# jizongFox/Self-paced-Contrastive-Learning

Measured on AMD Instinct MI355X. Metric: pretrain slices/sec/node (UNet+InfoNCE, 224^2, bs=32/GPU), higher is better.
Workload: dtype bf16; 1 GPU; BASELINE.json configs[1]: self-paced pretrain step, UNet base (max_channel=256) encoder to Conv5 + ProjectionHead(256,256,256) + SelfPacedSupConLoss(soft, partition labels, correct_grad) fwd+bwd + RAdam; slices_per_gpu=32, images_per_gpu_step=64, image=1x224x224, global_batch=32, parallelism=dp1, params=1311056, hipgraph=epocher, capture_steps=3

## Files before the change

### include/spcl_hip.h

```cpp
#ifndef SPCL_HIP_H
#define SPCL_HIP_H
#include <stddef.h>
#include <stdint.h>
#ifdef __cplusplus
extern "C" {
#endif

#define SPCL_F32 0
#define SPCL_BF16 1

#define SPCL_OK 0
#define SPCL_EINVAL (-1)
#define SPCL_ELAUNCH (-2)
#define SPCL_EUNSUPPORTED (-3)

#define SPCL_ABI_VERSION 22
int spcl_abi_version(void);
const char* spcl_last_error(void);

size_t spcl_supcon_workspace_bytes(int n, int d);
int spcl_supcon_forward(const float* z1, const float* z2, const float* labels, const float* mask, int n, int d,
                        float temperature, int sp_mode, float gamma, int correct_grad, float* ws, float* out,
                        void* stream);
int spcl_supcon_backward(const float* labels, const float* mask, int n, int d, float temperature, int sp_mode,
                         float gamma, const float* ws_fwd, float* ws_bwd, const float* out_fwd,
                         const float* grad_out, float* dz1, float* dz2, void* stream);
size_t spcl_supcon_bwd_workspace_bytes(int n, int d);
int spcl_supcon_unit_gradient_block(int n, int d, size_t* offset_floats, int* row_pitch);
int spcl_supcon_forward_heads(int K, const float* z1, const float* z2, size_t z_stride, const float* labels, int n,
                              int d, float temperature, int sp_mode, const float* gammas, int correct_grad, float* ws,
                              size_t ws_stride, float* out, void* stream);
int spcl_supcon_rows_supported(int n, int d);
int spcl_supcon_forward_rows(int K, const float* o1, const float* o2, size_t o_stride, const float* labels, int n, int d,
                             float temperature, int sp_mode, const float* gammas, int correct_grad, float* ws,
                             size_t ws_stride, float* out, void* stream);
int spcl_supcon_backward_heads(int K, const float* labels, int n, int d, float temperature, int sp_mode,
                               const float* gammas, const float* ws_fwd, size_t ws_stride, float* ws_bwd,
                               size_t wsb_stride, const float* out_fwd, const float* grad_out, float* dz1, float* dz2,
                               size_t z_stride, void* stream);
int spcl_supcon_materialize(const float* labels, const float* mask, int n, int d, float temperature, int sp_mode,
                            float gamma, const float* ws_fwd, float* sim_logits, float* sim_exp, float* pos_mask,
                            float* neg_mask, float* sp_mask, void* stream);

size_t spcl_supcon_xpos_workspace_bytes(int n, int d);
int spcl_supcon_xpos_forward(const float* z1, const float* z2, const float* labels, const float* mask, int n, int d,
                             float temperature, float* ws, float* out, void* stream);
int spcl_supcon_xpos_backward(const float* z1, const float* z2, int n, int d, float temperature, const float* ws,
                              const float* grad_out, float* dz1, float* dz2, void* stream);

size_t spcl_supcon_weighted_workspace_bytes(int n, int d);
int spcl_supcon_weighted_forward(const float* z1, const float* z2, const float* labels, const float* w11,
                                 const float* w22, const float* w12, int blocks, int mask_semantics, int in_mode, int n,
                                 int d, float temperature, float* ws, float* out, void* stream);
int spcl_supcon_weighted_backward(const float* z1, const float* z2, int n, int d, float temperature, float* ws,
                                  const float* grad_out, float* dz1, float* dz2, void* stream);
int spcl_supcon_weighted_materialize(const float* z1, const float* z2, const float* labels, const float* w11,
                                     const float* w22, const float* w12, int blocks, int mask_semantics, int n, int d,
                                     float temperature, float* ws, float* sim_logits, float* sim_exp, float* pos_weight,
                                     float* enable_mask, void* stream);

int spcl_proj_forward(const void* feat, int dtype, int N, int HW, int C, int Cs, const float* w1, const float* b1,
                      const float* w2, const float* b2, int hid, int out_dim, int normalize, float* pooled,
                      float* pre, float* o, float* z, void* stream);
int spcl_proj_backward(const float* dz, int dtype, int N, int HW, int C, int Cs, const float* w1, const float* w2,
                       int hid, int out_dim, int normalize, const float* pooled, const float* pre, const float* o,
                       float* dw1, float* db1, float* dw2, float* db2, float* scratch ,
                       void* dfeat, void* stream);

int spcl_proj_heads_forward(int K, const void* feat, int dtype, int N, int HW, int C, int Cs, const float* const* w1 ,
                            const float* const* b1 , const float* const* w2 , const float* const* b2 ,
                            int hid, int out_dim, int normalize, float* pooled, float* const* pre ,
                            float* const* o , float* const* z , void* stream);
int spcl_proj_heads_backward(int K, const float* const* dz , int dtype, int N, int HW, int C, int Cs,
                             const float* const* w1 , const float* const* w2 , int hid, int out_dim,
                             int normalize, const float* pooled, const float* const* pre ,
                             const float* const* o , float* const* dw1 , float* const* db1 ,
                             float* const* dw2 , float* const* db2 , float* scratch, void* dfeat, void* stream);
int spcl_proj_heads_backward_pooled(int K, const float* const* dz, int dtype, int N, int HW, int C, int Cs,
                                    const float* const* w1, const float* const* w2, int hid, int out_dim, int normalize,
                                    const float* pooled, const float* const* pre, const float* const* o, float* const* dw1,
                                    float* const* db1, float* const* dw2, float* const* db2, float* scratch, void* dfeat_nc,
                                    void* stream);


size_t spcl_conv_packed_elems(int Cin, int Cout, int kind, int dtype);
int spcl_conv_pack_weights(const float* w_oihw, int Cin, int Cout, int kind, int dtype, void* packed, void* stream);
int spcl_conv_pack_weights_both(const float* w_oihw, int Cin, int Cout, int dtype, void* packed_fwd,
                                void* packed_dgrad, void* stream);

int spcl_conv_pack_weights_block(const float* wa_oihw, int CinA, int CoutA, void* a_fwd, void* a_dgrad,
                                 const float* wb_oihw, int CinB, int CoutB, void* b_fwd, void* b_dgrad, int dtype,
                                 void* stream);
int spcl_conv_pack_weights_block_at(const float* wa_oihw, int CinA, int CoutA, void* a_fwd, void* a_dgrad,
                                    const float* wb_oihw, int CinB, int CoutB, void* b_fwd, void* b_dgrad, int dtype,
                                    int H, int W, void* stream);

#define SPCL_PACK_MULTI_MAX 24
typedef struct spcl_pack_item {
  const float* w_oihw;
// ... 236 lines not shown
                          void* stream);
int spcl_adam_apply_staged(float* param, const float* grad, double grad_scale, float* exp_avg, float* exp_avg_sq, size_t n,
                           int64_t* step, const float* coef, double beta1, double beta2, double eps, double weight_decay,
                           int decoupled, int k, const void* const* src, void* const* dst, const float* count, void* stream);
int spcl_sgd_step_scaled(float* param, const float* grad, double grad_scale, float* momentum_buffer, size_t n, int64_t* step,
                         const float* lr, double momentum, double dampening, double weight_decay, int nesterov, float* coef,
                         int k, const void* const* src, void* const* dst, const float* count, void* stream);
int spcl_sgd_apply_staged(float* param, const float* grad, double grad_scale, float* momentum_buffer, size_t n, int64_t* step,
                          const float* coef, double momentum, double dampening, double weight_decay, int nesterov, int k,
                          const void* const* src, void* const* dst, const float* count, void* stream);

int spcl_accumulate_scalars(int k, const void* const* src, void* const* dst, const float* count, void* stream);

int spcl_stage_bytes(void* dst, const void* host_src, size_t nbytes, void* stream);
int spcl_copy_pair(void* dst_a, const void* src_a, size_t bytes_a, void* dst_b, const void* src_b, size_t bytes_b,
                   void* stream);

int spcl_augment_views(const float* src, int S, int HS, int WS, const int* params, int nviews, float* out, int OH,
                       int OW, void* stream);
int spcl_augment_views_pil(const float* src, int S, int HS, int WS, const int* params, int nviews, float* out, int OH,
                           int OW, void* stream);
int spcl_rows_linear_forward(const void* x, int x_dtype, long ldx, int leaky_in, const float* W, const float* bias, int M,
                             int K, int N, float* y, void* stream);
int spcl_rows_linear_forward_act(const void* x, int x_dtype, long ldx, const float* W, const float* bias, int M, int K, int N,
                                 void* h, int h_dtype, void* stream);
int spcl_adaptive_avgpool2d_backward_act(const float* dout, const void* act, int dtype, int N, int H, int W, int C, int OH,
                                         int OW, void* dx, void* stream);
int spcl_rows_linear_backward_input(const void* g, int g_dtype, const float* W, const float* pre, int M, int N, int K, void* dx,
                                    int dx_dtype, long lddx, void* stream);
size_t spcl_rows_linear_backward_weight_workspace_bytes(int M, int N, int K);
int spcl_rows_linear_backward_weight(const void* g, int g_dtype, const void* x, int x_dtype, long ldx, int leaky_in, int M, int N,
                                     int K, float* ws, size_t ws_bytes, float* dW, float* db, void* stream);
int spcl_augment_views_recipe(const float* src, const unsigned char* labels, int S, int HS, int WS, const int* params,
                              int nviews, float* out, long long* label_out, int OH, int OW, int max_pad, void* stream);
size_t spcl_augment_views_recipe_workspace_bytes(int nviews, int OH, int OW);
int spcl_augment_views_recipe_ws(const float* src, const unsigned char* labels, int S, int HS, int WS, const int* params,
                                 int nviews, float* out, long long* label_out, int OH, int OW, int max_pad, void* workspace,
                                 size_t workspace_bytes, void* stream);
int spcl_resize_bilinear_pil(const float* src, int S, int HS, int WS, const int* bounds_x, const int* kk_x, int ksize_x,
                             const int* bounds_y, const int* kk_y, int ksize_y, float* tmp, float* out, int OH, int OW,
                             void* stream);

int spcl_flip_batch(const void* x, void* out, int elem_size, int N, int C, int H, int W, const uint8_t* flags,
                    void* stream);
int spcl_flip_pair(const void* first, const void* second, void* out, int elem_size, int N, int C, int H, int W,
                   const uint8_t* flags, void* stream);
int spcl_flip_pair_stage(const void* first, const void* second, void* out, int elem_size, int N, int C, int H, int W,
                         void* stage_dst, const void* host_src, size_t nbytes, size_t flag_off, void* stream);

int spcl_profile_enable(int on);
int spcl_profile_count(void);
int spcl_profile_get(int i, char* name, int name_cap, float* usec, double* bytes, double* flops);

typedef struct spcl_bn_acc {
  long long* acc;
  const float* gamma;
  const float* beta;
  float* running_mean;
  float* running_var;
  long long* num_batches_tracked;
  float* st;
  float momentum, eps;
  float count;
  int C, CS;
} spcl_bn_acc;
size_t spcl_bn_acc_elems(int CS);
int spcl_conv_bn_acc_supported(int dtype, int N, int H, int W, int CinK, int CoutS, int in_kind, int with_stats_acc);
int spcl_conv3x3_forward_acc(const void* x, int dtype, int N, int H, int W, int CinK, int CoutS, const void* w_packed,
                             const spcl_bn_acc* in_bn, const float* in_scale, const float* in_shift, void* y,
                             long long* stats_acc, float* stats_rows, void* stream);
int spcl_bnrelu_pool_forward_acc(const void* y, int dtype, int N, int H, int W, int CS, const spcl_bn_acc* bn, void* act_out,
                                 void* pool_out, void* stream);
int spcl_bnrelu_gap_supported(int dtype, int H, int W, int C, int CS);
int spcl_bnrelu_gap_forward(const void* y, int dtype, int N, int H, int W, int C, int CS, const float* scale,
                            const float* shift, const spcl_bn_acc* bn, void* act_out, float* gap_out, void* stream);
int spcl_conv_dgrad_bnstats_acc_supported(int dtype, int N, int H, int W, int CinK, int CoutS);
int spcl_conv3x3_dgrad_bnstats_acc(const void* dy, int dtype, int N, int H, int W, int CinK, int CoutS, const void* w_packed,
                                   void* g, const void* y2, const float* scale2, const float* shift2, const float* mean2,
                                   long long* acc, void* stream);
int spcl_conv_dgrad_poolstats_acc_supported(int dtype, int N, int H, int W, int CinK, int CoutS, int H2, int W2);
int spcl_conv3x3_dgrad_poolstats_acc(const void* dy, int dtype, int N, int H, int W, int CinK, int CoutS, const void* w_packed,
                                     void* g, const void* y2, int H2, int W2, const float* scale2, const float* shift2,
                                     const float* mean2, long long* acc, void* stream);
int spcl_bnrelu_backward_acc(const void* y, const void* dact, const void* dpool, const void* dact_nc, int dtype, int N, int H,
                             int W, int C, int CS, const float* st4, int training, long long* acc, float* dgamma, float* dbeta,
                             void* dy, void* stream);
int spcl_bnrelu_backward_fill_acc(const void* y, void* dact, int dact_stride, const void* dpool, const void* d_up, int dtype,
                                  int N, int H, int W, int C, int CS, const float* st4, int training, long long* acc,
                                  float* dgamma, float* dbeta, void* dy, void* stream);
int spcl_bnrelu_backward_rows_acc(const void* y, const void* dact, const void* dpool, const float* rows, int nrows, int dtype,
                                  int N, int H, int W, int C, int CS, const float* st4, int training, long long* acc,
                                  float* dgamma, float* dbeta, void* dy, void* stream);

size_t spcl_iic_joint_workspace_bytes(int S, int K, int pad);
int spcl_iic_joint_forward(const float* lx, const float* ly, long ld, int N, int H, int W, int S, int K, int pad,
                           const uint8_t* flags_x, long long* jacc, void* stream);
size_t spcl_iic_loss_workspace_bytes(int S, int T);
int spcl_iic_loss(const long long* jacc, const float* jf32, int S, int K, int T, int dense, float scale, float* j_out,
                  float* loss, float* dj, int* nan_flag, void* ws, size_t ws_bytes, void* stream);
int spcl_iic_joint_backward(const float* lx, const float* ly, long ld, int N, int H, int W, int S, int K, int pad,
                            const uint8_t* flags_x, const float* dj, const float* gscale, float* dlx, float* dly, void* stream);
size_t spcl_consistency_workspace_bytes(int N, int H, int W);
int spcl_consistency_softmax_mse(const float* a, const float* b, int N, int C, int H, int W, const uint8_t* flags_a,
                                 float weight, float* loss, float* db, void* ws, size_t ws_bytes, void* stream);

int spcl_iic_patch_plan(int N, int C, int H, int W, int pad, int patch, int* num_patches, size_t* ws_bytes, size_t* dj_elems);
int spcl_iic_patch_forward(const float* lx, const float* ly, int N, int C, int H, int W, int pad, int patch,
                           const uint8_t* flags_y, float scale, float* loss, float* patch_loss, int* nan_flag, float* dj,
                           void* ws, size_t ws_bytes, void* stream);
int spcl_iic_patch_backward(const float* lx, const float* ly, int N, int C, int H, int W, int pad, int patch,
                            const uint8_t* flags_y, const float* dj, const float* gscale, float* dlx, float* dly, void* stream);

int spcl_ema_update(float* teacher, const float* student, size_t n, double alpha, double decay, void* stream);
size_t spcl_mt_softmax_mse_workspace_bytes(int N, int H, int W);
int spcl_mt_softmax_mse(const float* teacher, const float* student_logits, int N, int C, int H, int W,
                        const uint8_t* flags_teacher, int teacher_mode, float weight, float* loss, float* dstudent, void* ws,
                        size_t ws_bytes, void* stream);
size_t spcl_entropy_softmax_workspace_bytes(int N, int H, int W);
int spcl_entropy_softmax(const float* logits, int N, int C, int H, int W, float eps, float weight, float* loss, float* dlogits,
                         void* ws, size_t ws_bytes, void* stream);
size_t spcl_ucmt_workspace_bytes(int N, int H, int W);
int spcl_ucmt_softmax_mse(const float* teacher, const float* const* noisy, int K, const float* student_logits, int N, int C,
                          int H, int W, const uint8_t* flags_teacher, float threshold, float eps, float weight, float* loss,
                          float* dstudent, unsigned long long* kept, uint8_t* mask, void* ws, size_t ws_bytes, void* stream);

int spcl_mixup_images(const float* image, const float* image_tf, const int* index, int N2, size_t per_sample, float lam,
                      float oml, float* out, void* stream);
size_t spcl_mixup_kl_workspace_bytes(int N2, int H, int W);
int spcl_mixup_kl_onehot(const float* logits, const int64_t* target, const int64_t* target_tf, const int* index, int N2, int C,
                         int H, int W, float lam, float oml, float eps, float weight, float* loss, float* dlogits, void* ws,
                         size_t ws_bytes, void* stream);

int spcl_patch4s2_rows_forward(const float* a, int Ca, long a_sn, long a_sc, long a_sh, long a_sw, const float* b, int Cb,
                               long b_sn, long b_sc, long b_sh, long b_sw, int N, int H, int W, int mode, const float* scale,
                               const float* shift, float* rows, void* stream);
int spcl_patch4s2_rows_backward(const float* drows, const float* x, int N, int H, int W, int C, int c_lo, int mode,
                                const float* scale, const float* shift, float* dx, void* stream);
size_t spcl_rows_bn_workspace_bytes(int M, int C);
int spcl_rows_bn_forward(const float* x, int M, int C, const float* gamma, const float* beta, float eps, float momentum,
                         float* running_mean, float* running_var, float* stats, void* ws, size_t ws_bytes, void* stream);
int spcl_rows_bn_eval_affine(const float* gamma, const float* beta, const float* running_mean, const float* running_var,
                             float eps, int C, float* stats, void* stream);
int spcl_rows_bn_backward(const float* du, const float* x, int M, int C, const float* gamma, const float* stats, int training,
                          float* dx, float* dgamma, float* dbeta, void* ws, size_t ws_bytes, void* stream);
size_t spcl_discr_head_workspace_bytes(int N, int H, int W, int C);
int spcl_discr_head_forward(const float* x, int N, int H, int W, int C, const float* scale, const float* shift, const float* w,
                            int y, float* t, float* d, float* loss, float* dt, void* ws, size_t ws_bytes, void* stream);
int spcl_discr_head_backward(const float* x, int N, int H, int W, int C, const float* scale, const float* shift, const float* w,
                             const float* dt, const float* grad, float* du, float* dw, void* ws, size_t ws_bytes, void* stream);

int spcl_mine_pairs_forward(const void* feat, const uint8_t* flags, int dtype, int n, int H, int W, int C, void* joint, void* marg,
                            void* stream);
int spcl_mine_pairs_backward(const void* djoint, const void* dmarg, const uint8_t* flags, int dtype, int n, int H, int W, int C,
                             void* dfeat, void* stream);
size_t spcl_mine_head_workspace_bytes(int n, int H, int W, int C);
int spcl_mine_head_forward(const void* act_joint, const void* act_marg, int dtype, int n, int H, int W, int C, const float* w,
                           const float* b, float* t, float* maxima, int* argmax, float* loss, void* ws, size_t ws_bytes,
                           void* stream);
int spcl_mine_head_backward(const float* t, const float* maxima, const int* argmax, const float* w, const float* grad, int dtype,
                            int n, int H, int W, int C, void* dact_joint, void* dact_marg, float* dw, float* db, void* stream);

size_t spcl_pica_workspace_bytes(int S);
int spcl_pica_seg_loss(const long long* jacc, const float* jf32, int S, int K, int T, double lamda_ne, float scale, float* j_out,
                       float* loss, float* ce_out, float* dj, void* ws, size_t ws_bytes, void* stream);
int spcl_pica_global_loss(const float* lx, const float* ly, long ld, int N, int S, int K, float lamda, float scale,
                          const float* gscale, float* loss, float* ce_out, float* dlx, float* dly, void* ws, size_t ws_bytes,
// ... 7 lines not shown
```

### self-paced-contrastive-learning_amd/csrc/bn.hip

```cpp
#include <mutex>
#include <type_traits>
#include "bn_acc.hpp"
#include "common.hpp"
#include "image_acorr.hpp"

namespace spcl {

typedef __attribute__((ext_vector_type(4))) uint32_t u32x4;
template <typename T> struct Chunk;
template <> struct Chunk<float> { static constexpr int EPC = 4; };
template <> struct Chunk<bf16_t> { static constexpr int EPC = 8; };

template <typename T> __device__ __forceinline__ void unpack(u32x4 raw, float* v);
template <> __device__ __forceinline__ void unpack<float>(u32x4 raw, float* v) {
#pragma unroll
  for (int e = 0; e < 4; ++e) v[e] = __uint_as_float(raw[e]);
}
template <> __device__ __forceinline__ void unpack<bf16_t>(u32x4 raw, float* v) {
#pragma unroll
  for (int e = 0; e < 4; ++e) {
    v[2 * e] = __uint_as_float(raw[e] << 16);
    v[2 * e + 1] = __uint_as_float(raw[e] & 0xffff0000u);
  }
}
// ... 120 lines not shown
    }
    __syncthreads();
    bn_fold_lanes<CW>(n, s1, s2, red);
    if (tl == 0) bn_final_channel(c, C, n, s1, s2, f, SPCL_BN_PREFETCH ? ch : bn_prefetch_channel(c, C, f));
    return;
  }
  if (tl != 0) return;
  if (!FINAL) {
    double* q = partial + (size_t)blockIdx.y * 3 * CS + c;
    q[0] = n; q[CS] = s1; q[2 * CS] = s2;
    return;
  }
  bn_final_channel(c, C, n, s1, s2, f, SPCL_BN_PREFETCH ? ch : bn_prefetch_channel(c, C, f));
}

__device__ __forceinline__ void bn_final_channel(int c, int C, double n, double s1, double s2, const BnFinalArgs& f,
                                                 const BnChan& ch) {
  if (c >= C) {
    f.mean[c] = 0.f; f.invstd[c] = 0.f; f.scale[c] = 0.f; f.shift[c] = 0.f;
    return;
  }
  const double mu = s1 / n;
  const double m2 = fmax(s2 - s1 * mu, 0.0);
  const double var = m2 / n;
  const float is = 1.0f / sqrtf((float)var + f.eps);
  const float sc = ch.gamma * is;
  f.mean[c] = (float)mu;
  f.invstd[c] = is;
  f.scale[c] = sc;
  f.shift[c] = ch.beta - (float)mu * sc;
  if (f.running_mean != nullptr) f.running_mean[c] = (1.f - f.momentum) * ch.rm + f.momentum * (float)mu;
  if (f.running_var != nullptr) {
    const double unbiased = n > 1.0 ? m2 / (n - 1.0) : var;
    f.running_var[c] = (1.f - f.momentum) * ch.rv + f.momentum * (float)unbiased;
  }
  if (f.nbt != nullptr && c == 0) f.nbt[0] += 1;
}

__global__ __launch_bounds__(256) void bn_eval_affine_kernel(int C, int CS, const float* __restrict__ gamma,
                                                             const float* __restrict__ beta,
                                                             const float* __restrict__ rm, const float* __restrict__ rv,
                                                             float eps, float* mean, float* invstd, float* scale,
                                                             float* shift) {
  const int c = blockIdx.x * blockDim.x + threadIdx.x;
  if (c >= CS) return;
  if (c >= C) { mean[c] = 0.f; invstd[c] = 0.f; scale[c] = 0.f; shift[c] = 0.f; return; }
  const float is = 1.0f / sqrtf(rv[c] + eps);
  const float sc = gamma[c] * is;
  mean[c] = rm[c];
  invstd[c] = is;
  scale[c] = sc;
  shift[c] = beta[c] - rm[c] * sc;
}

struct BnEvalItems {
  spcl_bn_eval_item it[SPCL_BN_EVAL_MAX];
  int blk_end[SPCL_BN_EVAL_MAX];
};
__global__ __launch_bounds__(256) void bn_eval_affine_multi_kernel(BnEvalItems p, int n) {
  int i = 0;
  for (int k = 0; k < n; ++k) i += (int)blockIdx.x >= p.blk_end[k] ? 1 : 0;
  if (i >= n) return;
  const spcl_bn_eval_item& q = p.it[i];
  const int c = ((int)blockIdx.x - (i > 0 ? p.blk_end[i - 1] : 0)) * 256 + threadIdx.x;
  if (c >= q.CS) return;
  float* mean = q.st;
  float* invstd = q.st + q.CS;
  float* scale = q.st + 2 * q.CS;
  float* shift = q.st + 3 * q.CS;
  if (c >= q.C) { mean[c] = 0.f; invstd[c] = 0.f; scale[c] = 0.f; shift[c] = 0.f; return; }
  const float is = 1.0f / sqrtf(q.running_var[c] + q.eps);
  const float sc = q.gamma[c] * is;
  mean[c] = q.running_mean[c];
  invstd[c] = is;
  scale[c] = sc;
  shift[c] = q.beta[c] - q.running_mean[c] * sc;
}

template <typename T> struct Word;
template <> struct Word<float> {
  static constexpr int EPW = 1;
  static __device__ __forceinline__ float get(uint32_t w, int) { return __uint_as_float(w); }
  static __device__ __forceinline__ uint32_t make(const float* v) { return __float_as_uint(v[0]); }
};
template <> struct Word<bf16_t> {
  static constexpr int EPW = 2;
  static __device__ __forceinline__ float get(uint32_t w, int h) {
    return __uint_as_float(h ? (w & 0xffff0000u) : (w << 16));
  }
  static __device__ __forceinline__ uint32_t make(const float* v) {
    return (uint32_t)f32_to_bf16(v[0]) | ((uint32_t)f32_to_bf16(v[1]) << 16);
  }
};

template <int EPC> __device__ __forceinline__ void load_coef(float* dst, const float* src, int cc) {
#pragma unroll
  for (int e = 0; e < EPC; e += 4) *(f32x4*)&dst[e] = *(const f32x4*)(src + cc * EPC + e);
}

template <int EPC>
__device__ __forceinline__ void acc_coef_fwd(const BnAccFwd& bn, int cc, float* sc, float* sh) {
  __shared__ float cl[2][256];
  const int c = threadIdx.x;
  if (c < bn.CS) {
    BnAccFwdRaw raw;
    raw.load(bn, c);
    float a, b;
    bn_acc_fwd_channel(bn, raw, c, a, b, blockIdx.x == 0);
    cl[0][c] = a;
    cl[1][c] = b;
  }
  __syncthreads();
#pragma unroll
  for (int e = 0; e < EPC; ++e) {
    sc[e] = cl[0][cc * EPC + e];
    sh[e] = cl[1][cc * EPC + e];
  }
}
template <int EPC>
__device__ __forceinline__ void acc_coef_bwd(const BnAccBwd& bw, int cc, float* A, float* B) {
  __shared__ float cl[2][256];
  const int c = threadIdx.x;
  if (c < bw.CS) {
    BnAccBwdRaw raw;
    raw.load(bw, c);
    float a, b;
    bn_acc_bwd_channel(bw, raw, c, a, b, blockIdx.x == 0);
    cl[0][c] = a;
    cl[1][c] = b;
  }
  __syncthreads();
#pragma unroll
  for (int e = 0; e < EPC; ++e) {
    A[e] = cl[0][cc * EPC + e];
    B[e] = cl[1][cc * EPC + e];
  }
}

constexpr int STREAM_UNROLL = 2;
constexpr int IMG_WGRAD_WG = 2048;

template <typename T>
__global__ __launch_bounds__(256, 6) void bnrelu_fwd_lin_kernel(const T* __restrict__ y, size_t npix, int CS,
                                                             const float* __restrict__ scale,
                                                             const float* __restrict__ shift, T* __restrict__ act,
                                                             int AS ,
                                                             BnAccFwd bn = BnAccFwd{}) {
  constexpr int EPC = Chunk<T>::EPC, U = STREAM_UNROLL;
  const int CPC = CS / EPC, PL = 256 / CPC;
  const int cc = threadIdx.x % CPC, pl = threadIdx.x / CPC;
  float sc[EPC], sh[EPC];
  if (bn.acc != nullptr) acc_coef_fwd<EPC>(bn, cc, sc, sh);
  if (pl >= PL) return;
  if (bn.acc == nullptr) {
    load_coef<EPC>(sc, scale, cc);
    load_coef<EPC>(sh, shift, cc);
  }
  const size_t stride = (size_t)gridDim.x * PL;
  for (size_t p = (size_t)blockIdx.x * PL + pl; p < npix; p += U * stride) {
    u32x4 r[U];
#pragma unroll
    for (int u = 0; u < U; ++u)
      if (p + u * stride < npix) r[u] = *(const u32x4*)(y + (p + u * stride) * CS + cc * EPC);
#pragma unroll
    for (int u = 0; u < U; ++u) {
      if (p + u * stride >= npix) break;
      float v[EPC];
      unpack<T>(r[u], v);
#pragma unroll
      for (int e = 0; e < EPC; ++e) v[e] = fmaxf(fmaf(sc[e], v[e], sh[e]), 0.f);
      *(u32x4*)(act + (p + u * stride) * AS + cc * EPC) = pack<T>(v);
    }
  }
}

// ... 44 lines not shown
#pragma unroll
      for (int u = 0; u < U; ++u) {
        if (p + u * PL >= HW) break;
        float v[EPC];
        unpack<T>(r[u], v);
#pragma unroll
        for (int e = 0; e < EPC; ++e) v[e] = fmaxf(fmaf(sc[e], v[e], sh[e]), 0.f);
        const u32x4 pk = pack<T>(v);
        *(u32x4*)(ab + (size_t)(p + u * PL) * CS) = pk;
        unpack<T>(pk, v);
#pragma unroll
        for (int e = 0; e < EPC; ++e) s[e] += v[e];
      }
    }
#pragma unroll
    for (int e = 0; e < EPC; ++e) part[pl * CW + cc * EPC + e] = s[e];
  }
  __syncthreads();
  const int c = threadIdx.x;
  if (c < CW && c0 + c < C) {
    float t = 0.f;
    for (int q = 0; q < PL; ++q) t += part[q * CW + c];
    gap[(size_t)blockIdx.x * C + c0 + c] = t / (float)HW;
  }
}

template <typename T>
__global__ __launch_bounds__(256, 6) void bnrelu_fwd_up2_kernel(const T* __restrict__ y, unsigned nrows , int W,
                                                             int CS, const float* __restrict__ scale,
                                                             const float* __restrict__ shift, T* __restrict__ up) {
  constexpr int EPC = Chunk<T>::EPC;
  const int CPC = CS / EPC, PL = 256 / CPC;
  const int cc = threadIdx.x % CPC, pl = threadIdx.x / CPC;
  if (pl >= PL) return;
  float sc[EPC], sh[EPC];
  load_coef<EPC>(sc, scale, cc);
  load_coef<EPC>(sh, shift, cc);
  for (unsigned r = blockIdx.x; r < nrows; r += gridDim.x) {
    const T* yr = y + (size_t)r * W * CS + cc * EPC;
    T* o0 = up + (size_t)(2 * r) * (2 * W) * CS + cc * EPC;
    for (int w = pl; w < W; w += 2 * PL) {
      u32x4 rr[2];
      const bool second = w + PL < W;
      rr[0] = *(const u32x4*)(yr + (size_t)w * CS);
      if (second) rr[1] = *(const u32x4*)(yr + (size_t)(w + PL) * CS);
#pragma unroll
      for (int u = 0; u < 2; ++u) {
        if (u == 1 && !second) break;
        float v[EPC];
        unpack<T>(rr[u], v);
#pragma unroll
        for (int e = 0; e < EPC; ++e) v[e] = fmaxf(fmaf(sc[e], v[e], sh[e]), 0.f);
        const u32x4 pv = pack<T>(v);
        T* o = o0 + (size_t)(2 * (w + u * PL)) * CS;
        *(u32x4*)o = pv;
        *(u32x4*)(o + CS) = pv;
        *(u32x4*)(o + (size_t)2 * W * CS) = pv;
        *(u32x4*)(o + (size_t)2 * W * CS + CS) = pv;
      }
    }
  }
}

template <typename T>
struct Window {
  u32x4 ry[4];
  bool valid[4];
  size_t off[4];
  template <bool FAST = false>
  __device__ __forceinline__ void load(const T* y, size_t row0, int oy, int ox, int H, int W, int CS, int cc) {
    constexpr int EPC = Chunk<T>::EPC;
    const bool y1 = FAST || 2 * oy + 1 < H, x1 = FAST || 2 * ox + 1 < W;
    const size_t o00 = (row0 * W + 2 * ox) * CS + cc * EPC;
    off[0] = o00; off[1] = o00 + CS; off[2] = o00 + (size_t)W * CS; off[3] = off[2] + CS;
    valid[0] = true; valid[1] = x1; valid[2] = y1; valid[3] = x1 && y1;
#pragma unroll
    for (int k = 0; k < 4; ++k) {
      ry[k] = (u32x4){0u, 0u, 0u, 0u};
      if (valid[k]) ry[k] = *(const u32x4*)(y + off[k]);
    }
  }
};

template <typename T, bool FAST>
__global__ __launch_bounds__(256, 4) void bnrelu_fwd_pool_kernel(const T* __restrict__ y, int N, int H, int W, int CS,
                                                              const float* __restrict__ scale,
                                                              const float* __restrict__ shift, T* __restrict__ act,
                                                              T* __restrict__ pool, int AS, BnAccFwd bn = BnAccFwd{}) {
  constexpr int EPC = Chunk<T>::EPC, EPW = Word<T>::EPW;
  const int CPC = CS / EPC, PL = 256 / CPC;
  const int cc = threadIdx.x % CPC, pl = threadIdx.x / CPC;
  float sc[EPC], sh[EPC];
  if (bn.acc != nullptr) acc_coef_fwd<EPC>(bn, cc, sc, sh);
  if (pl >= PL) return;
  const int PH = (H + 1) / 2, PW = (W + 1) / 2, OH = H / 2, OW = W / 2;
  if (bn.acc == nullptr) {
    load_coef<EPC>(sc, scale, cc);
    load_coef<EPC>(sh, shift, cc);
  }
  const int rows = N * PH;
  for (int r = blockIdx.x; r < rows; r += gridDim.x) {
    const int n = r / PH, oy = r - n * PH;
    const size_t row0 = (size_t)n * H + 2 * oy;
    for (int ox = pl; ox < PW; ox += 2 * PL) {
      Window<T> w[2];
      const bool second = ox + PL < PW;
      w[0].template load<FAST>(y, row0, oy, ox, H, W, CS, cc);
      if (second) w[1].template load<FAST>(y, row0, oy, ox + PL, H, W, CS, cc);
#pragma unroll
      for (int u = 0; u < 2; ++u) {
        if (u == 1 && !second) break;
        u32x4 mxw, aw[4];
#pragma unroll
        for (int wi = 0; wi < 4; ++wi) {
          float mx[EPW], a[4][EPW];
#pragma unroll
          for (int h = 0; h < EPW; ++h) {
            const int e = wi * EPW + h;
            mx[h] = 0.f;
#pragma unroll
            for (int k = 0; k < 4; ++k) {
              a[k][h] = fmaxf(fmaf(sc[e], Word<T>::get(w[u].ry[k][wi], h), sh[e]), 0.f);
              if (w[u].valid[k]) mx[h] = fmaxf(mx[h], a[k][h]);
            }
          }
          mxw[wi] = Word<T>::make(mx);
#pragma unroll
          for (int k = 0; k < 4; ++k) aw[k][wi] = Word<T>::make(a[k]);
        }
        const int oxu = ox + u * PL;
        if (act != nullptr) {
          const size_t a00 = (row0 * W + 2 * oxu) * AS + cc * EPC;
          const size_t aoff[4] = {a00, a00 + AS, a00 + (size_t)W * AS, a00 + (size_t)W * AS + AS};
#pragma unroll
          for (int k = 0; k < 4; ++k)
            if (w[u].valid[k]) *(u32x4*)(act + aoff[k]) = aw[k];
        }
        if (pool != nullptr && (FAST || (oy < OH && oxu < OW)))
          *(u32x4*)(pool + (((size_t)n * OH + oy) * OW + oxu) * CS + cc * EPC) = mxw;
      }
    }
  }
}

constexpr int BWD_MAX_WG = 2048;
constexpr int STREAM_MAX_WG = 2048;

template <typename T, int EPC>
__device__ __forceinline__ void wg_reduce_partials(const float* s1, const float* s2, int CS, int CPC, int PL,
                                                   float* __restrict__ partial, float (*red)[2 * EPC + 1],
                                                   long long* __restrict__ acc = nullptr) {
#pragma unroll
  for (int e = 0; e < EPC; ++e) {
    red[threadIdx.x][e] = s1[e];
    red[threadIdx.x][EPC + e] = s2[e];
  }
  __syncthreads();
  if (acc != nullptr) {
    for (int o = threadIdx.x; o < 4 * CS; o += 256) {
      const int c = o >> 2, which = (o >> 1) & 1, limb = o & 1;
      const int ccc = c / EPC, e = c - ccc * EPC;
      float s = 0.f;
      for (int p = 0; p < PL; ++p) s += red[p * CPC + ccc][which * EPC + e];
      bn_acc_add_word(acc, CS, (int)(blockIdx.x & (BN_ACC_REPLICAS - 1)), c, which, limb, s);
    }
    return;
  }
  for (int o = threadIdx.x; o < 2 * CS; o += 256) {
    const int which = o / CS, c = o - which * CS;
    const int ccc = c / EPC, e = c - ccc * EPC;
    float s = 0.f;
    for (int p = 0; p < PL; ++p) s += red[p * CPC + ccc][which * EPC + e];
    partial[((size_t)blockIdx.x * 2 + which) * CS + c] = s;
  }
}

template <typename T>
__global__ __launch_bounds__(256, 5) void bnrelu_bwd_reduce_lin_kernel(const T* __restrict__ y, const T* __restrict__ g,
                                                                    size_t npix, int CS,
                                                                    const float* __restrict__ mean,
                                                                    const float* __restrict__ invstd,
                                                                    const float* __restrict__ scale,
                                                                    const float* __restrict__ shift,
                                                                    float* __restrict__ partial ,
                                                                    int GS ,
                                                                    long long* __restrict__ acc = nullptr) {
  constexpr int EPC = Chunk<T>::EPC, EPW = Word<T>::EPW, U = STREAM_UNROLL;
  __shared__ float red[256][2 * EPC + 1];
  const int CPC = CS / EPC, PL = 256 / CPC;
  const int cc = threadIdx.x % CPC, pl = threadIdx.x / CPC;
  float s1[EPC], s2[EPC];
#pragma unroll
  for (int e = 0; e < EPC; ++e) s1[e] = s2[e] = 0.f;
  if (pl < PL) {
    float sc[EPC], sh[EPC], mu[EPC], is[EPC];
    load_coef<EPC>(sc, scale, cc);
    load_coef<EPC>(sh, shift, cc);
    load_coef<EPC>(mu, mean, cc);
    load_coef<EPC>(is, invstd, cc);
    const size_t stride = (size_t)gridDim.x * PL;
    for (size_t p = (size_t)blockIdx.x * PL + pl; p < npix; p += U * stride) {
      u32x4 ry[U], rg[U];
#pragma unroll
      for (int u = 0; u < U; ++u) {
        ry[u] = rg[u] = (u32x4){0u, 0u, 0u, 0u};
        if (p + u * stride < npix) {
          ry[u] = *(const u32x4*)(y + (p + u * stride) * CS + cc * EPC);
          rg[u] = *(const u32x4*)(g + (p + u * stride) * GS + cc * EPC);
        }
      }
#pragma unroll
      for (int u = 0; u < U; ++u)
#pragma unroll
        for (int wi = 0; wi < 4; ++wi)
#pragma unroll
          for (int h = 0; h < EPW; ++h) {
            const int e = wi * EPW + h;
            const float yv = Word<T>::get(ry[u][wi], h);
            const float dz = fmaf(sc[e], yv, sh[e]) > 0.f ? Word<T>::get(rg[u][wi], h) : 0.f;
            s1[e] += dz;
            s2[e] = fmaf(dz, yv - mu[e], s2[e]);
          }
// ... 177 lines not shown
    const float a = fmaxf(z[k], 0.f);
    if (k == 0) m = a;
    else if (a > m) { m = a; best = k; }
  }
  const float dp = complete ? Word<T>::get(rdp[wi], h) : 0.f;
#pragma unroll
  for (int k = 0; k < 4; ++k) {
    float g = has_g ? Word<T>::get(rg[k][wi], h) : 0.f;
    g += (k == best) ? dp : 0.f;
    dz[k] = z[k] > 0.f ? g : 0.f;
  }
}

#ifndef SPCL_BWD_POOL_MAXW
#define SPCL_BWD_POOL_MAXW 0
#endif
#if SPCL_BWD_POOL_MAXW
#define BWD_POOL_WPE __attribute__((amdgpu_waves_per_eu(3, SPCL_BWD_POOL_MAXW)))
#else
#define BWD_POOL_WPE
#endif
template <typename T, bool APPLY, bool FAST, bool ACC = false>
__global__ __launch_bounds__(256, 3) BWD_POOL_WPE void bnrelu_bwd_pool_kernel(const T* __restrict__ y, const T* __restrict__ dact,
                                                              const T* __restrict__ dpool, int N, int H, int W, int CS,
                                                              const float* __restrict__ mean,
                                                              const float* __restrict__ invstd,
                                                              const float* __restrict__ scale,
                                                              const float* __restrict__ shift,
                                                              const float* __restrict__ ab, float* __restrict__ partial,
                                                              T* __restrict__ dy, int GS = 0 ,
                                                              BnAccBwd bw = BnAccBwd{}) {
  constexpr int EPC = Chunk<T>::EPC, EPW = Word<T>::EPW;
  __shared__ float red[APPLY ? 1 : 256][2 * EPC + 1];
  const int CPC = CS / EPC, PL = 256 / CPC;
  const int cc = threadIdx.x % CPC, pl = threadIdx.x / CPC;
  const int PH = (H + 1) / 2, PW = (W + 1) / 2, OH = H / 2, OW = W / 2;
  const bool has_g = !FAST && dact != nullptr;
  float s1[EPC], s2[EPC];
#pragma unroll
  for (int e = 0; e < EPC; ++e) s1[e] = s2[e] = 0.f;
  float c0[EPC], c1[EPC];
  constexpr bool from_acc = APPLY && ACC;
  if (from_acc) acc_coef_bwd<EPC>(bw, cc, c0, c1);
  if (pl < PL) {
    float sc[EPC], sh[EPC];
    load_coef<EPC>(sc, scale, cc);
    load_coef<EPC>(sh, shift, cc);
    if (!from_acc) {
      load_coef<EPC>(c0, APPLY ? ab : mean, cc);
      load_coef<EPC>(c1, APPLY ? ab + CS : invstd, cc);
    }
    const int rows = N * PH;
    for (int r = blockIdx.x; r < rows; r += gridDim.x) {
      const int n = r / PH, oy = r - n * PH;
      const size_t row0 = (size_t)n * H + 2 * oy;
      for (int ox = pl; ox < PW; ox += PL) {
        Window<T> w;
        w.template load<FAST>(y, row0, oy, ox, H, W, CS, cc);
        u32x4 rg[4], rdp = {0u, 0u, 0u, 0u};
        if (has_g) {
          const size_t g00 = (row0 * W + 2 * ox) * GS + cc * EPC;
          const size_t goff[4] = {g00, g00 + GS, g00 + (size_t)W * GS, g00 + (size_t)W * GS + GS};
#pragma unroll
          for (int k = 0; k < 4; ++k) {
            rg[k] = (u32x4){0u, 0u, 0u, 0u};
            if (w.valid[k]) rg[k] = *(const u32x4*)(dact + goff[k]);
          }
        }
        const bool complete = FAST || (dpool != nullptr && oy < OH && ox < OW);
        if (complete) rdp = *(const u32x4*)(dpool + (((size_t)n * OH + oy) * OW + ox) * CS + cc * EPC);
        if (APPLY && FAST) __builtin_amdgcn_sched_barrier(0);
        u32x4 out[4];
#pragma unroll
        for (int wi = 0; wi < 4; ++wi) {
          float o[4][EPW];
#pragma unroll
          for (int h = 0; h < EPW; ++h) {
            const int e = wi * EPW + h;
            if (!APPLY && !has_g) {
              float zb = -1.f, yb = 0.f;
#pragma unroll
              for (int k = 0; k < 4; ++k) {
                const float yv = Word<T>::get(w.ry[k][wi], h);
                const float z = w.valid[k] ? fmaf(sc[e], yv, sh[e]) : -1.f;
                if (k == 0 || z > zb) { zb = z; yb = yv; }
              }
              const float dzb = (complete && zb > 0.f) ? Word<T>::get(rdp[wi], h) : 0.f;
              s1[e] += dzb;
              s2[e] = fmaf(dzb, yb - c0[e], s2[e]);
              continue;
            }
            if (APPLY && FAST) {
              float yk[4], z[4];
#pragma unroll
              for (int k = 0; k < 4; ++k) {
                yk[k] = Word<T>::get(w.ry[k][wi], h);
                z[k] = fmaf(sc[e], yk[k], sh[e]);
              }
              float m = fmaxf(z[0], 0.f);
              const bool s1 = z[1] > m;
              m = fmaxf(m, z[1]);
              const bool s2 = z[2] > m;
              m = fmaxf(m, z[2]);
              const bool s3 = z[3] > m;
              const bool b[4] = {z[0] > 0.f && !s1 && !s2 && !s3, s1 && !s2 && !s3, s2 && !s3, s3};
              const float dp = Word<T>::get(rdp[wi], h);
#pragma unroll
              for (int k = 0; k < 4; ++k) o[k][h] = fmaf(sc[e], b[k] ? dp : 0.f, fmaf(c0[e], yk[k], c1[e]));
              continue;
            }
            float yk[4], dz[4];
            window_dz<T>(w, rg, has_g, rdp, complete, wi, h, sc[e], sh[e], yk, dz);
#pragma unroll
            for (int k = 0; k < 4; ++k) {
              if (APPLY) o[k][h] = fmaf(sc[e], dz[k], fmaf(c0[e], yk[k], c1[e]));
              else {
                s1[e] += dz[k];
                s2[e] = fmaf(dz[k], yk[k] - c0[e], s2[e]);
              }
            }
          }
          if (APPLY) {
#pragma unroll
            for (int k = 0; k < 4; ++k) out[k][wi] = Word<T>::make(o[k]);
          }
        }
        if (APPLY) {
#pragma unroll
          for (int k = 0; k < 4; ++k)
            if (w.valid[k]) *(u32x4*)(dy + w.off[k]) = out[k];
        }
      }
    }
    if (!APPLY) {
#pragma unroll
      for (int e = 0; e < EPC; ++e) s2[e] *= bw.acc != nullptr ? 1.f : c1[e];
    }
  }
  if (!APPLY) wg_reduce_partials<T, EPC>(s1, s2, CS, CPC, PL, partial, red, const_cast<long long*>(bw.acc));
}

struct Image3Args {
  const float* acorr;
  int nacorr;
  const float* w_oihw;
  float* dw;
};
__device__ __forceinline__ int acorr_index(int a, int b) {
  return a * 9 - a * (a - 1) / 2 + (b - a);
}
__global__ __launch_bounds__(256) void bnrelu_bwd_fin_kernel(const float* __restrict__ partial, int nwg, int C, int CS,
                                                             float M, int training, const float* __restrict__ mean,
                                                             const float* __restrict__ invstd,
                                                             const float* __restrict__ scale,
                                                             float* __restrict__ dgamma, float* __restrict__ dbeta,
                                                             float* __restrict__ ab, float* __restrict__ zero_fill,
                                                             int nzero, int s2_centered, int rs, Image3Args im,
                                                             int transposed = 0) {
  __shared__ float red[11][4];
  __shared__ double racc4[4][64];
  __shared__ double racc[54];
  __shared__ float coef[2];
  const int c = blockIdx.x % CS, grp = blockIdx.x / CS;
  const bool split = gridDim.x == 3u * (unsigned)CS;
  const int t0 = split ? 3 * grp : 0, ntap = split ? 3 : 9;
  if (blockIdx.x == 0)
    for (int z = threadIdx.x; z < nzero; z += 256) zero_fill[z] = 0.f;
  const int lane = threadIdx.x & 63, wave = threadIdx.x >> 6;
// ... 251 lines not shown
      for (int u = 0; u < U; ++u) {
        const int ox = ox0 + u * PL;
        ok[u] = ox < W;
        const int c1 = min(ox, W - 1), c0 = max(c1 - 1, 0), c2 = min(c1 + 1, W - 1);
        const unsigned off = (unsigned)c1 * pix_bytes + lane_off;
        ry[u] = *(const raw_t*)(yr + off);
        rg[u] = *(const raw_t*)(gr + off);
        const bool left = ox > 0, right = ox + 1 < W;
#pragma unroll
        for (int k = 0; k < 3; ++k) {
          const char* xk = (const char*)xr[k];
          const float a0 = *(const float*)(xk + (unsigned)(c0 * 4)), a1 = *(const float*)(xk + (unsigned)(c1 * 4)),
                      a2 = *(const float*)(xk + (unsigned)(c2 * 4));
          xv[u][3 * k + 0] = left ? a0 : 0.f;
          xv[u][3 * k + 1] = a1;
          xv[u][3 * k + 2] = right ? a2 : 0.f;
        }
      }
#pragma unroll
      for (int u = 0; u < U; ++u)
#pragma unroll
        for (int e = 0; e < 4; ++e) {
          const float yv = Quad<T>::get(ry[u], e);
          const float dz = fmaf(sc[e], yv, sh[e]) > 0.f ? Quad<T>::get(rg[u], e) : 0.f;
          float dyv = fmaf(sc[e], dz, fmaf(A[e], yv, B[e]));
          dyv = ok[u] ? dyv : 0.f;
#pragma unroll
          for (int t = 0; t < 9; ++t) acc[t][e] = fmaf(dyv, xv[u][t], acc[t][e]);
        }
    }
  }
  const int lane = threadIdx.x & 63, wave = threadIdx.x >> 6;
  for (int o = 32; o >= QPP; o >>= 1) {
#pragma unroll
    for (int t = 0; t < 9; ++t)
#pragma unroll
      for (int e = 0; e < 4; ++e) acc[t][e] += __shfl_xor(acc[t][e], o, 64);
  }
  if (lane < QPP) {
#pragma unroll
    for (int t = 0; t < 9; ++t)
#pragma unroll
      for (int e = 0; e < 4; ++e) redw[(wave * 9 + t) * CS + lane * 4 + e] = acc[t][e];
  }
  __syncthreads();
  for (int o = threadIdx.x; o < 9 * CS; o += 256)
    wpart[(size_t)blockIdx.x * 9 * CS + o] =
        (redw[o] + redw[9 * CS + o]) + (redw[2 * 9 * CS + o] + redw[3 * 9 * CS + o]);
}

__global__ __launch_bounds__(256) void image_wgrad_final_kernel(const float* __restrict__ wpart, int nwg, int C, int CS,
                                                                float* __restrict__ dw) {
  __shared__ float red[256];
  const int t = blockIdx.x;
  const int RL = 256 / CS;
  const int c = threadIdx.x % CS, rl = threadIdx.x / CS;
  float s = 0.f;
  if (rl < RL) {
#pragma unroll 8
    for (int w = rl; w < nwg; w += RL) s += wpart[((size_t)w * 9 + t) * CS + c];
  }
  red[threadIdx.x] = s;
  __syncthreads();
  if (threadIdx.x < CS && threadIdx.x < C) {
    float tot = 0.f;
    for (int k = 0; k < RL; ++k) tot += red[k * CS + threadIdx.x];
    dw[threadIdx.x * 9 + t] = tot;
  }
}

static int stream_grid(size_t positions, int PL, int unroll, int cap) {
  size_t g = (positions + (size_t)PL * unroll - 1) / ((size_t)PL * unroll);
  if (g > (size_t)cap) g = cap;
  if (g < 1) g = 1;
  return (int)g;
}

static thread_local int tl_act_stride = 0, tl_dact_stride = 0;
static thread_local const void* tl_up2_src = nullptr;
static thread_local bool tl_acc_fill = false;

template <typename T>
static int bnrelu_fwd_launch(const void* y, int N, int H, int W, int CS, const float* scale, const float* shift,
                             void* act, void* pool, hipStream_t st, const BnAccFwd* bnp = nullptr) {
  constexpr int EPC = Chunk<T>::EPC;
  const BnAccFwd bn = bnp != nullptr ? *bnp : BnAccFwd{};
  static const int acc_wg = lab_env("SPCL_ACC_STREAM_WG", 768);
  const int STREAM_MAX_WG = bnp != nullptr ? acc_wg : spcl::STREAM_MAX_WG;
  const int PL = 256 / (CS / EPC);
  const int AS = tl_act_stride > 0 ? tl_act_stride : CS;
  const double tb = (double)N * H * W * CS * sizeof(T);
  prof_cost(tb * (1.0 + (act != nullptr ? 1.0 : 0.0) + (pool != nullptr ? 0.25 : 0.0)), 0.0);
  if (pool != nullptr) {
    const int rows = N * ((H + 1) / 2);
    if (H % 2 == 0 && W % 2 == 0) {
      SPCL_LAUNCH((bnrelu_fwd_pool_kernel<T, true>), dim3(rows < STREAM_MAX_WG ? rows : STREAM_MAX_WG), dim3(256), 0, st, (const T*)y, N, H,
                       W, CS, scale, shift, (T*)act, (T*)pool, AS, bn);
    } else {
      SPCL_LAUNCH((bnrelu_fwd_pool_kernel<T, false>), dim3(rows < STREAM_MAX_WG ? rows : STREAM_MAX_WG), dim3(256), 0, st, (const T*)y, N, H,
                       W, CS, scale, shift, (T*)act, (T*)pool, AS, bn);
    }
  } else {
    const size_t npix = (size_t)N * H * W;
    SPCL_LAUNCH((bnrelu_fwd_lin_kernel<T>), dim3(stream_grid(npix, PL, STREAM_UNROLL, STREAM_MAX_WG)), dim3(256), 0, st,
                       (const T*)y, npix, CS, scale, shift, (T*)act, AS, bn);
  }
  return 0;
}

template <typename T>
static int bnrelu_bwd_launch(const void* y, const void* dact, const void* dpool, int N, int H, int W, int C, int CS,
                             const float* mean, const float* invstd, const float* scale, const float* shift,
                             int training, float* ws, float* dgamma, float* dbeta, void* dy, hipStream_t st,
                             const float* img = nullptr, float* dw = nullptr, const float* rows = nullptr,
                             int nrows = 0, bool bcast = false ,
                             long long* acc = nullptr ) {
  constexpr int EPC = Chunk<T>::EPC;
  const BnAccBwd bw = acc != nullptr ? BnAccBwd{acc, mean , dgamma, dbeta,
                                                (float)((size_t)N * H * W), training, C, CS}
                                     : BnAccBwd{};
  static const int acc_wg = lab_env("SPCL_ACC_STREAM_WG", 768);
  const int STREAM_MAX_WG = acc != nullptr ? acc_wg : spcl::STREAM_MAX_WG;
  const bool pool = dpool != nullptr;
  const bool fill = acc != nullptr && tl_acc_fill;
  const int RED_MAX_WG = fill ? STREAM_MAX_WG : BWD_MAX_WG;
  const int GS = tl_dact_stride > 0 ? tl_dact_stride : CS;
  constexpr int rs = 2;
  const Image3Args im3{nullptr, 0, nullptr, nullptr};
  spcl_wgrad_tail* tail = img != nullptr ? take_tail_capture() : nullptr;
  const int PL = 256 / (CS / EPC);
  const size_t npix = (size_t)N * H * W;
  const int prows = N * ((H + 1) / 2);
  float* partial = ws;
  float* ab = ws != nullptr ? ws + (size_t)BWD_MAX_WG * 2 * CS : nullptr;
  const float M = (float)npix;
  int nwg, bsplit = 1;
  const double tb = (double)npix * CS * sizeof(T);
  const double gb = (dact != nullptr ? tb : 0.0) + (pool ? 0.25 * tb : 0.0);
  prof_cost(tb + gb, 0.0);
  const float* fin_src = partial;
  int fin_transposed = 0;
  if (acc != nullptr && !bcast && !fill) {
    nwg = 0;
  } else if (rows != nullptr && fill) {
    const int G = (nrows + 511) / 512;
    nwg = (nrows + G - 1) / G;
    SPCL_LAUNCH(bwd_rows_acc_kernel, dim3(nwg), dim3(256), 0, st, rows, nrows, G, CS, acc);
  } else if (rows != nullptr) {
    static const int fin_rows = lab_env("SPCL_BWD_FIN_MAX_ROWS", BWD_MAX_WG);
    if (nrows <= fin_rows) {
      fin_src = rows;
      nwg = nrows;
    } else {
      const int G = (nrows + BWD_MAX_WG - 1) / BWD_MAX_WG;
      nwg = (nrows + G - 1) / G;
      SPCL_LAUNCH(bwd_rows_group_kernel, dim3(nwg), dim3(256), 0, st, rows, nrows, G, CS, partial, rs, nwg,
                  (const float*)nullptr, 0, (float*)nullptr, 1);
      fin_transposed = 1;
    }
  } else if (pool) {
    nwg = prows < RED_MAX_WG ? prows : RED_MAX_WG;
    const BnAccBwd rbw = fill ? bw : BnAccBwd{};
    if (H % 2 == 0 && W % 2 == 0 && dact == nullptr && dpool != nullptr) {
      SPCL_LAUNCH((bnrelu_bwd_pool_kernel<T, false, true>), dim3(nwg), dim3(256), 0, st, (const T*)y, (const T*)dact,
                       (const T*)dpool, N, H, W, CS, mean, invstd, scale, shift, (const float*)nullptr, partial,
                       (T*)nullptr, 0, rbw);
    } else {
      SPCL_LAUNCH((bnrelu_bwd_pool_kernel<T, false, false>), dim3(nwg), dim3(256), 0, st, (const T*)y, (const T*)dact,
                       (const T*)dpool, N, H, W, CS, mean, invstd, scale, shift, (const float*)nullptr, partial,
                       (T*)nullptr, GS, rbw);
    }
  } else if (bcast) {
    static const int env_split = lab_env("SPCL_BCAST_SPLIT_MAX", 4);
    bsplit = (H * W + PL - 1) / PL;
    if (env_split > 0 && bsplit > env_split) bsplit = env_split;
    while (bsplit > 1 && N * bsplit > BWD_MAX_WG) bsplit = (bsplit + 1) / 2;
    nwg = N * bsplit;
    prof_cost(tb, 0.0);
    SPCL_LAUNCH((bnrelu_bwd_reduce_bcast_kernel<T>), dim3(nwg), dim3(256), 0, st, (const T*)y, (const T*)dact, H * W, CS,
                bsplit, mean, invstd, scale, shift, partial, acc);
  } else if (tl_up2_src != nullptr) {
    nwg = stream_grid(npix, PL, STREAM_UNROLL, RED_MAX_WG);
    prof_cost(tb * 6.0, 0.0);
// ... 132 lines not shown

extern "C" int spcl_bn_eval_affine_multi(const spcl_bn_eval_item* items, int n, void* stream) {
  SPCL_CHECK_ARG(items && n >= 1 && n <= SPCL_BN_EVAL_MAX, "bn_eval_affine_multi: 1 <= n <= %d layers", SPCL_BN_EVAL_MAX);
  BnEvalItems p;
  int blocks = 0;
  for (int i = 0; i < n; ++i) {
    SPCL_CHECK_ARG(items[i].gamma && items[i].beta && items[i].running_mean && items[i].running_var && items[i].st,
                   "bn_eval_affine_multi: null pointer (layer %d)", i);
    SPCL_CHECK_ARG(items[i].C > 0 && items[i].CS >= items[i].C, "bn_eval_affine_multi: bad shape (layer %d)", i);
    p.it[i] = items[i];
    blocks += cdiv(items[i].CS, 256);
    p.blk_end[i] = blocks;
  }
  SPCL_LAUNCH(bn_eval_affine_multi_kernel, dim3((unsigned)blocks), dim3(256), 0, (hipStream_t)stream, p, n);
  SPCL_LAUNCH_CHECK("bn_eval_affine_multi");
  return SPCL_OK;
}

extern "C" int spcl_bnrelu_pool_forward(const void* y, int dtype, int N, int H, int W, int CS, const float* scale,
                                        const float* shift, void* act_out, void* pool_out, void* stream) {
  SPCL_CHECK_ARG(y && scale && shift && (act_out || pool_out), "bnrelu_pool_forward: null pointer");
  SPCL_CHECK_ARG(N > 0 && H > 0 && W > 0 && CS > 0 && CS % 16 == 0 && CS <= 1024, "bnrelu_pool_forward: bad shape");
  SPCL_CHECK_ARG(!pool_out || (H >= 2 && W >= 2), "bnrelu_pool_forward: 2x2 pooling needs H,W >= 2");
  hipStream_t st = (hipStream_t)stream;
  if (dtype != SPCL_F32 && dtype != SPCL_BF16) {
    set_error("bnrelu_pool_forward: dtype %d", dtype);
    return SPCL_EINVAL;
  }
  if (dtype == SPCL_F32) bnrelu_fwd_launch<float>(y, N, H, W, CS, scale, shift, act_out, pool_out, st);
  else bnrelu_fwd_launch<bf16_t>(y, N, H, W, CS, scale, shift, act_out, pool_out, st);
  SPCL_LAUNCH_CHECK("bnrelu_pool_forward");
  return SPCL_OK;
}

extern "C" int spcl_bnrelu_gap_supported(int dtype, int H, int W, int C, int CS) {
  return (dtype == SPCL_F32 || dtype == SPCL_BF16) && H > 0 && W > 0 && (long)H * W <= 4096 && C > 0 && C <= CS && CS <= 256 &&
         CS % 16 == 0;
}

extern "C" int spcl_bnrelu_gap_forward(const void* y, int dtype, int N, int H, int W, int C, int CS, const float* scale,
                                       const float* shift, const spcl_bn_acc* bn, void* act_out, float* gap_out,
                                       void* stream) {
  SPCL_CHECK_ARG(y && act_out && gap_out && (bn || (scale && shift)), "bnrelu_gap_forward: null pointer");
  SPCL_CHECK_ARG(N > 0 && spcl_bnrelu_gap_supported(dtype, H, W, C, CS), "bnrelu_gap_forward: unsupported shape / dtype");
  BnAccFwd f{};
  if (bn != nullptr) {
    SPCL_CHECK_ARG(bn->acc && bn->gamma && bn->beta && bn->st && bn->CS == CS && bn->C > 0 && bn->C <= CS && bn->count >= 1.f,
                   "bnrelu_gap_forward: bad accumulator description");
    f = BnAccFwd{bn->acc, bn->gamma, bn->beta, bn->running_mean, bn->running_var, bn->num_batches_tracked, bn->st,
                 bn->momentum, bn->eps, bn->count, bn->C, bn->CS, 1.0 / (double)bn->count};
  }
  hipStream_t st = (hipStream_t)stream;
  const int CW = CS % 64 == 0 ? 64 : CS;
  if (dtype == SPCL_F32)
    SPCL_LAUNCH((bnrelu_fwd_gap_kernel<float>), dim3(N, CS / CW), dim3(256), 0, st, (const float*)y, H * W, C, CS, CW, scale,
                shift, (float*)act_out, gap_out, f);
  else
    SPCL_LAUNCH((bnrelu_fwd_gap_kernel<bf16_t>), dim3(N, CS / CW), dim3(256), 0, st, (const bf16_t*)y, H * W, C, CS, CW, scale,
                shift, (bf16_t*)act_out, gap_out, f);
  SPCL_LAUNCH_CHECK("bnrelu_gap_forward");
  return SPCL_OK;
}

extern "C" int spcl_bnrelu_pool_forward_acc(const void* y, int dtype, int N, int H, int W, int CS, const spcl_bn_acc* bn,
                                            void* act_out, void* pool_out, void* stream) {
  SPCL_CHECK_ARG(y && bn && (act_out || pool_out), "bnrelu_pool_forward_acc: null pointer");
  SPCL_CHECK_ARG(N > 0 && H > 0 && W > 0 && CS > 0 && CS % 16 == 0 && CS <= 256, "bnrelu_pool_forward_acc: bad shape (CS <= 256)");
  SPCL_CHECK_ARG(!pool_out || (H >= 2 && W >= 2), "bnrelu_pool_forward_acc: 2x2 pooling needs H,W >= 2");
  SPCL_CHECK_ARG(bn->acc && bn->gamma && bn->beta && bn->st && bn->CS == CS && bn->C > 0 && bn->C <= CS && bn->count >= 1.f,
                 "bnrelu_pool_forward_acc: bad accumulator description");
  hipStream_t st = (hipStream_t)stream;
  const BnAccFwd f{bn->acc, bn->gamma, bn->beta, bn->running_mean, bn->running_var, bn->num_batches_tracked, bn->st,
                   bn->momentum, bn->eps, bn->count, bn->C, bn->CS, 1.0 / (double)bn->count};
  if (dtype == SPCL_F32) bnrelu_fwd_launch<float>(y, N, H, W, CS, nullptr, nullptr, act_out, pool_out, st, &f);
  else if (dtype == SPCL_BF16) bnrelu_fwd_launch<bf16_t>(y, N, H, W, CS, nullptr, nullptr, act_out, pool_out, st, &f);
  else {
    set_error("bnrelu_pool_forward_acc: dtype %d", dtype);
    return SPCL_EINVAL;
  }
  SPCL_LAUNCH_CHECK("bnrelu_pool_forward_acc");
  return SPCL_OK;
}

extern "C" int spcl_bnrelu_backward_acc(const void* y, const void* dact, const void* dpool, const void* dact_nc, int dtype,
                                        int N, int H, int W, int C, int CS, const float* st4, int training, long long* acc,
                                        float* dgamma, float* dbeta, void* dy, void* stream) {
  SPCL_CHECK_ARG(y && st4 && acc && dgamma && dbeta && dy, "bnrelu_backward_acc: null pointer");
  SPCL_CHECK_ARG((dact != nullptr) + (dpool != nullptr) + (dact_nc != nullptr) == 1,
                 "bnrelu_backward_acc: exactly one of dact, dpool, dact_nc");
  SPCL_CHECK_ARG(N > 0 && H > 0 && W > 0 && C > 0 && CS >= C && CS % 16 == 0 && CS <= 256, "bnrelu_backward_acc: bad shape (CS <= 256)");
  SPCL_CHECK_ARG(!dpool || (H >= 2 && W >= 2 && H % 2 == 0 && W % 2 == 0), "bnrelu_backward_acc: pooled form needs even H, W");
  SPCL_CHECK_ARG(dtype == SPCL_BF16 || dtype == SPCL_F32, "bnrelu_backward_acc: dtype %d", dtype);
  hipStream_t st = (hipStream_t)stream;
  const float *mean = st4, *invstd = st4 + CS, *scale = st4 + 2 * CS, *shift = st4 + 3 * CS;
  const void* g = dact_nc != nullptr ? dact_nc : dact;
  if (dtype == SPCL_F32)
    bnrelu_bwd_launch<float>(y, g, dpool, N, H, W, C, CS, mean, invstd, scale, shift, training, nullptr, dgamma, dbeta, dy, st,
                             nullptr, nullptr, nullptr, 0, dact_nc != nullptr, acc);
  else
    bnrelu_bwd_launch<bf16_t>(y, g, dpool, N, H, W, C, CS, mean, invstd, scale, shift, training, nullptr, dgamma, dbeta, dy, st,
                              nullptr, nullptr, nullptr, 0, dact_nc != nullptr, acc);
  SPCL_LAUNCH_CHECK("bnrelu_backward_acc");
  return SPCL_OK;
}

extern "C" int spcl_bnrelu_up2_forward(const void* y, int dtype, int N, int H, int W, int CS, const float* scale,
                                       const float* shift, void* up_out, void* stream) {
  SPCL_CHECK_ARG(y && scale && shift && up_out, "bnrelu_up2_forward: null pointer");
  SPCL_CHECK_ARG(N > 0 && H > 0 && W > 0 && CS > 0 && CS % 16 == 0 && CS <= 1024, "bnrelu_up2_forward: bad shape");
  hipStream_t st = (hipStream_t)stream;
  const unsigned nrows = (unsigned)N * (unsigned)H;
  const unsigned grid = nrows < (unsigned)STREAM_MAX_WG ? nrows : (unsigned)STREAM_MAX_WG;
  const double tb = (double)N * H * W * CS * (dtype == SPCL_F32 ? 4.0 : 2.0);
  prof_cost(5.0 * tb, 0.0);
  if (dtype == SPCL_F32)
    SPCL_LAUNCH((bnrelu_fwd_up2_kernel<float>), dim3(grid), dim3(256), 0, st, (const float*)y, nrows, W, CS, scale, shift,
                (float*)up_out);
  else if (dtype == SPCL_BF16)
    SPCL_LAUNCH((bnrelu_fwd_up2_kernel<bf16_t>), dim3(grid), dim3(256), 0, st, (const bf16_t*)y, nrows, W, CS, scale, shift,
                (bf16_t*)up_out);
  else {
    set_error("bnrelu_up2_forward: dtype %d", dtype);
    return SPCL_EINVAL;
  }
  SPCL_LAUNCH_CHECK("bnrelu_up2_forward");
  return SPCL_OK;
}

extern "C" int spcl_bnrelu_pool_forward_strided(const void* y, int dtype, int N, int H, int W, int CS, const float* scale,
                                                const float* shift, void* act_out, int act_stride, void* pool_out,
                                                void* stream) {
  SPCL_CHECK_ARG(act_out && act_stride >= CS && act_stride % 8 == 0,
                 "bnrelu_pool_forward_strided: act_out with a pixel stride >= CS, a multiple of 8 elements");
  tl_act_stride = act_stride;
  const int rc = spcl_bnrelu_pool_forward(y, dtype, N, H, W, CS, scale, shift, act_out, pool_out, stream);
  tl_act_stride = 0;
  return rc;
}

extern "C" size_t spcl_bnrelu_bwd_workspace_bytes(int N, int H, int W, int CS) {
  (void)N; (void)H; (void)W;
  return ((size_t)BWD_MAX_WG * 2 * CS + 2 * (size_t)CS) * sizeof(float);
}

extern "C" int spcl_bnrelu_pool_backward(const void* y, const void* dact, const void* dpool, int dtype, int N, int H,
                                         int W, int C, int CS, const float* mean, const float* invstd,
                                         const float* scale, const float* shift, int training, float* ws,
                                         float* dgamma, float* dbeta, void* dy, void* stream) {
  SPCL_CHECK_ARG(y && (dact || dpool) && mean && invstd && scale && shift && ws && dgamma && dbeta && dy,
                 "bnrelu_pool_backward: null pointer");
  SPCL_CHECK_ARG(N > 0 && H > 0 && W > 0 && C > 0 && CS >= C && CS % 16 == 0 && CS <= 1024,
                 "bnrelu_pool_backward: bad shape");
  SPCL_CHECK_ARG(!dpool || (H >= 2 && W >= 2), "bnrelu_pool_backward: 2x2 pooling needs H,W >= 2");
  hipStream_t st = (hipStream_t)stream;
  if (dtype == SPCL_F32)
    bnrelu_bwd_launch<float>(y, dact, dpool, N, H, W, C, CS, mean, invstd, scale, shift, training, ws, dgamma, dbeta,
                             dy, st);
  else if (dtype == SPCL_BF16)
    bnrelu_bwd_launch<bf16_t>(y, dact, dpool, N, H, W, C, CS, mean, invstd, scale, shift, training, ws, dgamma, dbeta,
                              dy, st);
  else {
    set_error("bnrelu_pool_backward: dtype %d", dtype);
    return SPCL_EINVAL;
  }
  SPCL_LAUNCH_CHECK("bnrelu_pool_backward");
  return SPCL_OK;
// ... 253 lines not shown
```

### self-paced-contrastive-learning_amd/csrc/common.hpp

```cpp
#pragma once
#include <hip/hip_runtime.h>
#include <stdint.h>
#include <stdio.h>
#include <stdlib.h>
#include "../../include/spcl_hip.h"

typedef __attribute__((ext_vector_type(4))) float f32x4;
typedef __attribute__((ext_vector_type(8))) short bf16x8;
typedef __attribute__((ext_vector_type(4))) short s16x4;
typedef uint16_t bf16_t;

namespace spcl {

void set_error(const char* fmt, ...);

#define SPCL_CHECK_ARG(cond, ...)        \
  do {                                   \
    if (!(cond)) {                       \
      spcl::set_error(__VA_ARGS__);      \
      return SPCL_EINVAL;                \
    }                                    \
  } while (0)

void func_lds_limit(const void* fn, int bytes, const char* what);
const char* take_attr_error();

#define SPCL_LAUNCH_CHECK(name)                                                 \
  do {                                                                          \
    if (const char* a_ = spcl::take_attr_error()) {                             \
      (void)hipGetLastError();                                                  \
      spcl::set_error("%s: %s", name, a_);                                      \
      return SPCL_ELAUNCH;                                                      \
    }                                                                           \
    hipError_t e_ = hipGetLastError();                                          \
    if (e_ != hipSuccess) {                                                     \
      spcl::set_error("%s: launch failed: %s", name, hipGetErrorString(e_));    \
      return SPCL_ELAUNCH;                                                      \
    }                                                                           \
  } while (0)

extern bool g_prof_on;
void prof_begin(const void* kernel_fn, hipStream_t st);
void prof_end(hipStream_t st);
void prof_cost(double bytes, double flops);
struct ProfScope {
  hipStream_t st;
  bool on;
  ProfScope(const void* fn, hipStream_t s) : st(s), on(g_prof_on) { if (on) prof_begin(fn, s); }
  ~ProfScope() { if (on) prof_end(st); }
};
#define SPCL_LAUNCH(kernel, grid, block, lds, st, ...)                   \
  do {                                                                   \
    spcl::ProfScope prof_scope_((const void*)(kernel), (st));            \
    hipLaunchKernelGGL(kernel, grid, block, lds, st, __VA_ARGS__);       \
  } while (0)

__device__ __forceinline__ float bf16_to_f32(bf16_t v) { return __uint_as_float(((uint32_t)v) << 16); }
__device__ __forceinline__ bf16_t f32_to_bf16(float f) {
  __bf16 b = (__bf16)f;
  return __builtin_bit_cast(bf16_t, b);
}

template <typename T> struct Elem;
template <> struct Elem<float> {
  static constexpr int kDtype = SPCL_F32;
  __device__ static __forceinline__ float load(const float* p) { return *p; }
  __device__ static __forceinline__ void store(float* p, float v) { *p = v; }
};
template <> struct Elem<bf16_t> {
  static constexpr int kDtype = SPCL_BF16;
  __device__ static __forceinline__ float load(const bf16_t* p) { return bf16_to_f32(*p); }
  __device__ static __forceinline__ void store(bf16_t* p, float v) { *p = f32_to_bf16(v); }
};

__device__ __forceinline__ int lane_id() { return threadIdx.x & 63; }

__device__ __forceinline__ float wave_sum(float v) {
  v += __builtin_bit_cast(float, __builtin_amdgcn_update_dpp(0, __builtin_bit_cast(int, v), 0xB1, 0xF, 0xF, true));
  v += __builtin_bit_cast(float, __builtin_amdgcn_update_dpp(0, __builtin_bit_cast(int, v), 0x4E, 0xF, 0xF, true));
  v += __builtin_bit_cast(float, __builtin_amdgcn_update_dpp(0, __builtin_bit_cast(int, v), 0x141, 0xF, 0xF, true));
  v += __builtin_bit_cast(float, __builtin_amdgcn_update_dpp(0, __builtin_bit_cast(int, v), 0x140, 0xF, 0xF, true));
  v += __shfl_xor(v, 16, 64);
  v += __shfl_xor(v, 32, 64);
  return v;
}
__device__ __forceinline__ float wave_max(float v) {
  v = fmaxf(v, __builtin_bit_cast(float, __builtin_amdgcn_update_dpp(0, __builtin_bit_cast(int, v), 0xB1, 0xF, 0xF, true)));
  v = fmaxf(v, __builtin_bit_cast(float, __builtin_amdgcn_update_dpp(0, __builtin_bit_cast(int, v), 0x4E, 0xF, 0xF, true)));
  v = fmaxf(v, __builtin_bit_cast(float, __builtin_amdgcn_update_dpp(0, __builtin_bit_cast(int, v), 0x141, 0xF, 0xF, true)));
  v = fmaxf(v, __builtin_bit_cast(float, __builtin_amdgcn_update_dpp(0, __builtin_bit_cast(int, v), 0x140, 0xF, 0xF, true)));
  v = fmaxf(v, __shfl_xor(v, 16, 64));
  v = fmaxf(v, __shfl_xor(v, 32, 64));
  return v;
}
template <int CTRL> __device__ __forceinline__ double dpp_move_f64(double v) {
  const long long b = __builtin_bit_cast(long long, v);
  const int lo = __builtin_amdgcn_update_dpp(0, (int)(b & 0xffffffffll), CTRL, 0xF, 0xF, true);
  const int hi = __builtin_amdgcn_update_dpp(0, (int)(b >> 32), CTRL, 0xF, 0xF, true);
  return __builtin_bit_cast(double, ((long long)hi << 32) | (long long)(unsigned)lo);
}
__device__ __forceinline__ double row16_sum_f64(double v) {
  v += dpp_move_f64<0xB1>(v);
  v += dpp_move_f64<0x4E>(v);
  v += dpp_move_f64<0x141>(v);
  v += dpp_move_f64<0x140>(v);
  return v;
}
__device__ __forceinline__ float row16_max(float v) {
  v = fmaxf(v, __builtin_bit_cast(float, __builtin_amdgcn_update_dpp(0, __builtin_bit_cast(int, v), 0xB1, 0xF, 0xF, true)));
  v = fmaxf(v, __builtin_bit_cast(float, __builtin_amdgcn_update_dpp(0, __builtin_bit_cast(int, v), 0x4E, 0xF, 0xF, true)));
  v = fmaxf(v, __builtin_bit_cast(float, __builtin_amdgcn_update_dpp(0, __builtin_bit_cast(int, v), 0x141, 0xF, 0xF, true)));
  v = fmaxf(v, __builtin_bit_cast(float, __builtin_amdgcn_update_dpp(0, __builtin_bit_cast(int, v), 0x140, 0xF, 0xF, true)));
  return v;
}

spcl_wgrad_tail* take_tail_capture();

void launch_wgrad_reduce(const float* partial, int nsplit, int nblk_ci, int nblk_co, int CIB, int COB, int Cin, int Cout,
                         float* dw_oihw, hipStream_t st);

#ifndef SPCL_LAB
#define SPCL_LAB 0
#endif
inline int lab_env(const char* name, int dflt) {
#if SPCL_LAB
  const char* e = getenv(name);
  return e != nullptr ? atoi(e) : dflt;
#else
  (void)name;
  return dflt;
#endif
}

inline bool lab_flag(const char* name) {
#if SPCL_LAB
  return getenv(name) != nullptr;
#else
  (void)name;
  return false;
#endif
}

inline int cdiv(int a, int b) { return (a + b - 1) / b; }
inline int round_up(int a, int b) { return cdiv(a, b) * b; }

}
```

### self-paced-contrastive-learning_amd/csrc/conv.hip

```cpp
#include <stdlib.h>
#include "bn_acc.hpp"
#include "conv_common.hpp"
#include "image_acorr.hpp"

namespace spcl {

#ifndef SPCL_SPLIT_KC_MAX
#define SPCL_SPLIT_KC_MAX 64
#endif
__host__ __device__ inline int split_kc(int CinK, int CoutS) {
  const int cap = CoutS <= 16 ? 16 : (CoutS <= 32 ? 32 : SPCL_SPLIT_KC_MAX);
  return CinK < cap ? CinK : cap;
}
__host__ __device__ inline int split_pstride(int KC) {
  const int b = 3 * KC * 2;
  return (b / 32) % 2 == 1 ? b : b + 32;
}
__device__ __forceinline__ f32x4 mfma_bf16(u32x4 w, u32x4 x, f32x4 acc) {
  return __builtin_amdgcn_mfma_f32_16x16x32_bf16(__builtin_bit_cast(bf16x8, w), __builtin_bit_cast(bf16x8, x), acc, 0, 0, 0);
}

template <typename T, int TH, int TW, int NT, bool SPLIT = false>
__global__ __launch_bounds__(256) void conv3x3_mfma_kernel(ConvArgs a) {
  static_assert(!SPLIT || sizeof(T) == 4, "the split k-loop is the f32 storage path");
// ... 1469 lines not shown
  if (!(t.tw == 14 && launch_conv_fast(a, t.th, st))) {
    set_error("conv3x3_dgrad_bnstats_image: no specialised kernel for H=%d W=%d", H, W);
    return SPCL_EUNSUPPORTED;
  }
  SPCL_LAUNCH_CHECK("conv3x3_dgrad_bnstats_image");
  return SPCL_OK;
}

extern "C" int spcl_conv_dgrad_poolstats_supported(int dtype, int N, int H, int W, int CinK, int CoutS, int H2, int W2) {
  static const bool off = lab_flag("SPCL_NO_DGRAD_POOLSTATS");
  ConvArgs a;
  if (off || H != H2 / 2 || W != W2 / 2 || !dgrad_bnstats_args(a, dtype, N, H, W, CinK, CoutS)) return 0;
  if (conv_use_gemm(CinK, CoutS, H, W)) return 0;
  a.x = nullptr; a.y = nullptr; a.wp = nullptr;
  float dummy;
  a.rows2 = &dummy;
  a.H2 = H2; a.W2 = W2;
  TileCfg t = pick_tile(H, W);
  return (t.tw == 14 && launch_conv_fast(a, t.th, nullptr, true)) ? 1 : 0;
}

static int dgrad_poolstats_impl(const void* dy, int dtype, int N, int H, int W, int CinK, int CoutS, const void* w_packed,
                                void* g, const void* y2, int H2, int W2, const float* scale2, const float* shift2,
                                const float* mean2, float* rows2, long long* acc, void* stream);

extern "C" int spcl_conv3x3_dgrad_poolstats(const void* dy, int dtype, int N, int H, int W, int CinK, int CoutS,
                                            const void* w_packed, void* g, const void* y2, int H2, int W2,
                                            const float* scale2, const float* shift2, const float* mean2, float* rows2,
                                            void* stream) {
  SPCL_CHECK_ARG(rows2, "conv3x3_dgrad_poolstats: null pointer");
  return dgrad_poolstats_impl(dy, dtype, N, H, W, CinK, CoutS, w_packed, g, y2, H2, W2, scale2, shift2, mean2, rows2, nullptr,
                              stream);
}

extern "C" int spcl_conv_dgrad_poolstats_acc_supported(int dtype, int N, int H, int W, int CinK, int CoutS, int H2, int W2) {
  ConvArgs a;
  if (!spcl_conv_dgrad_poolstats_supported(dtype, N, H, W, CinK, CoutS, H2, W2)) return 0;
  if (!dgrad_bnstats_args(a, dtype, N, H, W, CinK, CoutS)) return 0;
  a.x = nullptr; a.y = nullptr; a.wp = nullptr;
  float dummy;
  long long dummy2;
  a.rows2 = &dummy;
  a.rows2_acc = &dummy2;
  a.H2 = H2; a.W2 = W2;
  TileCfg t = pick_tile(H, W);
  return (t.tw == 14 && launch_conv_fast(a, t.th, nullptr, true)) ? 1 : 0;
}

extern "C" int spcl_conv3x3_dgrad_poolstats_acc(const void* dy, int dtype, int N, int H, int W, int CinK, int CoutS,
                                                const void* w_packed, void* g, const void* y2, int H2, int W2,
                                                const float* scale2, const float* shift2, const float* mean2,
                                                long long* acc, void* stream) {
  SPCL_CHECK_ARG(acc, "conv3x3_dgrad_poolstats_acc: null pointer");
  return dgrad_poolstats_impl(dy, dtype, N, H, W, CinK, CoutS, w_packed, g, y2, H2, W2, scale2, shift2, mean2, nullptr, acc,
                              stream);
}

static int dgrad_poolstats_impl(const void* dy, int dtype, int N, int H, int W, int CinK, int CoutS, const void* w_packed,
                                void* g, const void* y2, int H2, int W2, const float* scale2, const float* shift2,
                                const float* mean2, float* rows2, long long* acc, void* stream) {
  SPCL_CHECK_ARG(dy && w_packed && g && y2 && scale2 && shift2 && mean2, "conv3x3_dgrad_poolstats: null pointer");
  ConvArgs a;
  if (H != H2 / 2 || W != W2 / 2 || !dgrad_bnstats_args(a, dtype, N, H, W, CinK, CoutS) ||
      conv_use_gemm(CinK, CoutS, H, W)) {
    set_error("conv3x3_dgrad_poolstats: unsupported configuration");
    return SPCL_EUNSUPPORTED;
  }
  a.x = dy; a.y = g; a.wp = w_packed;
  a.y2 = y2; a.scale2 = scale2; a.shift2 = shift2; a.mean2 = mean2;
  a.rows2 = acc != nullptr ? (float*)acc : rows2;
  a.rows2_acc = acc;
  a.H2 = H2; a.W2 = W2;
  hipStream_t st = (hipStream_t)stream;
  const double px = (double)N * H * W;
  prof_cost(px * (CinK + CoutS) * 2.0 + (double)N * H2 * W2 * CoutS * 2.0 + 9.0 * CinK * CoutS * 2.0, 2.0 * px * 9.0 * CinK * CoutS);
  TileCfg t = pick_tile(H, W);
  if (!(t.tw == 14 && launch_conv_fast(a, t.th, st))) {
    set_error("conv3x3_dgrad_poolstats: no specialised kernel for H=%d W=%d CinK=%d CoutS=%d", H, W, CinK, CoutS);
    return SPCL_EUNSUPPORTED;
  }
  SPCL_LAUNCH_CHECK("conv3x3_dgrad_poolstats");
  return SPCL_OK;
}
```

### self-paced-contrastive-learning_amd/csrc/conv_common.hpp

```cpp
#pragma once
#include "common.hpp"

namespace spcl {

struct BnAccFwd;
template <typename T> struct Chunk;
template <> struct Chunk<float> { static constexpr int EPC = 4; };
template <> struct Chunk<bf16_t> { static constexpr int EPC = 8; };

struct uint4_ { uint32_t x, y, z, w; };
typedef __attribute__((ext_vector_type(4))) uint32_t u32x4;

__host__ __device__ inline int conv_kc(int CinK) { return CinK < 64 ? CinK : 64; }
template <typename T> __host__ __device__ inline int conv_pstride(int KC) {
  int b = KC * (int)sizeof(T);
  return b == 32 ? 32 : b + 32;
}
template <typename T> __host__ __device__ inline int conv_nsteps(int KC) {
  int cp = KC / Chunk<T>::EPC;
  return (9 * cp + 3) / 4;
}

struct ConvArgs {
  const void* x;
  void* y;
  const void* wp;
  float* stats;
  const float* in_scale;
  const float* in_shift;
  int N, H, W;
  int CinS;
  int CinK;
  int CoutS;
  int in_mode;
  int tilesX, tilesY;
  int tpw;
  int dbg;
  const void* y2 = nullptr;
  const float* scale2 = nullptr;
  const float* shift2 = nullptr;
  const float* mean2 = nullptr;
  float* rows2 = nullptr;
  int H2 = 0, W2 = 0;
  const float* img2 = nullptr;
  const void* x2 = nullptr;
  void* y_hi = nullptr;
  bool x_up2 = false;
  float* acorr_rows = nullptr;
  const float* img1 = nullptr;
  const void* wp1 = nullptr;
  long long* stats_acc = nullptr;
  long long* rows2_acc = nullptr;
  const struct BnAccFwd* in_bn = nullptr;
};

struct split_f32 { float v; };
template <> struct Chunk<split_f32> { static constexpr int EPC = 4; };
bool conv_f32_split();

typedef __attribute__((ext_vector_type(2))) float f32x2_;
typedef __attribute__((ext_vector_type(2))) __bf16 bf16x2v_;
struct Split3 { uint32_t hi, mid, lo; };
__device__ __forceinline__ Split3 split3_pair(float v0, float v1) {
  Split3 o;
  f32x2_ v = {v0, v1};
  o.hi = __builtin_bit_cast(uint32_t, __builtin_convertvector(v, bf16x2v_));
  v[0] -= __uint_as_float(o.hi << 16);
  v[1] -= __uint_as_float(o.hi & 0xffff0000u);
  o.mid = __builtin_bit_cast(uint32_t, __builtin_convertvector(v, bf16x2v_));
  v[0] -= __uint_as_float(o.mid << 16);
  v[1] -= __uint_as_float(o.mid & 0xffff0000u);
  o.lo = __builtin_bit_cast(uint32_t, __builtin_convertvector(v, bf16x2v_));
  return o;
}
__device__ __forceinline__ void split3_chunk(const float* e, u32x4& ph, u32x4& pm, u32x4& pl) {
#pragma unroll
  for (int k = 0; k < 4; ++k) {
    const Split3 o = split3_pair(e[2 * k], e[2 * k + 1]);
    ph[k] = o.hi;
    pm[k] = o.mid;
    pl[k] = o.lo;
  }
}
template <typename T> __device__ __forceinline__ f32x4 mfma_chunk(u32x4 w, u32x4 x, f32x4 acc);
template <> __device__ __forceinline__ f32x4 mfma_chunk<bf16_t>(u32x4 w, u32x4 x, f32x4 acc) {
  return __builtin_amdgcn_mfma_f32_16x16x32_bf16(__builtin_bit_cast(bf16x8, w), __builtin_bit_cast(bf16x8, x), acc, 0,
                                                 0, 0);
}
template <> __device__ __forceinline__ f32x4 mfma_chunk<float>(u32x4 w, u32x4 x, f32x4 acc) {
  f32x4 wf = __builtin_bit_cast(f32x4, w), xf = __builtin_bit_cast(f32x4, x);
  acc = __builtin_amdgcn_mfma_f32_16x16x4f32(wf[0], xf[0], acc, 0, 0, 0);
  acc = __builtin_amdgcn_mfma_f32_16x16x4f32(wf[1], xf[1], acc, 0, 0, 0);
  acc = __builtin_amdgcn_mfma_f32_16x16x4f32(wf[2], xf[2], acc, 0, 0, 0);
  acc = __builtin_amdgcn_mfma_f32_16x16x4f32(wf[3], xf[3], acc, 0, 0, 0);
  return acc;
}

__device__ __forceinline__ float row16_sum(float v) {
  v += __builtin_bit_cast(float, __builtin_amdgcn_update_dpp(0, __builtin_bit_cast(int, v), 0xB1, 0xF, 0xF, true));
  v += __builtin_bit_cast(float, __builtin_amdgcn_update_dpp(0, __builtin_bit_cast(int, v), 0x4E, 0xF, 0xF, true));
  v += __builtin_bit_cast(float, __builtin_amdgcn_update_dpp(0, __builtin_bit_cast(int, v), 0x141, 0xF, 0xF, true));
  v += __builtin_bit_cast(float, __builtin_amdgcn_update_dpp(0, __builtin_bit_cast(int, v), 0x140, 0xF, 0xF, true));
  return v;
}

typedef __attribute__((ext_vector_type(2))) float f32x2;
typedef __attribute__((ext_vector_type(2))) __bf16 bf16x2v;
typedef __attribute__((ext_vector_type(2))) short s16x2v;

__device__ __forceinline__ uint32_t relu_bf16x2(uint32_t packed) {
  const s16x2v z = {0, 0};
  return __builtin_bit_cast(uint32_t, __builtin_elementwise_max(__builtin_bit_cast(s16x2v, packed), z));
}

template <typename T> __device__ __forceinline__ u32x4 bnrelu_regs(u32x4 raw, const float* s, const float* b);
template <> __device__ __forceinline__ u32x4 bnrelu_regs<float>(u32x4 raw, const float* s, const float* b) {
  f32x4 v = __builtin_bit_cast(f32x4, raw);
#pragma unroll
  for (int e = 0; e < 4; ++e) v[e] = fmaxf(fmaf(s[e], v[e], b[e]), 0.f);
  return __builtin_bit_cast(u32x4, v);
}
template <> __device__ __forceinline__ u32x4 bnrelu_regs<bf16_t>(u32x4 raw, const float* s, const float* b) {
  u32x4 out;
#pragma unroll
  for (int e = 0; e < 4; ++e) {
    float lo = __uint_as_float(raw[e] << 16), hi = __uint_as_float(raw[e] & 0xffff0000u);
// ... 47 lines not shown
```

### self-paced-contrastive-learning_amd/csrc/conv_fast.hip

```cpp
#include <stdlib.h>
#include <type_traits>
#include <vector>
#include "bn_acc.hpp"
#include "conv_common.hpp"

namespace spcl {

struct FastArgs {
  const unsigned char* x;
  const unsigned char* x2;
  unsigned char* y;
  unsigned char* y_hi;
  int up2;
  const u32x4* wp;
  float* stats;
  const float* in_scale;
  const float* in_shift;
  int N, H, W, CinK, CoutS, tilesX, tilesY, gy;
  unsigned long long* stamps;
  int ipw;
  int lds_flip;
  int xcd_remap;
  const unsigned char* y2;
  const float* scale2;
// ... 558 lines not shown
        }
      }
    }
  };
  if (!RM || r16 < TW) {
  if (YPRE) {
    request_chunk(0);
    __builtin_amdgcn_sched_barrier(0);
  }
  uint2 pk_prev[NT];
  int ob_prev = 0;
#pragma unroll
  for (int i = 0; i < MT; ++i) {
    const bool ok = RM || (16 * i + 15 < NPIX) || (16 * i + r16 < NPIX);
    if (YPRE && i % GM == 0 && (i / GM + 1) * GM < MT) {
      request_chunk(i / GM + 1);
      __builtin_amdgcn_sched_barrier(0);
    }
    if (ok) {
      const float keep = (!shifted || (pyc >= oy && px >= ox)) ? 1.f : 0.f;
#pragma unroll
      for (int j = 0; j < NT; ++j) {
        if (MODE != 4 || a.y != nullptr) {
          constexpr bool PAIRED = SPCL_FAST_WIDE_STORES && MODE != 4 && !(KC == 64 && NW == 1);
          const bool first = PAIRED && i % 2 == 0 && i + 1 < MT && (RM || 16 * (i + 1) + 15 < NPIX);
          const bool second = PAIRED && i % 2 == 1 && (RM || 16 * i + 15 < NPIX);
          if (first || second) {
            const f32x2 lo = {acc[i][j][0], acc[i][j][1]}, hi = {acc[i][j][2], acc[i][j][3]};
            uint2 pkc;
            pkc.x = __builtin_bit_cast(uint32_t, __builtin_convertvector(lo, bf16x2v));
            pkc.y = __builtin_bit_cast(uint32_t, __builtin_convertvector(hi, bf16x2v));
            if (first) {
              pk_prev[j] = pkc;
              ob_prev = ob;
            } else {
              const auto rx = __builtin_amdgcn_permlane16_swap(pk_prev[j].x, pkc.x, false, false);
              const auto ry = __builtin_amdgcn_permlane16_swap(pk_prev[j].y, pkc.y, false, false);
              const u32x4 v = {rx[0], ry[0], rx[1], ry[1]};
              *(u32x4*)(yj[j] + ((g & 1) ? ob - 8 : ob_prev)) = v;
            }
          } else {
            store4_fast<bf16_t>(yj[j] + ob, acc[i][j]);
          }
        }
        if (M2) {
          const uint2 yr = YPRE ? ypre[i][j][0] : *(const uint2*)(y2j[j] + ob);
          const f32x2 glo = {acc[i][j][0], acc[i][j][1]}, ghi = {acc[i][j][2], acc[i][j][3]};
          const uint32_t g0 = __builtin_bit_cast(uint32_t, __builtin_convertvector(glo, bf16x2v));
          const uint32_t g1 = __builtin_bit_cast(uint32_t, __builtin_convertvector(ghi, bf16x2v));
          const float yv[4] = {__uint_as_float(yr.x << 16), __uint_as_float(yr.x & 0xffff0000u),
                               __uint_as_float(yr.y << 16), __uint_as_float(yr.y & 0xffff0000u)};
          const float gv[4] = {__uint_as_float(g0 << 16), __uint_as_float(g0 & 0xffff0000u),
                               __uint_as_float(g1 << 16), __uint_as_float(g1 & 0xffff0000u)};
#pragma unroll
          for (int r = 0; r < 4; ++r) {
            const float dz = (st2[j] && fmaf(sc2[j][r], yv[r], sh2[j][r]) > 0.f) ? gv[r] * keep : 0.f;
            ssum[j][r] += dz;
            ssq[j][r] = fmaf(dz, yv[r] - mu2[j][r], ssq[j][r]);
            if (MODE == 4) *(bf16_t*)(lds + M4_DZ + (4 * g + r) * 448 + pyc * 32 + px * 2) = f32_to_bf16(dz);
          }
        } else if (MODE == 3) {
          const f32x2 glo = {acc[i][j][0], acc[i][j][1]}, ghi = {acc[i][j][2], acc[i][j][3]};
          const uint32_t g0 = __builtin_bit_cast(uint32_t, __builtin_convertvector(glo, bf16x2v));
          const uint32_t g1 = __builtin_bit_cast(uint32_t, __builtin_convertvector(ghi, bf16x2v));
          const float gv[4] = {__uint_as_float(g0 << 16), __uint_as_float(g0 & 0xffff0000u),
                               __uint_as_float(g1 << 16), __uint_as_float(g1 & 0xffff0000u)};
          uint2 yr[4];
          if (YPRE) {
#pragma unroll
            for (int k = 0; k < 4; ++k) yr[k] = ypre[i][j][k];
          } else {
            const unsigned char* wb = a.y2 + ((((size_t)n * a.H2 + 2 * (y0 + pyc)) * a.W2 + 2 * (x0 + px)) * rowb) +
                                      ((nt0 + j) * 16 + 4 * g) * 2;
#pragma unroll
            for (int k = 0; k < 4; ++k) yr[k] = *(const uint2*)(wb + ((size_t)(k >> 1) * a.W2 + (k & 1)) * rowb);
          }
#pragma unroll
          for (int r = 0; r < 4; ++r) {
            float zb = -1.f, yb = 0.f;
#pragma unroll
            for (int k = 0; k < 4; ++k) {
              const uint32_t wd = r < 2 ? yr[k].x : yr[k].y;
              const float yv = (r & 1) ? __uint_as_float(wd & 0xffff0000u) : __uint_as_float(wd << 16);
              const float z = fmaf(sc2[j][r], yv, sh2[j][r]);
              if (k == 0 || z > zb) {
                zb = z;
                yb = yv;
              }
            }
            const float dz = zb > 0.f ? gv[r] * keep : 0.f;
            ssum[j][r] += dz;
            ssq[j][r] = fmaf(dz, yb - mu2[j][r], ssq[j][r]);
          }
        } else {
          const f32x4 av = acc[i][j] * keep;
          ssum[j] += av;
          ssq[j] += av * acc[i][j];
        }
      }
    }
    px += DPX;
    pyc += DPY;
    ob += dob;
    if (!RM && px >= TW) {
      px -= TW;
      pyc += 1;
      ob += wrapo;
    }
  }
  }
  constexpr int RS = MODE == 4 ? 11 : 2;
  const int replica = (int)((blockIdx.x + gridDim.x * (blockIdx.y + gridDim.y * blockIdx.z)) & (BN_ACC_REPLICAS - 1));
  if ((MODE == 2 || MODE == 3) && a.rows2_acc != nullptr) {
#pragma unroll
    for (int j = 0; j < NT; ++j) {
      f32x4 s1, s2;
#pragma unroll
      for (int r = 0; r < 4; ++r) {
        s1[r] = row16_sum(ssum[j][r]);
        s2[r] = row16_sum(ssq[j][r]);
      }
      bn_acc_add_row16(a.rows2_acc, a.CoutS, replica, (nt0 + j) * 16 + 4 * g, r16, s1, s2);
    }
  } else if (M2 || MODE == 3) {
#pragma unroll
    for (int j = 0; j < NT; ++j) {
      f32x4 o;
#pragma unroll
      for (int r = 0; r < 4; ++r) {
        const float s1 = row16_sum(ssum[j][r]), s2 = row16_sum(ssq[j][r]);
        o[r] = r16 == 0 ? s1 : s2;
      }
      if (up_only) {
        if (r16 < 2 && st2[j])
          *(f32x4*)(a.rows2 + ((size_t)tile * RS + r16) * (a.CoutS / 2) + (nt0 + j - ntn / 2) * 16 + 4 * g) = o;
      } else if (r16 < 2) *(f32x4*)(a.rows2 + ((size_t)tile * RS + r16) * a.CoutS + (nt0 + j) * 16 + 4 * g) = o;
    }
    if (MODE == 4) {
      static_assert(MODE != 4 || NT == 1, "image tap sums: one n-tile");
      __syncthreads();
      const int tap = r16 < 9 ? r16 : 0, tky = tap / 3, tkx = tap - 3 * tky;
      const unsigned char* pa = lds + M4_DZ + r16 * 448 + (g >> 1) * 32 + (g & 1) * 16;
      const unsigned char* pb = lds + M4_IM + tkx * 512 + ((g >> 1) + tky) * 32 + (g & 1) * 16;
      f32x4 D = {0.f, 0.f, 0.f, 0.f};
#pragma unroll
      for (int ks = 0; ks < TH / 2; ++ks)
        D = mfma_chunk<bf16_t>(*(const u32x4*)(pa + ks * 64), *(const u32x4*)(pb + ks * 64), D);
      if (r16 < 9) *(f32x4*)(a.rows2 + ((size_t)tile * RS + 2 + r16) * a.CoutS + nt0 * 16 + 4 * g) = D;
    }
  } else if ((MODE == 0 || M1) && a.stats_acc != nullptr) {
#pragma unroll
    for (int j = 0; j < NT; ++j) {
      f32x4 s1, s2;
#pragma unroll
      for (int r = 0; r < 4; ++r) {
        s1[r] = row16_sum(ssum[j][r]);
        s2[r] = row16_sum(ssq[j][r]);
      }
      bn_acc_add_row16(a.stats_acc, a.CoutS, replica, (nt0 + j) * 16 + 4 * g, r16, s1, s2);
    }
  } else if (a.stats != nullptr) {
#pragma unroll
    for (int j = 0; j < NT; ++j)
      write_tile_stats(a.stats, tile, a.CoutS, (nt0 + j) * 16 + 4 * g, r16, (float)((TH - oy) * (TW - ox)), ssum[j],
                       ssq[j]);
  }
  if (stamp) {
    __builtin_amdgcn_s_waitcnt(0);
    const unsigned long long t_end = __builtin_amdgcn_s_memtime();
    unsigned long long* o = a.stamps + ((size_t)(blockIdx.z * gridDim.y + blockIdx.y) * gridDim.x + blockIdx.x) * 4;
    o[0] = t_store - t_begin; o[1] = t_k0 - t_store; o[2] = t_k1 - t_k0; o[3] = t_end - t_k1;
// ... 204 lines not shown
  } else if (mode == 8) {
    if constexpr (KC == 16 && TH == 14 && NT == 1 && NW == 1)
      SPCL_LAUNCH((conv3x3_fast_kernel<KC, TH, NT, 8, NW>), grid, block, lds, st, b);
  } else if (mode == 1 && a.in_bn.acc != nullptr) {
    if constexpr (KC == 64) {
      const int tpc = 64 * NW / a.CinK;
      if (tpc == 4) SPCL_LAUNCH((conv3x3_fast_kernel<KC, TH, NT, 5, NW>), grid, block, lds, st, b);
      else if (tpc == 2) SPCL_LAUNCH((conv3x3_fast_kernel<KC, TH, NT, 6, NW>), grid, block, lds, st, b);
      else SPCL_LAUNCH((conv3x3_fast_kernel<KC, TH, NT, 7, NW>), grid, block, lds, st, b);
    }
  } else if (mode == 1) SPCL_LAUNCH((conv3x3_fast_kernel<KC, TH, NT, 1, NW>), grid, block, lds, st, b);
  else if (a.rows2 != nullptr && a.H2 > 0) SPCL_LAUNCH((conv3x3_fast_kernel<KC, TH, NT, 3, NW>), grid, block, lds, st, b);
  else if (a.rows2 != nullptr) SPCL_LAUNCH((conv3x3_fast_kernel<KC, TH, NT, 2, NW>), grid, block, lds, st, b);
  else SPCL_LAUNCH((conv3x3_fast_kernel<KC, TH, NT, 0, NW>), grid, block, lds, st, b);
  if (b.stamps != nullptr) {
    std::vector<unsigned long long> h(nwg * 4);
    (void)hipStreamSynchronize(st);
    (void)hipMemcpy(h.data(), b.stamps, h.size() * 8, hipMemcpyDeviceToHost);
    (void)hipFree(b.stamps);
    double s4[4] = {0, 0, 0, 0};
    for (size_t i = 0; i < nwg; ++i)
      for (int k = 0; k < 4; ++k) s4[k] += (double)h[i * 4 + k];
    fprintf(stderr, "[conv_fast stamps] <%d,%d,%d,m%d,%d> %dx%d CinK %d CoutS %d wgs %zu | s_memtime ticks per wg: setup + first "
            "halo + LDS store %.0f, barrier %.0f, k-loops (all slabs) %.0f, epilogue %.0f\n", KC, TH, NT,
            mode == 1 ? 1 : (a.rows2 ? (a.H2 > 0 ? 3 : 2) : 0), NW, a.H, a.W, a.CinK, a.CoutS, nwg, s4[0] / nwg, s4[1] / nwg,
            s4[2] / nwg, s4[3] / nwg);
  }
}

bool launch_conv_fast(const ConvArgs& c, int th, hipStream_t st, bool dry) {
  if (c.H < th || c.W < 14) return false;
  if (c.in_mode == 2) {
    if (c.CinS != 1 || c.CoutS != 16 || th != 14) return false;
    FastArgs a;
    if (c.x2 != nullptr) return false;
    if (c.y_hi != nullptr) return false;
    if (c.x_up2) return false;
    a.x = (const unsigned char*)c.x; a.x2 = nullptr; a.y = (unsigned char*)c.y; a.y_hi = nullptr; a.wp = (const u32x4*)c.wp; a.stats = c.stats;
    a.up2 = 0;
    a.in_scale = a.in_shift = nullptr;
    a.y2 = nullptr; a.scale2 = a.shift2 = a.mean2 = nullptr; a.rows2 = nullptr; a.H2 = a.W2 = 0; a.img2 = nullptr;
    a.N = c.N; a.H = c.H; a.W = c.W; a.CinK = 16; a.CoutS = 16;
    static const int env_img_remap = lab_env("SPCL_IMAGE_XCD_REMAP", 1);
    a.tilesX = cdiv(c.W, 14); a.tilesY = cdiv(c.H, 14); a.gy = 1; a.xcd_remap = env_img_remap; a.lds_flip = 0; a.stamps = nullptr;
    a.acorr_rows = c.acorr_rows;
    a.img1 = nullptr; a.wp1 = nullptr; a.ipw = 1;
    a.stats_acc = a.rows2_acc = nullptr;
    a.in_bn = BnAccFwd{};
    if (c.stats_acc != nullptr || c.rows2_acc != nullptr || c.in_bn != nullptr) return false;
    if (c.acorr_rows != nullptr && !(c.H % 14 == 0 && c.W % 14 == 0)) return false;
    if (c.y == nullptr && !dry && c.acorr_rows == nullptr) return false;
    if (!dry) {
      if (c.acorr_rows != nullptr && c.y == nullptr) {
        a.ipw = (int)(((long)a.tilesX * a.tilesY * a.N + 4095) / 4096);
        a.ipw = a.ipw < 1 ? 1 : (a.ipw > a.N ? a.N : a.ipw);
        SPCL_LAUNCH((conv3x3_image_kernel<14, true, true, false>), dim3(a.tilesX, a.tilesY, cdiv(a.N, a.ipw)), dim3(64), 0, st, a);
      }
      else if (c.acorr_rows != nullptr) SPCL_LAUNCH((conv3x3_image_kernel<14, true, true>), dim3(a.tilesX, a.tilesY, a.N), dim3(64), 0, st, a);
      else if (c.H % 14 == 0 && c.W % 14 == 0) SPCL_LAUNCH((conv3x3_image_kernel<14, true>), dim3(a.tilesX, a.tilesY, a.N), dim3(64), 0, st, a);
      else SPCL_LAUNCH((conv3x3_image_kernel<14, false>), dim3(a.tilesX, a.tilesY, a.N), dim3(64), 0, st, a);
    }
    return true;
  }
  if (c.CinS != c.CinK) return false;
  const bool wants_acc = c.stats_acc != nullptr || c.rows2_acc != nullptr || c.in_bn != nullptr;
  const int ntn = c.CoutS / 16, KC = conv_kc(c.CinK);
  static const int env_nt1 = lab_env("SPCL_CONV_FAST_NT1", 0);
  int NT = ntn >= 2 ? 2 : 1;
  if (env_nt1 == 1 && KC == 64 && ntn == 2) NT = 1;
  if (env_nt1 != 2 && KC == 64 && ntn == 2 && c.rows2 != nullptr && c.H2 > 0) NT = 1;
  if (env_nt1 != 2 && KC == 64 && ntn == 2) NT = 1;
  if (KC == 64 && ntn == 4 && env_nt1 != 3 && (c.in_mode == 1 || c.H <= 28)) NT = 1;
  static const int env_wide = lab_env("SPCL_CONV_FAST_NT1_WIDE", 1);
  if (env_wide && KC == 64 && ntn == 4 && c.CinK > 64) NT = 1;
  static const int env_all4 = lab_env("SPCL_CONV_FAST_NT1_64", 1);
  if (env_all4 && KC == 64 && ntn == 4) NT = 1;
  static const int env_fill = lab_env("SPCL_CONV_FAST_FILL", 1);
  static const int env_fill_max = lab_env("SPCL_CONV_FAST_FILL_MAX", 512);
  if (env_fill && KC == 64 && NT == 2 && ntn >= 8 && ntn % 4 == 0 &&
      (long)c.N * cdiv(c.W, 14) * cdiv(c.H, th) * cdiv(ntn, 8) < env_fill_max)
    NT = 1;
  static const int env_narrow = lab_env("SPCL_CONV_FAST_NARROW_NT1", 2);
  if (env_narrow == 1 && KC < 64 && ntn == 2 && th == 7) NT = 1;
  if (env_narrow == 2 && KC == 32 && ntn == 2 && th == 7 && c.rows2 != nullptr && c.H2 == 0 && c.img2 == nullptr) NT = 1;
  int nw = ntn / NT;
  if (nw > 4) nw = 4;
  if (ntn % (NT * nw) != 0) return false;
  FastArgs a;
  a.x = (const unsigned char*)c.x; a.y = (unsigned char*)c.y; a.wp = (const u32x4*)c.wp; a.stats = c.stats;
  a.x2 = (const unsigned char*)c.x2;
  a.y_hi = (unsigned char*)c.y_hi;
  a.up2 = c.x_up2 ? 1 : 0;
  if (c.x_up2 && !(c.in_mode == 0 && c.x2 == nullptr && c.rows2 == nullptr && c.img2 == nullptr && c.H % 2 == 0 &&
                   c.W % 2 == 0 && (double)c.N * c.H * c.W / 4.0 * c.CinK * 2.0 < 2147483648.0))
    return false;
  if (c.y_hi != nullptr && !(c.in_mode == 0 && (c.rows2 == nullptr || c.H2 == 0) && c.img2 == nullptr && c.stats == nullptr &&
                             ntn % 2 == 0))
    return false;
  if (c.x2 != nullptr && !(((c.CinK == KC && KC >= 32) || (KC == 64 && (c.CinK / 64) % 2 == 0)) && c.rows2 == nullptr &&
                           c.img2 == nullptr))
    return false;
  if (c.x2 != nullptr && c.in_mode == 1 && c.CinK != KC) return false;
  a.in_scale = c.in_scale; a.in_shift = c.in_shift;
  a.y2 = (const unsigned char*)c.y2; a.scale2 = c.scale2; a.shift2 = c.shift2; a.mean2 = c.mean2; a.rows2 = c.rows2;
  a.H2 = c.H2; a.W2 = c.W2;
  a.img2 = c.img2;
  a.acorr_rows = nullptr;
  a.img1 = c.img1; a.wp1 = (const u32x4*)c.wp1; a.ipw = 1;
  if (c.img1 != nullptr && !(c.in_mode == 1 && KC == 16 && th == 14 && ntn == 1 && c.x2 == nullptr && c.y_hi == nullptr &&
                             !c.x_up2 && c.rows2 == nullptr && c.img2 == nullptr && !wants_acc && c.H % 14 == 0 && c.W % 14 == 0 &&
                             (dry || (c.wp1 != nullptr && c.in_scale != nullptr && c.in_shift != nullptr))))
    return false;
  a.stats_acc = c.stats_acc;
  a.rows2_acc = c.rows2_acc;
  a.in_bn = c.in_bn != nullptr ? *c.in_bn : BnAccFwd{};
  if (wants_acc) {
    const long tiles = (long)c.N * cdiv(c.W, 14) * cdiv(c.H, th);
    if (c.y_hi != nullptr || c.img2 != nullptr) return false;
    if (c.stats_acc != nullptr && (c.rows2 != nullptr || tiles > BN_ACC_MAX_TILES_FWD)) return false;
    if (c.rows2_acc != nullptr && (c.rows2 == nullptr || tiles > BN_ACC_MAX_TILES_BWD)) return false;
    if (c.in_bn != nullptr && !(c.in_mode == 1 && KC == 64 && c.x2 == nullptr && c.in_bn->CS == c.CinK &&
                                (c.CinK * 4 == 64 * nw || c.CinK * 2 == 64 * nw || c.CinK == 64 * nw)))
      return false;
  }
  if (c.rows2 != nullptr && c.in_mode != 0) return false;
  if (c.img2 != nullptr && !(c.rows2 != nullptr && c.H2 == 0 && KC == 16 && th == 14 && ntn == 1)) return false;
  a.N = c.N; a.H = c.H; a.W = c.W; a.CinK = c.CinK; a.CoutS = c.CoutS;
  a.tilesX = cdiv(c.W, 14); a.tilesY = cdiv(c.H, th); a.gy = ntn / (NT * nw);
  static const int env_remap = lab_env("SPCL_CONV_XCD_REMAP", 1);
  a.xcd_remap = (env_remap && a.gy == 1) ? 1 : 0;
  if (c.rows2 != nullptr && c.H2 > 0 && KC == 64 && nw == 1) return false;
#define SPCL_FAST_CASE(KC_, TH_, NT_, NW_)                               \
  if (KC == KC_ && th == TH_ && NT == NT_ && nw == NW_) {                \
    if (!dry) launch_fast<KC_, TH_, NT_, NW_>(a, c.img1 != nullptr ? 8 : c.in_mode, st); \
    return true;                                                         \
  }
  SPCL_FAST_CASE(16, 14, 1, 1)
  SPCL_FAST_CASE(16, 14, 2, 1)
  SPCL_FAST_CASE(32, 14, 1, 1)
  SPCL_FAST_CASE(16, 7, 2, 1)
  SPCL_FAST_CASE(16, 7, 1, 2)
  SPCL_FAST_CASE(32, 7, 1, 2)
  SPCL_FAST_CASE(32, 7, 1, 1)
  SPCL_FAST_CASE(32, 7, 2, 1)
  SPCL_FAST_CASE(32, 7, 2, 2)
  SPCL_FAST_CASE(64, 7, 2, 1)
  SPCL_FAST_CASE(64, 7, 1, 2)
  SPCL_FAST_CASE(64, 7, 2, 2)
  SPCL_FAST_CASE(64, 7, 1, 4)
  SPCL_FAST_CASE(64, 7, 2, 4)
#undef SPCL_FAST_CASE
  return false;
}

}
```

### self-paced-contrastive-learning_amd/functional.py

```python
from __future__ import annotations

import ctypes
import math
import os
from ctypes import c_double, c_float, c_int

import torch

from . import native as _n

SP_NONE, SP_HARD, SP_SOFT = 0, 1, 2


def take_grad_sink(param, needed: bool = True):
    if not needed or param is None:
        return None
    sink = getattr(param, "_grad_sink", None)
    if sink is None or not getattr(param, "_grad_sink_armed", False):
        return None
    if sink.shape != param.shape or sink.dtype != torch.float32 or not sink.is_contiguous() or sink.device != param.device:
        return None
    param._grad_sink_armed = False
    return sink

# ... 683 lines not shown
                _n.ptr(dpre), _n.stream())
        wgrad(dpre, M, x, xdt, cs, hid, C, dw1, db1)
        gfeat = None
        if ng[0]:
            dfeat = (torch.zeros if cs != C else torch.empty)(N, H, W, cs, dtype=xdt, device=dev)
            _n.call("spcl_rows_linear_backward_input", _n.ptr(dpre), _n.dtype_code(dpre.dtype), _n.ptr(w1c), None, M, hid, C,
                    _n.ptr(dfeat), _n.dtype_code(xdt), cs, _n.stream())
            gfeat = nhwc_to_logical(dfeat, C)
            if gfeat.dtype != fdt:
                gfeat = gfeat.to(fdt)
        return gfeat, dw1.view(ctx.params[0].shape), db1, dw2.view(ctx.params[2].shape), db2, None


def pixelwise_mlp_pooled_supported(feat, w1, w2) -> bool:
    return bool(feat.is_cuda and w2 is not None and feat.shape[1] % 4 == 0 and w1.shape[0] % 4 == 0 and w2.shape[0] % 4 == 0)


def pixelwise_mlp_pooled(feat, w1, b1, w2, b2, out_hw):
    return _PixelMlpPooledFn.apply(feat, w1, b1, w2, b2, tuple(int(v) for v in out_hw))


def pixelwise_mlp(feat, w1, b1, w2=None, b2=None):
    dims = [feat.shape[1], w1.shape[0]] + ([w2.shape[0]] if w2 is not None else [])
    if feat.is_cuda and all(d % 4 == 0 for d in dims):
        return _PixelMlpFn.apply(feat, w1, b1, w2, b2)
    xs, cs = as_nhwc(feat)
    N, H, W, _ = xs.shape
    C = feat.shape[1]
    rows = torch.as_strided(xs, (N * H * W, C, 1, 1), (cs, 1, cs, cs), xs.storage_offset())
    o = projector(rows, w1.reshape(w1.shape[0], -1), b1, None if w2 is None else w2.reshape(w2.shape[0], -1), b2,
                  normalize=False)
    return o.view(N, H, W, o.shape[1]).permute(0, 3, 1, 2)


def _ru16(c: int) -> int:
    return (c + 15) // 16 * 16


def to_nhwc_padded(x: torch.Tensor, dtype: torch.dtype):
    N, C, H, W = x.shape
    cs = _ru16(C)
    if x.dtype == dtype and cs == C:
        sN, sC, sH, sW = x.stride()
        if sC == 1 and sW == cs and sH == W * cs and sN == H * W * cs:
            return x.permute(0, 2, 3, 1)
    if cs == C:
        return x.to(dtype).contiguous(memory_format=torch.channels_last).permute(0, 2, 3, 1)
    out = torch.zeros(N, H, W, cs, dtype=dtype, device=x.device)
    out[..., :C] = x.permute(0, 2, 3, 1)
    return out


def nhwc_channel_slice(x, dtype):
    if x is None or x.dim() != 4 or x.dtype != dtype:
        return None
    N, C, H, W = x.shape
    sN, sC, sH, sW = x.stride()
    if sC != 1 or sW <= C or sW % 8 or C % 16 or sH != W * sW or sN != H * W * sW:
        return None
    if (x.storage_offset() * x.element_size()) % 16:
        return None
    return x.permute(0, 2, 3, 1), sW


def _bnrelu_fwd(y, dt_code, N, H, W, cs, scale, shift, act, pool):
    if act is not None and act.stride(2) != cs:
        _n.call("spcl_bnrelu_pool_forward_strided", _n.ptr(y), dt_code, N, H, W, cs, _n.ptr(scale), _n.ptr(shift),
                _n.ptr(act), int(act.stride(2)), _n.ptr(pool), _n.stream())
    else:
        _n.call("spcl_bnrelu_pool_forward", _n.ptr(y), dt_code, N, H, W, cs, _n.ptr(scale), _n.ptr(shift), _n.ptr(act),
                _n.ptr(pool), _n.stream())


def _act_buffer(cfg, N, H, W, cs, dtype, dev):
    dst = getattr(cfg, "act_dst", None)
    if (dst is not None and tuple(dst.shape) == (N, H, W, cs) and dst.dtype == dtype and dst.device == dev
            and dst.stride(3) == 1 and dst.stride(2) % 8 == 0 and dst.stride(1) == W * dst.stride(2)
            and dst.stride(0) == H * W * dst.stride(2) and (dst.storage_offset() * dst.element_size()) % 16 == 0):
        return dst
    return torch.empty(N, H, W, cs, dtype=dtype, device=dev)


class PoolLink:
    __slots__ = ("yb", "stb", "N", "H", "W", "cout_s", "rows", "dx_ptr", "holder", "version", "acc")

    def __init__(self, yb, stb, N, H, W, cout_s, acc=None):
        self.yb, self.stb, self.N, self.H, self.W, self.cout_s = yb, stb, N, H, W, cout_s
        self.acc = acc
        self.rows, self.dx_ptr, self.holder, self.version = None, 0, None, 0

    def fresh(self, ptr):
        return self.rows is not None and ptr == self.dx_ptr and self.holder is not None and self.holder._version == self.version


class ActLink:
    __slots__ = ("yb", "stb", "N", "H", "W", "C", "cs", "rows", "dx_ptr", "holder", "version")

    def __init__(self, yb, stb, N, H, W, C, cs):
        self.yb, self.stb, self.N, self.H, self.W, self.C, self.cs = yb, stb, N, H, W, C, cs
        self.rows, self.dx_ptr, self.holder, self.version = None, 0, None, 0

    fresh = PoolLink.fresh


class UpLink:
    __slots__ = ("d_up", "dx_ptr", "holder", "version")

    def __init__(self):
        self.d_up, self.dx_ptr, self.holder, self.version = None, 0, None, 0


class BlockCfg:
    __slots__ = ("dtype", "training", "momentum", "eps", "track", "need_act", "need_pool", "image_input", "buffers",
                 "link_in", "link_out", "act_dst", "up2", "lazy_act", "link_act", "x2_link", "bn_link", "x2_bn", "up_in", "up_link",
                 "gap", "want_gap")

    def __init__(self, dtype, training, momentum, eps, track, need_act, need_pool, image_input, buffers):
        self.dtype, self.training, self.momentum, self.eps, self.track = dtype, training, momentum, eps, track
        self.need_act, self.need_pool, self.image_input, self.buffers = need_act, need_pool, image_input, buffers
        self.link_in = None
        self.link_out = None
        self.act_dst = None
        self.lazy_act = False
        self.link_act = None
        self.x2_link = None
        self.up_in = False
        self.up_link = None
        self.bn_link = None
        self.x2_bn = None
        self.gap = None
        self.want_gap = False
        self.up2 = False


def _pack(w, kind, dt_code, dtype):
    co, ci = w.shape[0], w.shape[1]
    n = _n.call("spcl_conv_packed_elems", ci, co, kind, dt_code)
    buf = torch.empty(n, dtype=dtype, device=w.device)
    wc = w.detach().contiguous().float()
    _n.call("spcl_conv_pack_weights", _n.ptr(wc), ci, co, kind, dt_code, _n.ptr(buf), _n.stream())
    return buf


def _pack_both(w, dt_code, dtype):
    co, ci = w.shape[0], w.shape[1]
    n0 = _n.call("spcl_conv_packed_elems", ci, co, 0, dt_code)
    n1 = _n.call("spcl_conv_packed_elems", ci, co, 1, dt_code)
    buf = torch.empty(n0 + n1, dtype=dtype, device=w.device)
    wc = w.detach().contiguous().float()
    p0, p1 = buf[:n0], buf[n0:]
    _n.call("spcl_conv_pack_weights_both", _n.ptr(wc), ci, co, dt_code, _n.ptr(p0), _n.ptr(p1), _n.stream())
    return p0, p1


def _pack_block(wa, wb, dt_code, dtype, H=0, W=0):
    sizes = []
    for w in (wa, wb):
        co, ci = w.shape[0], w.shape[1]
        sizes += [_n.call("spcl_conv_packed_elems", ci, co, 0, dt_code), _n.call("spcl_conv_packed_elems", ci, co, 1, dt_code)]
    buf = torch.empty(sum(sizes), dtype=dtype, device=wa.device)
    parts, off = [], 0
    for n_ in sizes:
        parts.append(buf[off:off + n_])
        off += n_
    wac, wbc = wa.detach().contiguous().float(), wb.detach().contiguous().float()
    _n.call("spcl_conv_pack_weights_block_at", _n.ptr(wac), wa.shape[1], wa.shape[0], _n.ptr(parts[0]), _n.ptr(parts[1]),
            _n.ptr(wbc), wb.shape[1], wb.shape[0], _n.ptr(parts[2]), _n.ptr(parts[3]), dt_code, int(H), int(W), _n.stream())
    return (parts[0], parts[1]), (parts[2], parts[3])


_PREPACKED = {}
_PREPACK = os.environ.get("SPCL_PREPACK", "1") != "0"


_PREPACKED_ACORR = {}


def take_prepacked_acorr(image):
    return _PREPACKED_ACORR.pop((image.data_ptr(), image._version), None)


_EVAL_AFFINE = {}


def clear_prepacked():
    _PREPACKED.clear()
    _PREPACKED_ACORR.clear()
    _EVAL_AFFINE.clear()


def prepare_eval_affines(bns):
    _EVAL_AFFINE.clear()
    bns = [bn for bn in bns if bn.running_mean is not None and bn.running_mean.is_cuda and bn.weight is not None]
    for i in range(0, len(bns), _n.BN_EVAL_MAX):
        part = bns[i:i + _n.BN_EVAL_MAX]
        dev = part[0].running_mean.device
        sizes = [_ru16(bn.num_features) for bn in part]
        buf = torch.empty(4 * sum(sizes), dtype=torch.float32, device=dev)
        items, keep, off = [], [], 0
        for bn, cs in zip(part, sizes):
            g, b = bn.weight.detach().contiguous().float(), bn.bias.detach().contiguous().float()
            st = buf[off:off + 4 * cs].view(4, cs)
            off += 4 * cs
            items.append(_n.BnEvalItem(g.data_ptr(), b.data_ptr(), bn.running_mean.data_ptr(), bn.running_var.data_ptr(),
                                       st.data_ptr(), bn.num_features, cs, float(bn.eps)))
            keep.append((g, b))
            _EVAL_AFFINE[(bn.running_mean.data_ptr(), cs)] = st
        arr = (_n.BnEvalItem * len(items))(*items)
        _n.call("spcl_bn_eval_affine_multi", arr, len(items), _n.stream())


def prepack_weights(layers, dtype, image=None):
    _PREPACKED.clear()
    _PREPACKED_ACORR.clear()
# ... 586 lines not shown
            xl = getattr(cfg, "x2_link", None)
            if xl is not None:
                assert xl.yb.data_ptr() == x2s.data_ptr() and xl.cs == chalf, "x2 is not the linked producer's output"
            ctx.x2_coef = (xl.stb[2], xl.stb[3]) if xl is not None else (None, None)
        elif cfg.image_input:
            if cin > 16:
                raise NotImplementedError("image-input block supports input_dim <= 16")
            xs = x.detach().float().permute(0, 2, 3, 1).contiguous()
            cin_s, cin_k, mode_a = cin, 16, 2
        else:
            xs = to_nhwc_padded(x.detach(), dtype)
            cin_s = cin_k = xs.shape[3]
            mode_a = 0
        need_bwd = any(ctx.needs_input_grad)
        ctx.acorr = None
        acorr_rows = 0
        if (need_bwd and ctx.needs_input_grad[1] and not ctx.needs_input_grad[0]
                and _image3_supported(cfg, cin, dtc, N, H, W, cout_s)):
            ctx.acorr = take_prepacked_acorr(xs)
            acorr_rows = _acorr_in_conv_rows(dtc, N, H, W, cin, cout_s) if (ctx.acorr is None and x2s is None) else 0
            if ctx.acorr is None and acorr_rows == 0:
                ctx.acorr = _image_autocorr(xs, N, H, W)
        pre_a, pre_b = take_prepacked(wa, dtc, H, W), take_prepacked(wb, dtc, H, W)
        if pre_a is not None and pre_b is not None:
            (wpa, wpa_t), (wpb, wpb_t) = pre_a, pre_b
        elif need_bwd:
            (wpa, wpa_t), (wpb, wpb_t) = _pack_block(wa, wb, dtc, dtype, *((H, W) if _PACK_AT else (0, 0)))
        else:
            wpa, wpb, wpa_t, wpb_t = _pack(wa, 0, dtc, dtype), _pack(wb, 0, dtc, dtype), None, None
        ctx.up2 = bool(getattr(cfg, "up2", False)) and cfg.need_act and not cfg.need_pool
        lazy = (bool(getattr(cfg, "lazy_act", False)) and cfg.need_act and not cfg.need_pool and not ctx.up2
                and getattr(cfg, "act_dst", None) is None)
        count = float(N) * H * W
        acc_ok = _BN_ACC and cfg.training and dtype == torch.bfloat16 and cout_s <= 256 and cout == cout_s
        sup = lambda ci, co, kind, out: bool(_n.call("spcl_conv_bn_acc_supported", dtc, N, H, W, ci, co, kind, out))
        use_a = (acc_ok and x2s is None and acorr_rows == 0 and mode_a == 0 and sup(cin_k, cout_s, 0, 1)
                 and sup(cout_s, cout_s, 1, 0))
        use_b = (acc_ok and not lazy and not ctx.up2 and getattr(cfg, "act_dst", None) is None
                 and sup(cout_s, cout_s, 1 if use_a else 2, 1))
        keep = []
        recompute = False
        ctx.acc_bwd_a = ctx.acc_bwd_b = ctx.acc_rows_a = None
        if use_a:
            acc_a = bn_acc_block(cout_s, dev)
            ya, _ = _conv_acc(xs, dtc, dtype, N, H, W, cin_k, cout_s, wpa, None, None, None, acc_a, False)
            sta = torch.empty(4, cout_s, dtype=torch.float32, device=dev)
            bn_a = _bn_acc_desc(acc_a, cfg, cout, cout_s, ga, ba, 0, count, sta, keep)
        else:
            if x2s is not None:
                ya, sa = _conv_cat(xs, x2s, dtc, dtype, N, H, W, chalf, cout_s, wpa, cfg.training, *ctx.x2_coef)
            elif acorr_rows > 0:
                recompute = (_BLOCK1_RECOMPUTE and _CONV16_FUSED and cfg.training and not use_b and cin == 1
                             and cout == cout_s and ctx.needs_input_grad[4]
                             and bool(_n.call("spcl_block1_recompute_supported", dtc, N, H, W, cin_s, cout_s)))
                ya, sa, ctx.acorr = _conv_image_acorr(xs, dtc, dtype, N, H, W, cin_s, cout_s, wpa, cfg.training, acorr_rows,
                                                      store=not recompute)
            else:
                ya, sa = _conv(xs, dtc, dtype, N, H, W, cin_s, cin_k, cout_s, wpa, mode_a, None, None, cfg.training)
            sta = _bn_stats(sa, cfg, cout, cout_s, ga, ba, 0, dev)
        if use_a or use_b:
            acc_b = bn_acc_block(cout_s, dev) if use_b else None
            yb, sb = _conv_acc(ya, dtc, dtype, N, H, W, cout_s, cout_s, wpb, bn_a if use_a else None,
                               None if use_a else sta[2], None if use_a else sta[3], acc_b, cfg.training)
        elif recompute:
            yb, sb = _conv_from_image(xs, None, dtc, dtype, N, H, W, cout_s, wpa, sta[2], sta[3], wpb, cfg.training)
        else:
            yb, sb = _conv(ya, dtc, dtype, N, H, W, cout_s, cout_s, cout_s, wpb, 1, sta[2], sta[3], cfg.training)
        ctx.wpa_fwd = wpa if recompute else None
        if use_b:
            stb = torch.empty(4, cout_s, dtype=torch.float32, device=dev)
            bn_b = _bn_acc_desc(acc_b, cfg, cout, cout_s, gb, bb, 1, count, stb, keep)
        else:
            stb = _bn_stats(sb, cfg, cout, cout_s, gb, bb, 1, dev)
        if acc_ok and any(ctx.needs_input_grad):
            if not cfg.image_input and _n.call("spcl_conv_dgrad_bnstats_acc_supported", dtc, N, H, W, cout_s, cout_s):
                ctx.acc_bwd_a = bn_acc_block(cout_s, dev)
            elif not cfg.image_input and _ACC_FILL:
                ctx.acc_rows_a = bn_acc_block(cout_s, dev)
            ctx.acc_bwd_b = bn_acc_block(cout_s, dev)
        cfg.gap = None
        want_gap = (_GAP and getattr(cfg, "want_gap", False) and cfg.need_act and not cfg.need_pool and not lazy
                    and not ctx.up2 and cfg.act_dst is None
                    and H * W <= 1024 and _n.call("spcl_bnrelu_gap_supported", dtc, H, W, cout, cout_s))
        if want_gap:
            act, pool = torch.empty(N, H, W, cout_s, dtype=dtype, device=dev), None
            cfg.gap = torch.empty(N, cout, dtype=torch.float32, device=dev)
            _n.call("spcl_bnrelu_gap_forward", _n.ptr(yb), dtc, N, H, W, cout, cout_s, None if use_b else _n.ptr(stb[2]),
                    None if use_b else _n.ptr(stb[3]), ctypes.byref(bn_b) if use_b else None, _n.ptr(act), _n.ptr(cfg.gap),
                    _n.stream())
        elif use_b:
            act = torch.empty(N, H, W, cout_s, dtype=dtype, device=dev) if cfg.need_act else None
            pool = torch.empty(N, H // 2, W // 2, cout_s, dtype=dtype, device=dev) if cfg.need_pool else None
            _n.call("spcl_bnrelu_pool_forward_acc", _n.ptr(yb), dtc, N, H, W, cout_s, ctypes.byref(bn_b), _n.ptr(act),
                    _n.ptr(pool), _n.stream())
        elif lazy:
            act, pool = yb, None
            cfg.link_act = ActLink(yb, stb, N, H, W, cout, cout_s)
        elif ctx.up2:
            act = torch.empty(N, 2 * H, 2 * W, cout_s, dtype=dtype, device=dev)
            pool = None
            _n.call("spcl_bnrelu_up2_forward", _n.ptr(yb), dtc, N, H, W, cout_s, _n.ptr(stb[2]), _n.ptr(stb[3]), _n.ptr(act),
                    _n.stream())
        else:
            act = _act_buffer(cfg, N, H, W, cout_s, dtype, dev) if cfg.need_act else None
            pool = torch.empty(N, H // 2, W // 2, cout_s, dtype=dtype, device=dev) if cfg.need_pool else None
            _bnrelu_fwd(yb, dtc, N, H, W, cout_s, stb[2], stb[3], act, pool)
        ctx.save_for_backward(xs, ya, yb, sta, stb, wa, wb)
        ctx.x2s = x2s
        ctx.params = (wa, ga, ba, wb, gb, bb)
        ctx.packed_t = (wpa_t, wpb_t)
        ctx.cfg = cfg
        if need_bwd and pool is not None and act is None and cfg.training and dtype == torch.bfloat16:
            cfg.link_out = PoolLink(yb, stb, N, H, W, cout_s, ctx.acc_bwd_b)
        ctx.meta = (N, cin, H, W, cout, cout_s, cin_s, cin_k, mode_a, x.dtype)
        outs = []
        outs.append(nhwc_to_logical(act, cout) if act is not None else None)
        outs.append(nhwc_to_logical(pool, cout) if pool is not None else None)
        return tuple(outs)

    @staticmethod
    def backward(ctx, d_act, d_pool):
        xs, ya, yb, sta, stb, wa, wb = ctx.saved_tensors
        cfg = ctx.cfg
        N, cin, H, W, cout, cout_s, cin_s, cin_k, mode_a, xdt = ctx.meta
        dtype = cfg.dtype
        dtc = _n.dtype_code(dtype)
        g_nc = broadcast_rows(d_act, dtype) if (_BCAST and d_pool is None and d_act is not None and not ctx.up2
                                                  and d_act.shape[1] == cout_s) else None
        d_up = None
        ul = getattr(cfg, "up_link", None)
        if ul is not None and ul.d_up is not None:
            du, holder = ul.d_up, ul.holder
            same = (d_act is not None and d_pool is None and d_act.data_ptr() == ul.dx_ptr and d_act.dtype == holder.dtype
                    and holder._version == ul.version and nhwc_channel_slice(d_act, dtype) is None
                    and to_nhwc_padded(d_act, dtype).data_ptr() == ul.dx_ptr)
            dirty = holder._version != ul.version
            ul.d_up, ul.dx_ptr, ul.holder = None, 0, None
            if same:
                d_up, d_act = du, None
            else:
                gs = torch.empty(N, H, W, cout_s, dtype=dtype, device=du.device)
                _n.call("spcl_upsample2x_backward", _n.ptr(du), _n.ptr(gs), dtc, N, H, W, cout_s, _n.stream())
                gl = nhwc_to_logical(gs, cout)
                d_act = gl if d_act is None else d_act.to(gl.dtype) + gl
                if dirty:
                    holder.zero_()
        elif ctx.up2 and d_act is not None:
            du = to_nhwc_padded(d_act, dtype)
            if _UP2_BWD_FUSED and d_pool is None:
                d_up, d_act = du, None
            else:
                dsum = torch.empty(N, H, W, cout_s, dtype=dtype, device=du.device)
                _n.call("spcl_upsample2x_backward", _n.ptr(du), _n.ptr(dsum), dtc, N, H, W, cout_s, _n.stream())
                d_act = nhwc_to_logical(dsum, cout)
        da_stride = 0
        da_sl = nhwc_channel_slice(d_act, dtype) if (d_act is not None and g_nc is None) else None
        if da_sl is not None:
            da_s, da_stride = da_sl
        else:
            da_s = to_nhwc_padded(d_act, dtype) if (d_act is not None and g_nc is None) else None
        dp_s = to_nhwc_padded(d_pool, dtype) if d_pool is not None else None
        if da_s is None and dp_s is None and g_nc is None and d_up is None:
            return (None,) * 9
        x2s = ctx.x2s
        ng = ctx.needs_input_grad
        sk = tuple(take_grad_sink(p, ng[i + 1]) for i, p in enumerate(ctx.params))
        lk = cfg.link_out
        la = getattr(cfg, "link_act", None)
        if la is not None and da_s is not None and dp_s is None and da_stride == 0 and la.fresh(da_s.data_ptr()):
            dyb, dgb, dbb = _bnrelu_bwd_rows(yb, da_s, None, la.rows, dtc, dtype, N, H, W, cout, cout_s, stb, cfg.training,
                                             sk[4:6])
        elif g_nc is not None:
            acc = _take_acc(ctx, "acc_bwd_b")
            if acc is not None:
                dyb, dgb, dbb = _bnrelu_bwd_acc(yb, None, None, g_nc, dtc, dtype, N, H, W, cout, cout_s, stb, cfg.training,
                                                sk[4:6], acc)
            else:
                dyb, dgb, dbb = _bnrelu_bwd_bcast(yb, g_nc, dtc, dtype, N, H, W, cout, cout_s, stb, cfg.training, sk[4:6])
        elif lk is not None and da_s is None and dp_s is not None and lk.fresh(dp_s.data_ptr()):
            if lk.rows is ACC_ROWS:
                dyb, dgb, dbb = _bnrelu_bwd_acc(yb, None, dp_s, None, dtc, dtype, N, H, W, cout, cout_s, stb, cfg.training,
                                                sk[4:6], _take_acc(ctx, "acc_bwd_b"))
            else:
                acc = _take_acc(ctx, "acc_bwd_b") if (_ACC_FILL and H % 2 == 0 and W % 2 == 0 and cout_s <= 256) else None
                if acc is not None:
                    dyb, dgb, dbb = _bnrelu_bwd_rows_acc(yb, None, dp_s, lk.rows, dtc, dtype, N, H, W, cout, cout_s, stb,
                                                         cfg.training, sk[4:6], acc)
                else:
                    dyb, dgb, dbb = _bnrelu_pool_bwd_rows(yb, dp_s, lk.rows, dtc, dtype, N, H, W, cout, cout_s, stb,
                                                          cfg.training, sk[4:6])
        else:
            acc = _take_acc(ctx, "acc_bwd_b") if _ACC_FILL else None
            if acc is not None and lk is not None and lk.rows is ACC_ROWS:
                acc = None
            if acc is not None:
                dyb, dgb, dbb = _bnrelu_bwd_fill(yb, da_s, dp_s, dtc, dtype, N, H, W, cout, cout_s, stb, cfg.training, sk[4:6],
                                                 acc, dact_stride=da_stride, d_up=d_up)
            else:
                dyb, dgb, dbb = _bnrelu_bwd(yb, da_s, dp_s, dtc, dtype, N, H, W, cout, cout_s, stb, cfg.training, sk[4:6],
                                            dact_stride=da_stride, d_up=d_up)
        if lk is not None:
            lk.rows, lk.dx_ptr, lk.holder = None, 0, None
        if la is not None:
            la.rows, la.dx_ptr, la.holder = None, 0, None
        wpa_t, wpb_t = ctx.packed_t
        if wpb_t is None:
            wpb_t = _pack(wb, 1, dtc, dtype)
        image3 = ctx.acorr is not None
        one_pass = (image3 and (_CONV16_FUSED or ya is None) and ctx.needs_input_grad[4] and cout == cout_s
                    and _n.call("spcl_conv16_bwd_fused_supported", dtc, N, H, W, cout_s, cout_s))
        if ya is None and not one_pass:
            raise RuntimeError("image block backward: the first convolution's output was not stored and the one-pass kernel "
                               "that forms it again is not available")
        if one_pass:
            dwb, rows16 = _conv16_bwd_fused(dyb, wpb_t, ya, sta, xs, dtc, N, H, W, cout, cout, cout_s, sk[3],
                                            acorr=ctx.acorr if _CONV16_WGROWS else None, wp_image=ctx.wpa_fwd)
        else:
            dwb = _wgrad(ya, dyb, dtc, N, H, W, cout, cout_s, cout_s, cout, cout_s, 1, sta[2], sta[3], sk[3]) \
                if ctx.needs_input_grad[4] else None
        if one_pass:
            fused = (None, rows16)
        elif image3:
            fused = _dgrad_bnstats_image(dyb, wpb_t, ya, sta, xs, dtc, dtype, N, H, W, cout_s)
        else:
            acc = _take_acc(ctx, "acc_bwd_a")
            if acc is not None:
                fused = (_dgrad_bnstats_acc(dyb, wpb_t, ya, sta, dtc, dtype, N, H, W, cout_s, cout_s, acc), (ACC_ROWS, acc))
            else:
                fused = _dgrad_bnstats(dyb, wpb_t, ya, sta, dtc, dtype, N, H, W, cout_s, cout_s) \
                    if dtype == torch.bfloat16 else None
        if fused is not None:
            daa, rows = fused
        else:
            daa, _ = _conv(dyb, dtc, dtype, N, H, W, cout_s, cout_s, cout_s, wpb_t, 0, None, None, False)
        image_fused = ctx.needs_input_grad[1] and not ctx.needs_input_grad[0] and _image_wgrad_fusable(cfg, cin, cout_s)
        if image3:
            dya = None
            dwa, dga, dba = _bnrelu_bwd_rows_image3(rows, ctx.acorr, wa, N, H, W, cout, cout_s, sta, cfg.training, sk[0:3])
        elif image_fused:
            dya = None
            if fused is not None:
                dwa, dga, dba = _bnrelu_bwd_rows(ya, daa, xs, rows, dtc, dtype, N, H, W, cout, cout_s, sta, cfg.training,
                                                 sk[0:3])
            else:
                dwa, dga, dba = _bnrelu_bwd_image_wgrad(ya, daa, xs, dtc, N, H, W, cout, cout_s, sta, cfg.training,
                                                        sk[0:3])
        else:
            if fused is not None and isinstance(rows, tuple) and rows[0] is ACC_ROWS:
                dya, dga, dba = _bnrelu_bwd_acc(ya, daa, None, None, dtc, dtype, N, H, W, cout, cout_s, sta, cfg.training,
                                                sk[1:3], rows[1])
            elif fused is not None:
                acc = _take_acc(ctx, "acc_rows_a")
                if acc is not None:
                    dya, dga, dba = _bnrelu_bwd_rows_acc(ya, daa, None, rows, dtc, dtype, N, H, W, cout, cout_s, sta,
                                                         cfg.training, sk[1:3], acc)
                else:
                    dya, dga, dba = _bnrelu_bwd_rows(ya, daa, None, rows, dtc, dtype, N, H, W, cout, cout_s, sta,
                                                     cfg.training, sk[1:3])
            else:
                dya, dga, dba = _bnrelu_bwd(ya, daa, None, dtc, dtype, N, H, W, cout, cout_s, sta, cfg.training,
                                            sk[1:3])
            if not ctx.needs_input_grad[1]:
                dwa = None
            elif x2s is not None:
                dwa = _wgrad_cat(xs, x2s, dya, dtc, N, H, W, cin // 2, cout, cout_s, sk[0], *ctx.x2_coef)
            else:
                dwa = _wgrad(xs, dya, dtc, N, H, W, cin, cin_s, cin_k, cout, cout_s, mode_a, None, None, sk[0])
        dx = dx2 = None
        if ctx.needs_input_grad[0] or (x2s is not None and ctx.needs_input_grad[8]):
            if cfg.image_input:
                raise NotImplementedError("gradient w.r.t. the input image is not on the hot path")
            if wpa_t is None:
                wpa_t = _pack(wa, 1, dtc, dtype)
            li = cfg.link_in
            dxs = None
            if (li is not None and dtype == torch.bfloat16 and li.cout_s == cin_s and li.N == N
                    and _n.call("spcl_conv_dgrad_poolstats_supported", dtc, N, H, W, cout_s, cin_s, li.H, li.W)):
                dxs = torch.empty(N, H, W, cin_s, dtype=dtype, device=dya.device)
                if (li.acc is not None and _n.call("spcl_conv_dgrad_poolstats_acc_supported", dtc, N, H, W, cout_s, cin_s,
                                                   li.H, li.W)):
                    acc_in, li.acc = li.acc, None
                    _n.call("spcl_conv3x3_dgrad_poolstats_acc", _n.ptr(dya), dtc, N, H, W, cout_s, cin_s, _n.ptr(wpa_t),
                            _n.ptr(dxs), _n.ptr(li.yb), li.H, li.W, _n.ptr(li.stb[2]), _n.ptr(li.stb[3]), _n.ptr(li.stb[0]),
                            _n.ptr(acc_in), _n.stream())
                    rows = ACC_ROWS
                else:
                    nt = _n.call("spcl_conv_stat_rows", dtc, N, H, W, cout_s, cin_s)
                    rows = torch.empty(nt * 2 * cin_s, dtype=torch.float32, device=dya.device)
                    _n.call("spcl_conv3x3_dgrad_poolstats", _n.ptr(dya), dtc, N, H, W, cout_s, cin_s, _n.ptr(wpa_t),
                            _n.ptr(dxs), _n.ptr(li.yb), li.H, li.W, _n.ptr(li.stb[2]), _n.ptr(li.stb[3]), _n.ptr(li.stb[0]),
                            _n.ptr(rows), _n.stream())
                    rows.ntiles = nt
                li.rows, li.dx_ptr, li.holder, li.version = rows, dxs.data_ptr(), dxs, dxs._version
            split = None
            if (dxs is None and x2s is not None and _CONV_SPLIT
                    and _n.call("spcl_conv_split_supported", dtc, N, H, W, cout_s, cin_s)):
                split = (torch.empty(N, H, W, cin_s // 2, dtype=dtype, device=dya.device),
                         torch.empty(N, H, W, cin_s // 2, dtype=dtype, device=dya.device))
                xb = getattr(cfg, "x2_bn", None)
                if (xb is not None and xb.cs == cin_s // 2 and (xb.N, xb.H, xb.W) == (N, H, W) and cfg.training
                        and _n.call("spcl_conv_split_bnstats_supported", dtc, N, H, W, cout_s, cin_s)):
                    nt = _n.call("spcl_conv_stat_rows", dtc, N, H, W, cout_s, cin_s)
                    rows = torch.empty(nt * 2 * (cin_s // 2), dtype=torch.float32, device=dya.device)
                    rows.ntiles = nt
                    _n.call("spcl_conv3x3_dgrad_split_bnstats", _n.ptr(dya), dtc, N, H, W, cout_s, cin_s, _n.ptr(wpa_t),
                            _n.ptr(split[0]), _n.ptr(split[1]), _n.ptr(xb.yb), _n.ptr(xb.stb[2]), _n.ptr(xb.stb[3]),
                            _n.ptr(xb.stb[0]), _n.ptr(rows), _n.stream())
                    xb.rows, xb.dx_ptr, xb.holder, xb.version = rows, split[1].data_ptr(), split[1], split[1]._version
                else:
                    _n.call("spcl_conv3x3_forward_split", _n.ptr(dya), dtc, N, H, W, cout_s, cin_s, _n.ptr(wpa_t),
                            _n.ptr(split[0]), _n.ptr(split[1]), _n.stream())
            elif dxs is None:
                dxs, _ = _conv(dya, dtc, dtype, N, H, W, cout_s, cout_s, cin_s, wpa_t, 0, None, None, False)
            if x2s is not None:
                if split is not None:
                    dx, dx2 = nhwc_to_logical(split[0], cin // 2), nhwc_to_logical(split[1], cin // 2)
                else:
                    full = dxs.permute(0, 3, 1, 2)
                    dx, dx2 = full[:, :cin // 2], full[:, cin // 2:]
                if dx.dtype != xdt:
                    dx, dx2 = dx.to(xdt), dx2.to(xdt)
                if not ctx.needs_input_grad[0]:
                    dx = None
                if not ctx.needs_input_grad[8]:
                    dx2 = None
            else:
                dx = nhwc_to_logical(dxs, cin)
                if dx.dtype != xdt:
                    dx = dx.to(xdt)
        ng = ctx.needs_input_grad
        return (dx, dwa, dga if ng[2] else None, dba if ng[3] else None, dwb, dgb if ng[5] else None,
                dbb if ng[6] else None, None, dx2)


def conv_block(x, wa, ga, ba, wb, gb, bb, cfg: BlockCfg, x2=None):
    act, pool = _ConvBlockFn.apply(x, wa, ga, ba, wb, gb, bb, cfg, x2)
    gap = getattr(cfg, "gap", None)
    if gap is not None and act is not None:
        act._spcl_gap = (gap, act._version)
        cfg.gap = None
    return act, pool


def _gap_of(feat, N, C):
    gap = getattr(feat, "_spcl_gap", None)
    if (gap is None or gap[1] != feat._version or tuple(gap[0].shape) != (N, C) or gap[0].device != feat.device
            or tuple(feat.shape[:2]) != (N, C)):
        return None
    return gap[0]


def cat_pair_shape_ok(N, C, H, W, cout, dtype):
    return bool(_CONV_CAT and dtype == torch.bfloat16
                and _n.call("spcl_conv_cat_supported", _n.dtype_code(dtype), N, H, W, C, _ru16(cout)))


def cat_pair_supported(a, b, cout, dtype):
    if not (_CONV_CAT and a.is_cuda and b.is_cuda and a.shape == b.shape and a.dim() == 4 and dtype == torch.bfloat16
            and a.dtype == dtype and b.dtype == dtype):
        return False
    N, C, H, W = a.shape
    for t in (a, b):
        st, cs = as_nhwc(t)
        if cs != C or (st.data_ptr() % 16):
            return False
    return bool(_n.call("spcl_conv_cat_supported", _n.dtype_code(dtype), N, H, W, C, _ru16(cout)))


class _ConvBNReLUFn(torch.autograd.Function):

    @staticmethod
    def forward(ctx, x, w, gamma, beta, cfg: BlockCfg):
        _n.require_gpu(x, w)
        dtype, dev = cfg.dtype, x.device
        dtc = _n.dtype_code(dtype)
        N, cin, H, W = x.shape
        up_in = bool(getattr(cfg, "up_in", False))
        if up_in:
            H, W = 2 * H, 2 * W
        cout = w.shape[0]
        cout_s = _ru16(cout)
        xs = to_nhwc_padded(x.detach(), dtype)
        cin_s = xs.shape[3]
        need_bwd = any(ctx.needs_input_grad)
        pre = take_prepacked(w, dtc, H, W)
        if pre is not None:
            wp, wp_t = pre
        elif need_bwd:
            wp, wp_t = _pack_both(w, dtc, dtype)
        else:
            wp, wp_t = _pack(w, 0, dtc, dtype), None
        if up_in:
            assert cin_s == cin, "the in-place upsample needs an unpadded channel count"
            y = torch.empty(N, H, W, cout_s, dtype=dtype, device=dev)
            s = None
            if cfg.training:
                nt = _n.call("spcl_conv_stat_rows", dtc, N, H, W, cin_s, cout_s)
                s = torch.empty(_n.call("spcl_bn_stats_elems", nt, cout_s), dtype=torch.float32, device=dev)
                s.ntiles = nt
            _n.call("spcl_conv3x3_forward_up2", _n.ptr(xs), dtc, N, H, W, cin_s, cout_s, _n.ptr(wp), _n.ptr(y), _n.ptr(s),
                    _n.stream())
        else:
            y, s = _conv(xs, dtc, dtype, N, H, W, cin_s, cin_s, cout_s, wp, 0, None, None, cfg.training)
        st = _bn_stats(s, cfg, cout, cout_s, gamma, beta, 0, dev)
        if bool(getattr(cfg, "lazy_act", False)) and getattr(cfg, "act_dst", None) is None and cout == cout_s:
            act = y
            cfg.link_act = ActLink(y, st, N, H, W, cout, cout_s)
        else:
            act = _act_buffer(cfg, N, H, W, cout_s, dtype, dev)
            _bnrelu_fwd(y, dtc, N, H, W, cout_s, st[2], st[3], act, None)
        ctx.save_for_backward(xs, y, st, w)
        ctx.params = (w, gamma, beta)
        ctx.packed_t = wp_t
        ctx.cfg = cfg
        ctx.acc_bwd = (bn_acc_block(cout_s, dev) if (_BN_ACC and _ACC_FILL and need_bwd and cfg.training and cout_s <= 256
                                                     and dtype == torch.bfloat16) else None)
        cfg.bn_link = ActLink(y, st, N, H, W, cout, cout_s) if (need_bwd and cout == cout_s) else None
        ctx.meta = (N, cin, H, W, cout, cout_s, cin_s, x.dtype)
# ... 1283 lines not shown
```

### self-paced-contrastive-learning_amd/native.py

```python
from __future__ import annotations

import ctypes
import os
from ctypes import c_char_p, c_double, c_float, c_int, c_long, c_size_t, c_void_p

import torch

HERE = os.path.dirname(os.path.abspath(__file__))
LIB_PATH = os.path.join(HERE, "lib", "libspcl_hip.so")
SPCL_F32, SPCL_BF16 = 0, 1

_lib = None

_P = c_void_p
_SIGNATURES = {
    "spcl_abi_version": (c_int, []),
    "spcl_last_error": (c_char_p, []),
    "spcl_supcon_workspace_bytes": (c_size_t, [c_int, c_int]),
    "spcl_supcon_forward": (c_int, [_P, _P, _P, _P, c_int, c_int, c_float, c_int, c_float, c_int, _P, _P, _P]),
    "spcl_supcon_backward": (c_int, [_P, _P, c_int, c_int, c_float, c_int, c_float, _P, _P, _P, _P, _P, _P, _P]),
    "spcl_supcon_bwd_workspace_bytes": (c_size_t, [c_int, c_int]),
    "spcl_supcon_unit_gradient_block": (c_int, [c_int, c_int, _P, _P]),
    "spcl_supcon_materialize": (c_int, [_P, _P, c_int, c_int, c_float, c_int, c_float, _P, _P, _P, _P, _P, _P, _P]),
    "spcl_supcon_xpos_workspace_bytes": (c_size_t, [c_int, c_int]),
# ... 107 lines not shown
                                      _P, _P, c_int, _P, _P]),
    "spcl_bnrelu_backward_wgrows_image3": (c_int, [_P, c_int, _P, c_int, _P, c_int, c_int, c_int, c_int, c_int, _P, _P, _P,
                                                   c_int, _P, _P, _P, _P, _P]),
    "spcl_conv3x3_dgrad_bnstats_image": (c_int, [_P, c_int, c_int, c_int, c_int, c_int, c_int, _P, _P, _P, _P, _P, _P, _P,
                                                 _P, _P]),
    "spcl_bnrelu_image3_workspace_bytes": (c_size_t, [c_int]),
    "spcl_bnrelu_backward_rows_image3": (c_int, [_P, c_int, _P, c_int, _P, c_int, c_int, c_int, c_int, c_int, _P, _P, _P,
                                                 c_int, _P, _P, _P, _P, _P]),
    "spcl_conv1x1_forward": (c_int, [_P, c_int, c_size_t, c_int, c_int, c_int, _P, _P, _P, _P]),
    "spcl_conv1x1_bwd_workspace_bytes": (c_size_t, [c_int, c_int]),
    "spcl_conv1x1_backward": (c_int, [_P, _P, c_int, c_size_t, c_int, c_int, c_int, _P, _P, _P, _P, _P, _P]),
    "spcl_conv1x1_forward_bn": (c_int, [_P, c_int, c_size_t, c_int, c_int, c_int, _P, _P, _P, _P, _P, _P]),
    "spcl_conv1x1_bwd_rows": (c_int, [c_size_t]),
    "spcl_conv1x1_backward_bn": (c_int, [_P, _P, c_int, c_size_t, c_int, c_int, c_int, _P, _P, _P, _P, _P, _P, _P, _P, _P, _P]),
    "spcl_softmax_forward": (c_int, [_P, c_size_t, c_int, _P, _P]),
    "spcl_softmax_backward": (c_int, [_P, _P, c_size_t, c_int, _P, _P]),
    "spcl_kl_workspace_bytes": (c_size_t, []),
    "spcl_kl_div_forward": (c_int, [_P, _P, c_size_t, c_int, c_float, _P, _P, _P]),
    "spcl_kl_div_backward": (c_int, [_P, _P, c_size_t, c_int, c_float, _P, _P, _P]),
    "spcl_sup_loss_forward": (c_int, [_P, _P, c_int, c_int, c_int, c_float, _P, _P, _P, _P, _P, _P]),
    "spcl_one_hot": (c_int, [_P, c_size_t, c_int, _P, _P]),
    "spcl_argmax_classes": (c_int, [_P, c_size_t, c_int, _P, _P]),
    "spcl_dice_counts": (c_int, [_P, _P, c_int, c_int, c_int, _P, _P, _P]),
    "spcl_surface_workspace_bytes": (c_size_t, [c_int, c_int, c_int, c_int]),
    "spcl_surface_distances": (c_int, [_P, _P, c_int, c_int, c_int, c_int, _P, c_int, c_double, c_double, c_double, _P, _P, _P,
                                       _P, _P, c_size_t, _P]),
    "spcl_surface_3d_workspace_bytes": (c_size_t, [c_int, c_int, c_int, c_int, c_int]),
    "spcl_surface_distances_3d": (c_int, [_P, _P, c_int, c_int, c_int, c_int, c_int, _P, c_int, c_double, c_double, c_double,
                                          c_double, _P, _P, _P, _P, _P, c_size_t, _P]),
    "spcl_upsample2x_forward": (c_int, [_P, _P, c_int, c_int, c_int, c_int, c_int, _P]),
    "spcl_upsample2x_backward": (c_int, [_P, _P, c_int, c_int, c_int, c_int, c_int, _P]),
    "spcl_concat2_channels": (c_int, [_P, _P, _P, c_int, c_size_t, c_int, c_int, _P]),
    "spcl_split2_channels": (c_int, [_P, _P, _P, c_int, c_size_t, c_int, c_int, _P]),
    "spcl_augment_views": (c_int, [_P, c_int, c_int, c_int, _P, c_int, _P, c_int, c_int, _P]),
    "spcl_augment_views_recipe": (c_int, [_P, _P, c_int, c_int, c_int, _P, c_int, _P, _P, c_int, c_int, c_int, _P]),
    "spcl_augment_views_recipe_workspace_bytes": (c_size_t, [c_int, c_int, c_int]),
    "spcl_rows_linear_forward": (c_int, [_P, c_int, c_long, c_int, _P, _P, c_int, c_int, c_int, _P, _P]),
    "spcl_rows_linear_forward_act": (c_int, [_P, c_int, c_long, _P, _P, c_int, c_int, c_int, _P, c_int, _P]),
    "spcl_adaptive_avgpool2d_backward_act": (c_int, [_P, _P, c_int, c_int, c_int, c_int, c_int, c_int, c_int, _P, _P]),
    "spcl_rows_linear_backward_input": (c_int, [_P, c_int, _P, _P, c_int, c_int, c_int, _P, c_int, c_long, _P]),
    "spcl_rows_linear_backward_weight_workspace_bytes": (c_size_t, [c_int, c_int, c_int]),
    "spcl_rows_linear_backward_weight": (c_int, [_P, c_int, _P, c_int, c_long, c_int, c_int, c_int, c_int, _P, c_size_t, _P, _P, _P]),
    "spcl_augment_views_recipe_ws": (c_int, [_P, _P, c_int, c_int, c_int, _P, c_int, _P, _P, c_int, c_int, c_int, _P, c_size_t,
                                             _P]),
    "spcl_resize_bilinear_pil": (c_int, [_P, c_int, c_int, c_int, _P, _P, c_int, _P, _P, c_int, _P, _P, c_int, c_int, _P]),
    "spcl_augment_views_pil": (c_int, [_P, c_int, c_int, c_int, _P, c_int, _P, c_int, c_int, _P]),
    "spcl_flip_batch": (c_int, [_P, _P, c_int, c_int, c_int, c_int, c_int, _P, _P]),
    "spcl_flip_pair": (c_int, [_P, _P, _P, c_int, c_int, c_int, c_int, c_int, _P, _P]),
    "spcl_flip_pair_stage": (c_int, [_P, _P, _P, c_int, c_int, c_int, c_int, c_int, _P, _P, c_size_t, c_size_t, _P]),
    "spcl_profile_enable": (c_int, [c_int]),
    "spcl_profile_count": (c_int, []),
    "spcl_profile_get": (c_int, [c_int, c_char_p, c_int, _P, _P, _P]),
    "spcl_radam_step": (c_int, [_P, _P, _P, _P, c_size_t, _P, _P, c_double, c_double, c_double, c_double, _P, _P]),
    "spcl_radam_step_scalars": (c_int, [_P, _P, _P, _P, c_size_t, _P, _P, c_double, c_double, c_double, c_double, _P,
                                        c_int, _P, _P, _P, _P]),
    "spcl_radam_step_scaled": (c_int, [_P, _P, c_double, _P, _P, c_size_t, _P, _P, c_double, c_double, c_double, c_double,
                                       _P, c_int, _P, _P, _P, _P]),
    "spcl_bnrelu_gap_supported": (c_int, [c_int, c_int, c_int, c_int, c_int]),
    "spcl_bnrelu_gap_forward": (c_int, [_P, c_int, c_int, c_int, c_int, c_int, c_int, _P, _P, _P, _P, _P, _P]),
    "spcl_bnrelu_backward_fill_acc": (c_int, [_P, _P, c_int, _P, _P, c_int, c_int, c_int, c_int, c_int, c_int, _P, c_int, _P, _P,
                                              _P, _P, _P]),
    "spcl_copy_pair": (c_int, [_P, _P, c_size_t, _P, _P, c_size_t, _P]),
    "spcl_bnrelu_backward_rows_acc": (c_int, [_P, _P, _P, _P, c_int, c_int, c_int, c_int, c_int, c_int, c_int, _P, c_int, _P, _P,
                                              _P, _P, _P]),
    "spcl_radam_apply_staged": (c_int, [_P, _P, c_double, _P, _P, c_size_t, _P, _P, c_double, c_double, c_double, c_double,
                                        c_int, _P, _P, _P, _P]),
    "spcl_adam_step_scaled": (c_int, [_P, _P, c_double, _P, _P, c_size_t, _P, _P, c_double, c_double, c_double, c_double,
                                      c_int, _P, c_int, _P, _P, _P, _P]),
    "spcl_adam_apply_staged": (c_int, [_P, _P, c_double, _P, _P, c_size_t, _P, _P, c_double, c_double, c_double, c_double,
                                       c_int, c_int, _P, _P, _P, _P]),
    "spcl_sgd_step_scaled": (c_int, [_P, _P, c_double, _P, c_size_t, _P, _P, c_double, c_double, c_double, c_int, _P, c_int,
                                     _P, _P, _P, _P]),
    "spcl_sgd_apply_staged": (c_int, [_P, _P, c_double, _P, c_size_t, _P, _P, c_double, c_double, c_double, c_int, c_int, _P,
                                      _P, _P, _P]),
    "spcl_bn_acc_elems": (c_size_t, [c_int]),
    "spcl_conv_bn_acc_supported": (c_int, [c_int, c_int, c_int, c_int, c_int, c_int, c_int, c_int]),
    "spcl_conv3x3_forward_acc": (c_int, [_P, c_int, c_int, c_int, c_int, c_int, c_int, _P, _P, _P, _P, _P, _P, _P, _P]),
    "spcl_bnrelu_pool_forward_acc": (c_int, [_P, c_int, c_int, c_int, c_int, c_int, _P, _P, _P, _P]),
    "spcl_conv_dgrad_bnstats_acc_supported": (c_int, [c_int, c_int, c_int, c_int, c_int, c_int]),
    "spcl_conv3x3_dgrad_bnstats_acc": (c_int, [_P, c_int, c_int, c_int, c_int, c_int, c_int, _P, _P, _P, _P, _P, _P, _P, _P]),
    "spcl_conv_dgrad_poolstats_acc_supported": (c_int, [c_int, c_int, c_int, c_int, c_int, c_int, c_int, c_int]),
    "spcl_conv3x3_dgrad_poolstats_acc": (c_int, [_P, c_int, c_int, c_int, c_int, c_int, c_int, _P, _P, _P, c_int, c_int, _P,
                                                 _P, _P, _P, _P]),
    "spcl_bnrelu_backward_acc": (c_int, [_P, _P, _P, _P, c_int, c_int, c_int, c_int, c_int, c_int, _P, c_int, _P, _P, _P, _P,
                                         _P]),
    "spcl_iic_joint_workspace_bytes": (c_size_t, [c_int, c_int, c_int]),
    "spcl_iic_joint_forward": (c_int, [_P, _P, c_long, c_int, c_int, c_int, c_int, c_int, c_int, _P, _P, _P]),
    "spcl_iic_loss_workspace_bytes": (c_size_t, [c_int, c_int]),
    "spcl_iic_loss": (c_int, [_P, _P, c_int, c_int, c_int, c_int, c_float, _P, _P, _P, _P, _P, c_size_t, _P]),
    "spcl_iic_joint_backward": (c_int, [_P, _P, c_long, c_int, c_int, c_int, c_int, c_int, c_int, _P, _P, _P, _P, _P, _P]),
    "spcl_consistency_workspace_bytes": (c_size_t, [c_int, c_int, c_int]),
    "spcl_consistency_softmax_mse": (c_int, [_P, _P, c_int, c_int, c_int, c_int, _P, c_float, _P, _P, _P, c_size_t, _P]),
    "spcl_iic_patch_plan": (c_int, [c_int, c_int, c_int, c_int, c_int, c_int, _P, _P, _P]),
    "spcl_iic_patch_forward": (c_int, [_P, _P, c_int, c_int, c_int, c_int, c_int, c_int, _P, c_float, _P, _P, _P, _P, _P,
                                       c_size_t, _P]),
    "spcl_iic_patch_backward": (c_int, [_P, _P, c_int, c_int, c_int, c_int, c_int, c_int, _P, _P, _P, _P, _P, _P]),
    "spcl_ema_update": (c_int, [_P, _P, c_size_t, c_double, c_double, _P]),
    "spcl_mt_softmax_mse_workspace_bytes": (c_size_t, [c_int, c_int, c_int]),
    "spcl_mt_softmax_mse": (c_int, [_P, _P, c_int, c_int, c_int, c_int, _P, c_int, c_float, _P, _P, _P, c_size_t, _P]),
    "spcl_entropy_softmax_workspace_bytes": (c_size_t, [c_int, c_int, c_int]),
    "spcl_entropy_softmax": (c_int, [_P, c_int, c_int, c_int, c_int, c_float, c_float, _P, _P, _P, c_size_t, _P]),
    "spcl_ucmt_workspace_bytes": (c_size_t, [c_int, c_int, c_int]),
    "spcl_ucmt_softmax_mse": (c_int, [_P, _P, c_int, _P, c_int, c_int, c_int, c_int, _P, c_float, c_float, c_float, _P, _P, _P,
                                      _P, _P, c_size_t, _P]),
    "spcl_mixup_images": (c_int, [_P, _P, _P, c_int, c_size_t, c_float, c_float, _P, _P]),
    "spcl_mixup_kl_workspace_bytes": (c_size_t, [c_int, c_int, c_int]),
    "spcl_mixup_kl_onehot": (c_int, [_P, _P, _P, _P, c_int, c_int, c_int, c_int, c_float, c_float, c_float, c_float, _P, _P, _P,
                                     c_size_t, _P]),
    "spcl_patch4s2_rows_forward": (c_int, [_P, c_int, c_long, c_long, c_long, c_long, _P, c_int, c_long, c_long, c_long, c_long,
                                           c_int, c_int, c_int, c_int, _P, _P, _P, _P]),
    "spcl_patch4s2_rows_backward": (c_int, [_P, _P, c_int, c_int, c_int, c_int, c_int, c_int, _P, _P, _P, _P]),
    "spcl_rows_bn_workspace_bytes": (c_size_t, [c_int, c_int]),
    "spcl_rows_bn_forward": (c_int, [_P, c_int, c_int, _P, _P, c_float, c_float, _P, _P, _P, _P, c_size_t, _P]),
    "spcl_rows_bn_eval_affine": (c_int, [_P, _P, _P, _P, c_float, c_int, _P, _P]),
    "spcl_rows_bn_backward": (c_int, [_P, _P, c_int, c_int, _P, _P, c_int, _P, _P, _P, _P, c_size_t, _P]),
    "spcl_discr_head_workspace_bytes": (c_size_t, [c_int, c_int, c_int, c_int]),
    "spcl_discr_head_forward": (c_int, [_P, c_int, c_int, c_int, c_int, _P, _P, _P, c_int, _P, _P, _P, _P, _P, c_size_t, _P]),
    "spcl_discr_head_backward": (c_int, [_P, c_int, c_int, c_int, c_int, _P, _P, _P, _P, _P, _P, _P, _P, c_size_t, _P]),
    "spcl_mine_pairs_forward": (c_int, [_P, _P, c_int, c_int, c_int, c_int, c_int, _P, _P, _P]),
    "spcl_mine_pairs_backward": (c_int, [_P, _P, _P, c_int, c_int, c_int, c_int, c_int, _P, _P]),
    "spcl_mine_head_workspace_bytes": (c_size_t, [c_int, c_int, c_int, c_int]),
    "spcl_mine_head_forward": (c_int, [_P, _P, c_int, c_int, c_int, c_int, c_int, _P, _P, _P, _P, _P, _P, _P, c_size_t, _P]),
    "spcl_mine_head_backward": (c_int, [_P, _P, _P, _P, _P, c_int, c_int, c_int, c_int, c_int, _P, _P, _P, _P, _P]),
    "spcl_pica_workspace_bytes": (c_size_t, [c_int]),
    "spcl_pica_seg_loss": (c_int, [_P, _P, c_int, c_int, c_int, c_double, c_float, _P, _P, _P, _P, _P, c_size_t, _P]),
    "spcl_pica_global_loss": (c_int, [_P, _P, c_long, c_int, c_int, c_int, c_float, c_float, _P, _P, _P, _P, _P, _P, c_size_t,
                                      _P]),
}


class WgradItem(ctypes.Structure):
    _fields_ = [("x", c_void_p), ("dy", c_void_p), ("in_scale", c_void_p), ("in_shift", c_void_p),
                ("dw_oihw", c_void_p), ("N", c_int), ("H", c_int), ("W", c_int), ("Cin", c_int), ("CinS", c_int),
                ("Cout", c_int), ("CoutS", c_int), ("in_mode", c_int), ("x2", c_void_p), ("x_up2", c_int)]


class PackItem(ctypes.Structure):
    _fields_ = [("w_oihw", c_void_p), ("fwd", c_void_p), ("dgrad", c_void_p), ("Cin", c_int), ("Cout", c_int),
                ("H", c_int), ("W", c_int)]


BN_EVAL_MAX = 32


class BnEvalItem(ctypes.Structure):
    _fields_ = [("gamma", c_void_p), ("beta", c_void_p), ("running_mean", c_void_p), ("running_var", c_void_p),
                ("st", c_void_p), ("C", c_int), ("CS", c_int), ("eps", c_float)]


class BnAcc(ctypes.Structure):
    _fields_ = [("acc", c_void_p), ("gamma", c_void_p), ("beta", c_void_p), ("running_mean", c_void_p),
                ("running_var", c_void_p), ("num_batches_tracked", c_void_p), ("st", c_void_p), ("momentum", c_float),
                ("eps", c_float), ("count", c_float), ("C", c_int), ("CS", c_int)]


PACK_MULTI_MAX = 24


class WgradTail(ctypes.Structure):
    _fields_ = [("partial", c_void_p), ("dw", c_void_p), ("kind", c_int), ("nsplit", c_int), ("nblk_ci", c_int),
                ("nblk_co", c_int), ("CIB", c_int), ("COB", c_int), ("Cin", c_int), ("Cout", c_int)]


ABI_VERSION = 22
WGRAD_BATCH_MAX = 16
WGRAD_TAILS_MAX = 16
_NO_STATUS = ("spcl_abi_version", "spcl_block1_recompute_supported", "spcl_block1_kernels_take", "spcl_conv16_bwd_fused_image_supported", "spcl_conv3x3_forward_image_acorr_rows", "spcl_image_autocorr_rows", "spcl_conv_dgrad_bnstats_image_supported", "spcl_conv16_bwd_fused_supported", "spcl_conv16_bwd_fused_splits", "spcl_conv_num_tiles", "spcl_conv_stat_rows", "spcl_conv_set_gemm", "spcl_conv_set_f32_split", "spcl_conv_get_f32_split", "spcl_supcon_unit_gradient_block", "spcl_conv_cat_supported", "spcl_conv_up2_supported", "spcl_conv_split_supported", "spcl_conv_split_bnstats_supported", "spcl_conv1x1_bwd_rows", "spcl_profile_count", "spcl_conv_dgrad_bnstats_supported", "spcl_conv_dgrad_poolstats_supported",
              "spcl_conv_wgrad_batched_supported", "spcl_conv_bn_acc_supported", "spcl_conv_dgrad_bnstats_acc_supported",
              "spcl_conv_dgrad_poolstats_acc_supported", "spcl_supcon_rows_supported", "spcl_bnrelu_gap_supported")


class NativeLibraryError(RuntimeError):
    pass


def lib():
    global _lib
    if _lib is None:
        if not os.path.exists(LIB_PATH):
            raise NativeLibraryError(
                f"{LIB_PATH} is missing: build it with `python self-paced-contrastive-learning_amd/build.py` "
                "(there is no CPU / eager fallback for the hot path)")
        L = ctypes.CDLL(LIB_PATH)
        L.spcl_abi_version.restype, L.spcl_abi_version.argtypes = c_int, []
        have = L.spcl_abi_version()
        if have != ABI_VERSION:
            raise NativeLibraryError(
                f"{LIB_PATH} has C-ABI version {have}, this binding was written for {ABI_VERSION} (include/spcl_hip.h "
                "SPCL_ABI_VERSION): a stale build -- rebuild with `python self-paced-contrastive-learning_amd/build.py`")
        for name, (res, args) in _SIGNATURES.items():
            fn = getattr(L, name, None)
            if fn is None:
                continue
            fn.restype, fn.argtypes = res, args
        _lib = L
    return _lib


def call(name: str, *args):
    L = lib()
    fn = getattr(L, name, None)
    if fn is None:
        raise NativeLibraryError(f"libspcl_hip.so does not export {name}")
    rc = fn(*args)
    if fn.restype is c_int and name not in _NO_STATUS and rc != 0:
        raise RuntimeError(f"{name} failed ({rc}): {L.spcl_last_error().decode()}")
    return rc


def require_gpu(*tensors):
    for t in tensors:
        if t is None:
            continue
        if not t.is_cuda:
            raise RuntimeError("self-paced-contrastive-learning_amd runs on MI355X only: got a CPU tensor "
                               "(the HIP path has no CPU fallback)")


def ptr(t):
    return None if t is None else c_void_p(t.data_ptr())


def stream():
    return c_void_p(torch.cuda.current_stream().cuda_stream)


def ptr_array(tensors):
    return (c_void_p * len(tensors))(*[None if t is None else t.data_ptr() for t in tensors])


def dtype_code(dt: torch.dtype) -> int:
    if dt == torch.float32:
        return SPCL_F32
    if dt == torch.bfloat16:
        return SPCL_BF16
    raise TypeError(f"unsupported activation dtype {dt}")
```

Before: 31230 slices/s.

## Save pooled argmax pre-activation in forward to shrink pool-backward reads in dgrad

When a conv block max-pools its output, the forward BN+ReLU+pool kernel now also writes a quarter-size tensor holding the raw pre-BN value that won each 2x2 window (ymax). It can also skip writing the full-resolution activation. The next layer's dgrad kernel with fused pool/BN-stat backward reads this compact tensor instead of re-reading the full-resolution y and recomputing each window's max. This is meant to cut backward memory traffic at the cost of an extra forward write, an extra buffer kept alive, and lower occupancy in one kernel variant.

```diff
diff --git a/include/spcl_hip.h b/include/spcl_hip.h
--- a/include/spcl_hip.h
+++ b/include/spcl_hip.h
@@ -14,7 +14,7 @@
 #define SPCL_ELAUNCH (-2)
 #define SPCL_EUNSUPPORTED (-3)
 
-#define SPCL_ABI_VERSION 22
+#define SPCL_ABI_VERSION 23
 int spcl_abi_version(void);
 const char* spcl_last_error(void);
 
@@ -417,6 +417,17 @@
 int spcl_conv3x3_dgrad_poolstats_acc(const void* dy, int dtype, int N, int H, int W, int CinK, int CoutS, const void* w_packed,
                                      void* g, const void* y2, int H2, int W2, const float* scale2, const float* shift2,
                                      const float* mean2, long long* acc, void* stream);
+int spcl_bnrelu_pool_forward_ymax(const void* y, int dtype, int N, int H, int W, int CS, const float* scale,
+                                  const float* shift, const spcl_bn_acc* bn, void* act_out, void* pool_out, void* ymax_out,
+                                  void* stream);
+int spcl_conv_dgrad_poolmax_supported(int dtype, int N, int H, int W, int CinK, int CoutS);
+int spcl_conv3x3_dgrad_poolmax(const void* dy, int dtype, int N, int H, int W, int CinK, int CoutS, const void* w_packed,
+                               void* g, const void* ymax, const float* scale2, const float* shift2, const float* mean2,
+                               float* rows2, void* stream);
+int spcl_conv_dgrad_poolmax_acc_supported(int dtype, int N, int H, int W, int CinK, int CoutS);
+int spcl_conv3x3_dgrad_poolmax_acc(const void* dy, int dtype, int N, int H, int W, int CinK, int CoutS, const void* w_packed,
+                                   void* g, const void* ymax, const float* scale2, const float* shift2, const float* mean2,
+                                   long long* acc, void* stream);
 int spcl_bnrelu_backward_acc(const void* y, const void* dact, const void* dpool, const void* dact_nc, int dtype, int N, int H,
                              int W, int C, int CS, const float* st4, int training, long long* acc, float* dgamma, float* dbeta,
                              void* dy, void* stream);
diff --git a/self-paced-contrastive-learning_amd/csrc/bn.hip b/self-paced-contrastive-learning_amd/csrc/bn.hip
--- a/self-paced-contrastive-learning_amd/csrc/bn.hip
+++ b/self-paced-contrastive-learning_amd/csrc/bn.hip
@@ -226,6 +226,7 @@
   static constexpr int EPW = 1;
   static __device__ __forceinline__ float get(uint32_t w, int) { return __uint_as_float(w); }
   static __device__ __forceinline__ uint32_t make(const float* v) { return __float_as_uint(v[0]); }
+  static __device__ __forceinline__ uint32_t merge(const uint32_t* s) { return s[0]; }
 };
 template <> struct Word<bf16_t> {
   static constexpr int EPW = 2;
@@ -235,6 +236,7 @@
   static __device__ __forceinline__ uint32_t make(const float* v) {
     return (uint32_t)f32_to_bf16(v[0]) | ((uint32_t)f32_to_bf16(v[1]) << 16);
   }
+  static __device__ __forceinline__ uint32_t merge(const uint32_t* s) { return (s[0] & 0x0000ffffu) | (s[1] & 0xffff0000u); }
 };
 
 template <int EPC> __device__ __forceinline__ void load_coef(float* dst, const float* src, int cc) {
@@ -445,11 +447,12 @@
   }
 };
 
-template <typename T, bool FAST>
-__global__ __launch_bounds__(256, 4) void bnrelu_fwd_pool_kernel(const T* __restrict__ y, int N, int H, int W, int CS,
+template <typename T, bool FAST, bool YMAX = false, bool ACT = true>
+__global__ __launch_bounds__(256, (YMAX && ACT) ? 3 : 4) void bnrelu_fwd_pool_kernel(const T* __restrict__ y, int N, int H, int W, int CS,
                                                               const float* __restrict__ scale,
                                                               const float* __restrict__ shift, T* __restrict__ act,
-                                                              T* __restrict__ pool, int AS, BnAccFwd bn = BnAccFwd{}) {
+                                                              T* __restrict__ pool, int AS, BnAccFwd bn = BnAccFwd{},
+                                                              T* __restrict__ ymax = nullptr) {
   constexpr int EPC = Chunk<T>::EPC, EPW = Word<T>::EPW;
   const int CPC = CS / EPC, PL = 256 / CPC;
   const int cc = threadIdx.x % CPC, pl = threadIdx.x / CPC;
@@ -473,26 +476,34 @@
 #pragma unroll
       for (int u = 0; u < 2; ++u) {
         if (u == 1 && !second) break;
-        u32x4 mxw, aw[4];
+        u32x4 mxw, aw[4], ymw = {0u, 0u, 0u, 0u};
 #pragma unroll
         for (int wi = 0; wi < 4; ++wi) {
-          float mx[EPW], a[4][EPW];
+          float mx[EPW], a[4][EPW], zb[EPW];
+          uint32_t wb[EPW];
 #pragma unroll
           for (int h = 0; h < EPW; ++h) {
             const int e = wi * EPW + h;
             mx[h] = 0.f;
+            zb[h] = 0.f;
+            wb[h] = 0u;
 #pragma unroll
             for (int k = 0; k < 4; ++k) {
-              a[k][h] = fmaxf(fmaf(sc[e], Word<T>::get(w[u].ry[k][wi], h), sh[e]), 0.f);
+              const float z = fmaf(sc[e], Word<T>::get(w[u].ry[k][wi], h), sh[e]);
+              a[k][h] = fmaxf(z, 0.f);
               if (w[u].valid[k]) mx[h] = fmaxf(mx[h], a[k][h]);
+              if (YMAX) pool_first_max(k, z, w[u].ry[k][wi], zb[h], wb[h]);
             }
           }
           mxw[wi] = Word<T>::make(mx);
-#pragma unroll
-          for (int k = 0; k < 4; ++k) aw[k][wi] = Word<T>::make(a[k]);
+          if (YMAX) ymw[wi] = Word<T>::merge(wb);
+          if (ACT) {
+#pragma unroll
+            for (int k = 0; k < 4; ++k) aw[k][wi] = Word<T>::make(a[k]);
+          }
         }
         const int oxu = ox + u * PL;
-        if (act != nullptr) {
+        if (ACT && act != nullptr) {
           const size_t a00 = (row0 * W + 2 * oxu) * AS + cc * EPC;
           const size_t aoff[4] = {a00, a00 + AS, a00 + (size_t)W * AS, a00 + (size_t)W * AS + AS};
 #pragma unroll
@@ -501,6 +512,8 @@
         }
         if (pool != nullptr && (FAST || (oy < OH && oxu < OW)))
           *(u32x4*)(pool + (((size_t)n * OH + oy) * OW + oxu) * CS + cc * EPC) = mxw;
+        if (YMAX && (FAST || (oy < OH && oxu < OW)))
+          *(u32x4*)(ymax + (((size_t)n * OH + oy) * OW + oxu) * CS + cc * EPC) = ymw;
       }
     }
   }
@@ -844,8 +857,7 @@
 #pragma unroll
               for (int k = 0; k < 4; ++k) {
                 const float yv = Word<T>::get(w.ry[k][wi], h);
-                const float z = w.valid[k] ? fmaf(sc[e], yv, sh[e]) : -1.f;
-                if (k == 0 || z > zb) { zb = z; yb = yv; }
+                pool_first_max(k, w.valid[k] ? fmaf(sc[e], yv, sh[e]) : -1.f, yv, zb, yb);
               }
               const float dzb = (complete && zb > 0.f) ? Word<T>::get(rdp[wi], h) : 0.f;
               s1[e] += dzb;
@@ -1263,7 +1275,8 @@
 
 template <typename T>
 static int bnrelu_fwd_launch(const void* y, int N, int H, int W, int CS, const float* scale, const float* shift,
-                             void* act, void* pool, hipStream_t st, const BnAccFwd* bnp = nullptr) {
+                             void* act, void* pool, hipStream_t st, const BnAccFwd* bnp = nullptr,
+                             void* ymax = nullptr ) {
   constexpr int EPC = Chunk<T>::EPC;
   const BnAccFwd bn = bnp != nullptr ? *bnp : BnAccFwd{};
   static const int acc_wg = lab_env("SPCL_ACC_STREAM_WG", 768);
@@ -1271,15 +1284,29 @@
   const int PL = 256 / (CS / EPC);
   const int AS = tl_act_stride > 0 ? tl_act_stride : CS;
   const double tb = (double)N * H * W * CS * sizeof(T);
-  prof_cost(tb * (1.0 + (act != nullptr ? 1.0 : 0.0) + (pool != nullptr ? 0.25 : 0.0)), 0.0);
+  prof_cost(tb * (1.0 + (act != nullptr ? 1.0 : 0.0) + (pool != nullptr ? 0.25 : 0.0) + (ymax != nullptr ? 0.25 : 0.0)), 0.0);
   if (pool != nullptr) {
     const int rows = N * ((H + 1) / 2);
-    if (H % 2 == 0 && W % 2 == 0) {
-      SPCL_LAUNCH((bnrelu_fwd_pool_kernel<T, true>), dim3(rows < STREAM_MAX_WG ? rows : STREAM_MAX_WG), dim3(256), 0, st, (const T*)y, N, H,
-                       W, CS, scale, shift, (T*)act, (T*)pool, AS, bn);
+    const dim3 grid(rows < STREAM_MAX_WG ? rows : STREAM_MAX_WG);
+    const bool fast = H % 2 == 0 && W % 2 == 0;
+    if (ymax != nullptr && fast && act == nullptr) {
+      SPCL_LAUNCH((bnrelu_fwd_pool_kernel<T, true, true, false>), grid, dim3(256), 0, st, (const T*)y, N, H, W, CS, scale, shift,
+                  (T*)act, (T*)pool, AS, bn, (T*)ymax);
+    } else if (ymax != nullptr && fast) {
+      SPCL_LAUNCH((bnrelu_fwd_pool_kernel<T, true, true, true>), grid, dim3(256), 0, st, (const T*)y, N, H, W, CS, scale, shift,
+                  (T*)act, (T*)pool, AS, bn, (T*)ymax);
+    } else if (ymax != nullptr && act == nullptr) {
+      SPCL_LAUNCH((bnrelu_fwd_pool_kernel<T, false, true, false>), grid, dim3(256), 0, st, (const T*)y, N, H, W, CS, scale, shift,
+                  (T*)act, (T*)pool, AS, bn, (T*)ymax);
+    } else if (ymax != nullptr) {
+      SPCL_LAUNCH((bnrelu_fwd_pool_kernel<T, false, true, true>), grid, dim3(256), 0, st, (const T*)y, N, H, W, CS, scale, shift,
+                  (T*)act, (T*)pool, AS, bn, (T*)ymax);
+    } else if (fast) {
+      SPCL_LAUNCH((bnrelu_fwd_pool_kernel<T, true>), grid, dim3(256), 0, st, (const T*)y, N, H, W, CS, scale, shift, (T*)act,
+                  (T*)pool, AS, bn, (T*)nullptr);
     } else {
-      SPCL_LAUNCH((bnrelu_fwd_pool_kernel<T, false>), dim3(rows < STREAM_MAX_WG ? rows : STREAM_MAX_WG), dim3(256), 0, st, (const T*)y, N, H,
-                       W, CS, scale, shift, (T*)act, (T*)pool, AS, bn);
+      SPCL_LAUNCH((bnrelu_fwd_pool_kernel<T, false>), grid, dim3(256), 0, st, (const T*)y, N, H, W, CS, scale, shift, (T*)act,
+                  (T*)pool, AS, bn, (T*)nullptr);
     }
   } else {
     const size_t npix = (size_t)N * H * W;
@@ -1578,6 +1605,29 @@
   return SPCL_OK;
 }
 
+extern "C" int spcl_bnrelu_pool_forward_ymax(const void* y, int dtype, int N, int H, int W, int CS, const float* scale,
+                                             const float* shift, const spcl_bn_acc* bn, void* act_out, void* pool_out,
+                                             void* ymax_out, void* stream) {
+  SPCL_CHECK_ARG(y && pool_out && ymax_out && (bn || (scale && shift)), "bnrelu_pool_forward_ymax: null pointer");
+  SPCL_CHECK_ARG(N > 0 && H >= 2 && W >= 2 && CS > 0 && CS % 16 == 0 && CS <= (bn ? 256 : 1024),
+                 "bnrelu_pool_forward_ymax: bad shape (H, W >= 2; CS <= 256 with an accumulator block)");
+  SPCL_CHECK_ARG(dtype == SPCL_F32 || dtype == SPCL_BF16, "bnrelu_pool_forward_ymax: dtype");
+  BnAccFwd f{};
+  if (bn != nullptr) {
+    SPCL_CHECK_ARG(bn->acc && bn->gamma && bn->beta && bn->st && bn->CS == CS && bn->C > 0 && bn->C <= CS && bn->count >= 1.f,
+                   "bnrelu_pool_forward_ymax: bad accumulator description");
+    f = BnAccFwd{bn->acc, bn->gamma, bn->beta, bn->running_mean, bn->running_var, bn->num_batches_tracked, bn->st,
+                 bn->momentum, bn->eps, bn->count, bn->C, bn->CS, 1.0 / (double)bn->count};
+  }
+  hipStream_t st = (hipStream_t)stream;
+  if (dtype == SPCL_F32)
+    bnrelu_fwd_launch<float>(y, N, H, W, CS, scale, shift, act_out, pool_out, st, bn != nullptr ? &f : nullptr, ymax_out);
+  else
+    bnrelu_fwd_launch<bf16_t>(y, N, H, W, CS, scale, shift, act_out, pool_out, st, bn != nullptr ? &f : nullptr, ymax_out);
+  SPCL_LAUNCH_CHECK("bnrelu_pool_forward_ymax");
+  return SPCL_OK;
+}
+
 extern "C" int spcl_bnrelu_backward_acc(const void* y, const void* dact, const void* dpool, const void* dact_nc, int dtype,
                                         int N, int H, int W, int C, int CS, const float* st4, int training, long long* acc,
                                         float* dgamma, float* dbeta, void* dy, void* stream) {
diff --git a/self-paced-contrastive-learning_amd/csrc/common.hpp b/self-paced-contrastive-learning_amd/csrc/common.hpp
--- a/self-paced-contrastive-learning_amd/csrc/common.hpp
+++ b/self-paced-contrastive-learning_amd/csrc/common.hpp
@@ -75,6 +75,14 @@
 
 __device__ __forceinline__ int lane_id() { return threadIdx.x & 63; }
 
+template <typename Y>
+__device__ __forceinline__ void pool_first_max(int k, float z, Y y, float& zb, Y& yb) {
+  if (k == 0 || z > zb) {
+    zb = z;
+    yb = y;
+  }
+}
+
 __device__ __forceinline__ float wave_sum(float v) {
   v += __builtin_bit_cast(float, __builtin_amdgcn_update_dpp(0, __builtin_bit_cast(int, v), 0xB1, 0xF, 0xF, true));
   v += __builtin_bit_cast(float, __builtin_amdgcn_update_dpp(0, __builtin_bit_cast(int, v), 0x4E, 0xF, 0xF, true));
diff --git a/self-paced-contrastive-learning_amd/csrc/conv.hip b/self-paced-contrastive-learning_amd/csrc/conv.hip
--- a/self-paced-contrastive-learning_amd/csrc/conv.hip
+++ b/self-paced-contrastive-learning_amd/csrc/conv.hip
@@ -1575,3 +1575,66 @@
   SPCL_LAUNCH_CHECK("conv3x3_dgrad_poolstats");
   return SPCL_OK;
 }
+
+static bool dgrad_poolmax_dry(int dtype, int N, int H, int W, int CinK, int CoutS, bool acc) {
+  ConvArgs a;
+  if (!dgrad_bnstats_args(a, dtype, N, H, W, CinK, CoutS) || conv_use_gemm(CinK, CoutS, H, W)) return false;
+  a.x = nullptr; a.y = nullptr; a.wp = nullptr;
+  float dummy;
+  long long dummy2;
+  a.rows2 = &dummy;
+  a.rows2_acc = acc ? &dummy2 : nullptr;
+  a.y2_is_poolmax = true;
+  TileCfg t = pick_tile(H, W);
+  return t.tw == 14 && launch_conv_fast(a, t.th, nullptr, true);
+}
+
+extern "C" int spcl_conv_dgrad_poolmax_supported(int dtype, int N, int H, int W, int CinK, int CoutS) {
+  if (!spcl_conv_dgrad_poolstats_supported(dtype, N, H, W, CinK, CoutS, 2 * H, 2 * W)) return 0;
+  return dgrad_poolmax_dry(dtype, N, H, W, CinK, CoutS, false) ? 1 : 0;
+}
+
+extern "C" int spcl_conv_dgrad_poolmax_acc_supported(int dtype, int N, int H, int W, int CinK, int CoutS) {
+  if (!spcl_conv_dgrad_poolstats_acc_supported(dtype, N, H, W, CinK, CoutS, 2 * H, 2 * W)) return 0;
+  return dgrad_poolmax_dry(dtype, N, H, W, CinK, CoutS, true) ? 1 : 0;
+}
+
+static int dgrad_poolmax_impl(const void* dy, int dtype, int N, int H, int W, int CinK, int CoutS, const void* w_packed,
+                              void* g, const void* ymax, const float* scale2, const float* shift2, const float* mean2,
+                              float* rows2, long long* acc, void* stream) {
+  SPCL_CHECK_ARG(dy && w_packed && g && ymax && scale2 && shift2 && mean2, "conv3x3_dgrad_poolmax: null pointer");
+  ConvArgs a;
+  if (!dgrad_bnstats_args(a, dtype, N, H, W, CinK, CoutS) || conv_use_gemm(CinK, CoutS, H, W)) {
+    set_error("conv3x3_dgrad_poolmax: unsupported configuration");
+    return SPCL_EUNSUPPORTED;
+  }
+  a.x = dy; a.y = g; a.wp = w_packed;
+  a.y2 = ymax; a.scale2 = scale2; a.shift2 = shift2; a.mean2 = mean2;
+  a.rows2 = acc != nullptr ? (float*)acc : rows2;
+  a.rows2_acc = acc;
+  a.y2_is_poolmax = true;
+  hipStream_t st = (hipStream_t)stream;
+  const double px = (double)N * H * W;
+  prof_cost(px * (CinK + 2.0 * CoutS) * 2.0 + 9.0 * CinK * CoutS * 2.0, 2.0 * px * 9.0 * CinK * CoutS);
+  TileCfg t = pick_tile(H, W);
+  if (!(t.tw == 14 && launch_conv_fast(a, t.th, st))) {
+    set_error("conv3x3_dgrad_poolmax: no specialised kernel for H=%d W=%d CinK=%d CoutS=%d", H, W, CinK, CoutS);
+    return SPCL_EUNSUPPORTED;
+  }
+  SPCL_LAUNCH_CHECK("conv3x3_dgrad_poolmax");
+  return SPCL_OK;
+}
+
+extern "C" int spcl_conv3x3_dgrad_poolmax(const void* dy, int dtype, int N, int H, int W, int CinK, int CoutS,
+                                          const void* w_packed, void* g, const void* ymax, const float* scale2,
+                                          const float* shift2, const float* mean2, float* rows2, void* stream) {
+  SPCL_CHECK_ARG(rows2, "conv3x3_dgrad_poolmax: null pointer");
+  return dgrad_poolmax_impl(dy, dtype, N, H, W, CinK, CoutS, w_packed, g, ymax, scale2, shift2, mean2, rows2, nullptr, stream);
+}
+
+extern "C" int spcl_conv3x3_dgrad_poolmax_acc(const void* dy, int dtype, int N, int H, int W, int CinK, int CoutS,
+                                              const void* w_packed, void* g, const void* ymax, const float* scale2,
+                                              const float* shift2, const float* mean2, long long* acc, void* stream) {
+  SPCL_CHECK_ARG(acc, "conv3x3_dgrad_poolmax_acc: null pointer");
+  return dgrad_poolmax_impl(dy, dtype, N, H, W, CinK, CoutS, w_packed, g, ymax, scale2, shift2, mean2, nullptr, acc, stream);
+}
diff --git a/self-paced-contrastive-learning_amd/csrc/conv_common.hpp b/self-paced-contrastive-learning_amd/csrc/conv_common.hpp
--- a/self-paced-contrastive-learning_amd/csrc/conv_common.hpp
+++ b/self-paced-contrastive-learning_amd/csrc/conv_common.hpp
@@ -42,6 +42,7 @@
   const float* mean2 = nullptr;
   float* rows2 = nullptr;
   int H2 = 0, W2 = 0;
+  bool y2_is_poolmax = false;
   const float* img2 = nullptr;
   const void* x2 = nullptr;
   void* y_hi = nullptr;
diff --git a/self-paced-contrastive-learning_amd/csrc/conv_fast.hip b/self-paced-contrastive-learning_amd/csrc/conv_fast.hip
--- a/self-paced-contrastive-learning_amd/csrc/conv_fast.hip
+++ b/self-paced-contrastive-learning_amd/csrc/conv_fast.hip
@@ -664,11 +664,7 @@
             for (int k = 0; k < 4; ++k) {
               const uint32_t wd = r < 2 ? yr[k].x : yr[k].y;
               const float yv = (r & 1) ? __uint_as_float(wd & 0xffff0000u) : __uint_as_float(wd << 16);
-              const float z = fmaf(sc2[j][r], yv, sh2[j][r]);
-              if (k == 0 || z > zb) {
-                zb = z;
-                yb = yv;
-              }
+              pool_first_max(k, fmaf(sc2[j][r], yv, sh2[j][r]), yv, zb, yb);
             }
             const float dz = zb > 0.f ? gv[r] * keep : 0.f;
             ssum[j][r] += dz;
@@ -1039,7 +1035,8 @@
     NT = 1;
   static const int env_narrow = lab_env("SPCL_CONV_FAST_NARROW_NT1", 2);
   if (env_narrow == 1 && KC < 64 && ntn == 2 && th == 7) NT = 1;
-  if (env_narrow == 2 && KC == 32 && ntn == 2 && th == 7 && c.rows2 != nullptr && c.H2 == 0 && c.img2 == nullptr) NT = 1;
+  if (env_narrow == 2 && KC == 32 && ntn == 2 && th == 7 && c.rows2 != nullptr && c.H2 == 0 && !c.y2_is_poolmax && c.img2 == nullptr)
+    NT = 1;
   int nw = ntn / NT;
   if (nw > 4) nw = 4;
   if (ntn % (NT * nw) != 0) return false;
diff --git a/self-paced-contrastive-learning_amd/functional.py b/self-paced-contrastive-learning_amd/functional.py
--- a/self-paced-contrastive-learning_amd/functional.py
+++ b/self-paced-contrastive-learning_amd/functional.py
@@ -789,15 +789,20 @@
 
 
 class PoolLink:
-    __slots__ = ("yb", "stb", "N", "H", "W", "cout_s", "rows", "dx_ptr", "holder", "version", "acc")
-
-    def __init__(self, yb, stb, N, H, W, cout_s, acc=None):
+    __slots__ = ("yb", "stb", "N", "H", "W", "cout_s", "rows", "dx_ptr", "holder", "version", "acc", "ymax")
+
+    def __init__(self, yb, stb, N, H, W, cout_s, acc=None, ymax=None):
         self.yb, self.stb, self.N, self.H, self.W, self.cout_s = yb, stb, N, H, W, cout_s
+        self.ymax = ymax
         self.acc = acc
         self.rows, self.dx_ptr, self.holder, self.version = None, 0, None, 0
 
     def fresh(self, ptr):
         return self.rows is not None and ptr == self.dx_ptr and self.holder is not None and self.holder._version == self.version
+
+
+def _pool_ymax_pays(N, H, W, cout_s):
+    return N * H * W * cout_s * 2 >= 12 * 2 ** 20
 
 
 class ActLink:
@@ -820,7 +825,7 @@
 class BlockCfg:
     __slots__ = ("dtype", "training", "momentum", "eps", "track", "need_act", "need_pool", "image_input", "buffers",
                  "link_in", "link_out", "act_dst", "up2", "lazy_act", "link_act", "x2_link", "bn_link", "x2_bn", "up_in", "up_link",
-                 "gap", "want_gap")
+                 "gap", "want_gap", "grad_mode")
 
     def __init__(self, dtype, training, momentum, eps, track, need_act, need_pool, image_input, buffers):
         self.dtype, self.training, self.momentum, self.eps, self.track = dtype, training, momentum, eps, track
@@ -837,6 +842,7 @@
         self.x2_bn = None
         self.gap = None
         self.want_gap = False
+        self.grad_mode = True
         self.up2 = False
 
 
@@ -1589,6 +1595,10 @@
         want_gap = (_GAP and getattr(cfg, "want_gap", False) and cfg.need_act and not cfg.need_pool and not lazy
                     and not ctx.up2 and cfg.act_dst is None
                     and H * W <= 1024 and _n.call("spcl_bnrelu_gap_supported", dtc, H, W, cout, cout_s))
+        offers_link = need_bwd and cfg.need_pool and not cfg.need_act and cfg.training and dtype == torch.bfloat16
+        want_ymax = (offers_link and cfg.grad_mode and not want_gap and not lazy and not ctx.up2 and H >= 2 and W >= 2
+                     and _pool_ymax_pays(N, H, W, cout_s))
+        ymax = None
         if want_gap:
             act, pool = torch.empty(N, H, W, cout_s, dtype=dtype, device=dev), None
             cfg.gap = torch.empty(N, cout, dtype=torch.float32, device=dev)
@@ -1598,8 +1608,13 @@
         elif use_b:
             act = torch.empty(N, H, W, cout_s, dtype=dtype, device=dev) if cfg.need_act else None
             pool = torch.empty(N, H // 2, W // 2, cout_s, dtype=dtype, device=dev) if cfg.need_pool else None
-            _n.call("spcl_bnrelu_pool_forward_acc", _n.ptr(yb), dtc, N, H, W, cout_s, ctypes.byref(bn_b), _n.ptr(act),
-                    _n.ptr(pool), _n.stream())
+            if want_ymax:
+                ymax = torch.empty_like(pool)
+                _n.call("spcl_bnrelu_pool_forward_ymax", _n.ptr(yb), dtc, N, H, W, cout_s, None, None, ctypes.byref(bn_b),
+                        None, _n.ptr(pool), _n.ptr(ymax), _n.stream())
+            else:
+                _n.call("spcl_bnrelu_pool_forward_acc", _n.ptr(yb), dtc, N, H, W, cout_s, ctypes.byref(bn_b), _n.ptr(act),
+                        _n.ptr(pool), _n.stream())
         elif lazy:
             act, pool = yb, None
             cfg.link_act = ActLink(yb, stb, N, H, W, cout, cout_s)
@@ -1611,14 +1626,19 @@
         else:
             act = _act_buffer(cfg, N, H, W, cout_s, dtype, dev) if cfg.need_act else None
             pool = torch.empty(N, H // 2, W // 2, cout_s, dtype=dtype, device=dev) if cfg.need_pool else None
-            _bnrelu_fwd(yb, dtc, N, H, W, cout_s, stb[2], stb[3], act, pool)
+            if want_ymax:
+                ymax = torch.empty_like(pool)
+                _n.call("spcl_bnrelu_pool_forward_ymax", _n.ptr(yb), dtc, N, H, W, cout_s, _n.ptr(stb[2]), _n.ptr(stb[3]), None,
+                        None, _n.ptr(pool), _n.ptr(ymax), _n.stream())
+            else:
+                _bnrelu_fwd(yb, dtc, N, H, W, cout_s, stb[2], stb[3], act, pool)
         ctx.save_for_backward(xs, ya, yb, sta, stb, wa, wb)
         ctx.x2s = x2s
         ctx.params = (wa, ga, ba, wb, gb, bb)
         ctx.packed_t = (wpa_t, wpb_t)
         ctx.cfg = cfg
         if need_bwd and pool is not None and act is None and cfg.training and dtype == torch.bfloat16:
-            cfg.link_out = PoolLink(yb, stb, N, H, W, cout_s, ctx.acc_bwd_b)
+            cfg.link_out = PoolLink(yb, stb, N, H, W, cout_s, ctx.acc_bwd_b, ymax)
         ctx.meta = (N, cin, H, W, cout, cout_s, cin_s, cin_k, mode_a, x.dtype)
         outs = []
         outs.append(nhwc_to_logical(act, cout) if act is not None else None)
@@ -1784,21 +1804,33 @@
             if (li is not None and dtype == torch.bfloat16 and li.cout_s == cin_s and li.N == N
                     and _n.call("spcl_conv_dgrad_poolstats_supported", dtc, N, H, W, cout_s, cin_s, li.H, li.W)):
                 dxs = torch.empty(N, H, W, cin_s, dtype=dtype, device=dya.device)
+                ym = li.ymax if (li.ymax is not None and tuple(li.ymax.shape) == (N, H, W, cin_s)) else None
                 if (li.acc is not None and _n.call("spcl_conv_dgrad_poolstats_acc_supported", dtc, N, H, W, cout_s, cin_s,
                                                    li.H, li.W)):
                     acc_in, li.acc = li.acc, None
-                    _n.call("spcl_conv3x3_dgrad_poolstats_acc", _n.ptr(dya), dtc, N, H, W, cout_s, cin_s, _n.ptr(wpa_t),
-                            _n.ptr(dxs), _n.ptr(li.yb), li.H, li.W, _n.ptr(li.stb[2]), _n.ptr(li.stb[3]), _n.ptr(li.stb[0]),
-                            _n.ptr(acc_in), _n.stream())
+                    if ym is not None and _n.call("spcl_conv_dgrad_poolmax_acc_supported", dtc, N, H, W, cout_s, cin_s):
+                        _n.call("spcl_conv3x3_dgrad_poolmax_acc", _n.ptr(dya), dtc, N, H, W, cout_s, cin_s, _n.ptr(wpa_t),
+                                _n.ptr(dxs), _n.ptr(ym), _n.ptr(li.stb[2]), _n.ptr(li.stb[3]), _n.ptr(li.stb[0]),
+                                _n.ptr(acc_in), _n.stream())
+                    else:
+                        _n.call("spcl_conv3x3_dgrad_poolstats_acc", _n.ptr(dya), dtc, N, H, W, cout_s, cin_s, _n.ptr(wpa_t),
+                                _n.ptr(dxs), _n.ptr(li.yb), li.H, li.W, _n.ptr(li.stb[2]), _n.ptr(li.stb[3]),
+                                _n.ptr(li.stb[0]), _n.ptr(acc_in), _n.stream())
                     rows = ACC_ROWS
                 else:
                     nt = _n.call("spcl_conv_stat_rows", dtc, N, H, W, cout_s, cin_s)
                     rows = torch.empty(nt * 2 * cin_s, dtype=torch.float32, device=dya.device)
-                    _n.call("spcl_conv3x3_dgrad_poolstats", _n.ptr(dya), dtc, N, H, W, cout_s, cin_s, _n.ptr(wpa_t),
-                            _n.ptr(dxs), _n.ptr(li.yb), li.H, li.W, _n.ptr(li.stb[2]), _n.ptr(li.stb[3]), _n.ptr(li.stb[0]),
-                            _n.ptr(rows), _n.stream())
+                    if ym is not None and _n.call("spcl_conv_dgrad_poolmax_supported", dtc, N, H, W, cout_s, cin_s):
+                        _n.call("spcl_conv3x3_dgrad_poolmax", _n.ptr(dya), dtc, N, H, W, cout_s, cin_s, _n.ptr(wpa_t),
+                                _n.ptr(dxs), _n.ptr(ym), _n.ptr(li.stb[2]), _n.ptr(li.stb[3]), _n.ptr(li.stb[0]),
+                                _n.ptr(rows), _n.stream())
+                    else:
+                        _n.call("spcl_conv3x3_dgrad_poolstats", _n.ptr(dya), dtc, N, H, W, cout_s, cin_s, _n.ptr(wpa_t),
+                                _n.ptr(dxs), _n.ptr(li.yb), li.H, li.W, _n.ptr(li.stb[2]), _n.ptr(li.stb[3]),
+                                _n.ptr(li.stb[0]), _n.ptr(rows), _n.stream())
                     rows.ntiles = nt
                 li.rows, li.dx_ptr, li.holder, li.version = rows, dxs.data_ptr(), dxs, dxs._version
+                li.ymax = None
             split = None
             if (dxs is None and x2s is not None and _CONV_SPLIT
                     and _n.call("spcl_conv_split_supported", dtc, N, H, W, cout_s, cin_s)):
@@ -1841,6 +1873,7 @@
 
 
 def conv_block(x, wa, ga, ba, wb, gb, bb, cfg: BlockCfg, x2=None):
+    cfg.grad_mode = torch.is_grad_enabled()
     act, pool = _ConvBlockFn.apply(x, wa, ga, ba, wb, gb, bb, cfg, x2)
     gap = getattr(cfg, "gap", None)
     if gap is not None and act is not None:
diff --git a/self-paced-contrastive-learning_amd/native.py b/self-paced-contrastive-learning_amd/native.py
--- a/self-paced-contrastive-learning_amd/native.py
+++ b/self-paced-contrastive-learning_amd/native.py
@@ -213,6 +213,11 @@
     "spcl_conv_dgrad_poolstats_acc_supported": (c_int, [c_int, c_int, c_int, c_int, c_int, c_int, c_int, c_int]),
     "spcl_conv3x3_dgrad_poolstats_acc": (c_int, [_P, c_int, c_int, c_int, c_int, c_int, c_int, _P, _P, _P, c_int, c_int, _P,
                                                  _P, _P, _P, _P]),
+    "spcl_bnrelu_pool_forward_ymax": (c_int, [_P, c_int, c_int, c_int, c_int, c_int, _P, _P, _P, _P, _P, _P, _P]),
+    "spcl_conv_dgrad_poolmax_supported": (c_int, [c_int, c_int, c_int, c_int, c_int, c_int]),
+    "spcl_conv3x3_dgrad_poolmax": (c_int, [_P, c_int, c_int, c_int, c_int, c_int, c_int, _P, _P, _P, _P, _P, _P, _P, _P]),
+    "spcl_conv_dgrad_poolmax_acc_supported": (c_int, [c_int, c_int, c_int, c_int, c_int, c_int]),
+    "spcl_conv3x3_dgrad_poolmax_acc": (c_int, [_P, c_int, c_int, c_int, c_int, c_int, c_int, _P, _P, _P, _P, _P, _P, _P, _P]),
     "spcl_bnrelu_backward_acc": (c_int, [_P, _P, _P, _P, c_int, c_int, c_int, c_int, c_int, c_int, _P, c_int, _P, _P, _P, _P,
                                          _P]),
     "spcl_iic_joint_workspace_bytes": (c_size_t, [c_int, c_int, c_int]),
@@ -293,12 +298,13 @@
                 ("nblk_co", c_int), ("CIB", c_int), ("COB", c_int), ("Cin", c_int), ("Cout", c_int)]
 
 
-ABI_VERSION = 22
+ABI_VERSION = 23
 WGRAD_BATCH_MAX = 16
 WGRAD_TAILS_MAX = 16
 _NO_STATUS = ("spcl_abi_version", "spcl_block1_recompute_supported", "spcl_block1_kernels_take", "spcl_conv16_bwd_fused_image_supported", "spcl_conv3x3_forward_image_acorr_rows", "spcl_image_autocorr_rows", "spcl_conv_dgrad_bnstats_image_supported", "spcl_conv16_bwd_fused_supported", "spcl_conv16_bwd_fused_splits", "spcl_conv_num_tiles", "spcl_conv_stat_rows", "spcl_conv_set_gemm", "spcl_conv_set_f32_split", "spcl_conv_get_f32_split", "spcl_supcon_unit_gradient_block", "spcl_conv_cat_supported", "spcl_conv_up2_supported", "spcl_conv_split_supported", "spcl_conv_split_bnstats_supported", "spcl_conv1x1_bwd_rows", "spcl_profile_count", "spcl_conv_dgrad_bnstats_supported", "spcl_conv_dgrad_poolstats_supported",
               "spcl_conv_wgrad_batched_supported", "spcl_conv_bn_acc_supported", "spcl_conv_dgrad_bnstats_acc_supported",
-              "spcl_conv_dgrad_poolstats_acc_supported", "spcl_supcon_rows_supported", "spcl_bnrelu_gap_supported")
+              "spcl_conv_dgrad_poolstats_acc_supported", "spcl_supcon_rows_supported", "spcl_bnrelu_gap_supported",
+              "spcl_conv_dgrad_poolmax_supported", "spcl_conv_dgrad_poolmax_acc_supported")
 
 
 class NativeLibraryError(RuntimeError):
```

Result: faster. 31610 slices/s, median of 6 (+1.2%).
